# lrjconan/LanczosNetwork

Hardware: NVIDIA B200
Metric: QM8 molecules/sec (forward) (higher is better)
Workload: dtype f32

## Files before the change

include/lanczosnet_b200.h:

```cpp
#ifndef LANCZOSNET_B200_H_
#define LANCZOSNET_B200_H_

#include <stdint.h>

#ifdef __cplusplus
extern "C" {
#endif

typedef void* lnb_stream_t;

#define LNB_OK 0
#define LNB_ERR_ARG (-1)
#define LNB_ERR_UNSUPPORTED (-2)

int lnb_abi_version(void);
const char* lnb_last_error(void);
int64_t lnb_launch_count(void);

int lnb_unsorted_segment_sum_forward(lnb_stream_t stream, const float* data,
                                     const int64_t* segment_ids, const int* data_shape,
                                     int num_segments, float* output);
int lnb_unsorted_segment_sum_backward(lnb_stream_t stream, const float* grad_output,
                                      const int64_t* segment_ids, const int* data_shape,
                                      int num_segments, float* grad_data);

typedef struct lnb_gemm_desc {
  const float* A; int64_t a_sb, a_sz, a_sm, a_sk;
  const float* B; int64_t b_sb, b_sz, b_sk, b_sn;
  float* C;       int64_t c_sb, c_sz, c_sm, c_sn;
  const float* kscale; int64_t s_sb, s_sz, s_sk;
  const float* bias; int64_t bias_sz;
  int32_t batch, nz, M, N, K, relu;
  float alpha, beta;
  const float* addend; int64_t d_sb, d_sz, d_sm, d_sn;
} lnb_gemm_desc;
int lnb_batched_gemm(lnb_stream_t stream, const lnb_gemm_desc* desc );

int lnb_split_tf32(lnb_stream_t stream, const float* x, int64_t n, float* hi, float* lo);
int lnb_linear_tf32x3(lnb_stream_t stream, const float* A, const float* W_hi, const float* W_lo,
                      const float* bias, int M, int N, int K, int relu, float* C);
int lnb_linear_tf32x3_splitk(lnb_stream_t stream, const float* A, const float* W_hi, const float* W_lo,
                             const float* bias, int M, int N, int K, int relu, float* C, int splits,
                             float* workspace, int* counters);

int lnb_linear_tf32x3_grouped(lnb_stream_t stream, const float* A, const float* W_hi,
                              const float* W_lo, const float* bias, int M, int groups, int N, int K,
                              int relu, float* C);

int lnb_graph_prepare(lnb_stream_t stream, const float* L, const float* Q, int B, int N, int E1,
                      int K, float* ell_val, uint8_t* ell_idx, int32_t* ell_max, int32_t* gext,
                      int32_t* tiles, int32_t* rowmap, int32_t* nrows, int flags);
int lnb_spectral_conv_fused(lnb_stream_t stream, const float* X, const float* Q, const float* coeff,
                            const float* ell_val, const uint8_t* ell_idx, const int32_t* ell_max,
                            const int32_t* gext, const int32_t* tiles, const float* W_hi,
                            const float* W_lo, const float* bias, int B, int N, int Din, int E1,
                            int K, int S, int H, int relu, int write_pad, float* out);

int lnb_graph_prepare_sparse(lnb_stream_t stream, const int32_t* sizes, const int32_t* node_ptr,
                             const int32_t* node_feat, const int32_t* edge_ptr, const uint8_t* edges,
                             const float* V_rows, const double* inv_sqrt_deg, int B, int N, int E1,
                             int K, int flags, float* ell_val, uint8_t* ell_idx, int32_t* ell_max,
                             int32_t* gext, int32_t* tiles, int32_t* rowmap, int32_t* nrows,
                             int64_t* node_ids, uint8_t* mask, float* V, float* L_dense);

#define LNB_PACKED_HOST_TILES 2
int lnb_graph_prepare_sparse_packed(lnb_stream_t stream, const uint8_t* blob, const double* inv_sqrt_deg,
                                    int B, int N, int E1, int K, int flags, float* ell_val,
                                    uint8_t* ell_idx, int32_t* ell_max, int32_t* gext, int32_t* tiles,
                                    int32_t* rowmap, int32_t* nrows, int64_t* node_ids, uint8_t* mask,
                                    float* V, float* L_dense);

typedef struct lnb_spectral_stack {
  const float* X; const int64_t* node_ids; const float* emb_table;
  const float* Q; const float* coeff; int64_t coeff_layer_stride;
  const float* ell_val; const uint8_t* ell_idx; const int32_t* ell_max; const int32_t* gext;
  const int32_t* tiles;
  const float* W_hi; const float* W_lo; const float* bias;
  float* out_state;
  const float* W_out; const float* b_out; const float* w_att; const float* b_att;
  const uint8_t* mask; float* score;
  int32_t Din[8];
  int32_t num_layers, Kw, emb_rows, P, write_pad;
  int32_t B, N, E1, K, S, H, relu;
} lnb_spectral_stack;
int lnb_spectral_stack_forward(lnb_stream_t stream, const lnb_spectral_stack* desc );

int lnb_embedding_rows(lnb_stream_t stream, const int64_t* idx, const float* table,
                       int64_t rows, int num_embeddings, int dim, float* out);

int lnb_ritz_power_table(lnb_stream_t stream, const float* D, int64_t rows, const int* powers,
                         int S, float* table );

int lnb_ritz_rowmap(lnb_stream_t stream, const int32_t* gext, int B, int K, int32_t* rowmap,
                    int32_t* nrows);
int lnb_ritz_filter_mlp(lnb_stream_t stream, const float* table, const int32_t* rowmap,
                        const int32_t* nrows, const float* W_hi, const float* W_lo,
                        const float* bias_all, int Rall, int L, int S, int Hd, float* coeff);

int lnb_readout(lnb_stream_t stream, const float* state, const float* W_out, const float* b_out,
                const float* w_att, const float* b_att, const uint8_t* mask, int B, int N, int H,
                int P, float* score );

int lnb_operator_chain(lnb_stream_t stream, const float* L, const float* X, int B, int N, int E1,
                       int D, int steps, int chebyshev, const int* block_of_step ,
                       float* out, int64_t out_batch_stride, int64_t out_row_stride, int out_col0);

int lnb_graph_messages(lnb_stream_t stream, const float* L, const float* X, const float* Q,
                       const float* filt, int B, int N, int E1, int D, int K, int S, int dense_filter,
                       int short_steps, const int* block_of_step , int n_short, float* out,
                       int64_t out_batch_stride, int64_t out_row_stride);

int lnb_gaussian_laplacian(lnb_stream_t stream, const float* x, const float* L, int B, int N,
                           int Dx, int E1, float* out );

int lnb_lanczos_tridiag(lnb_stream_t stream, const float* A, const uint8_t* mask, const float* q1,
                        int B, int N, int K, float* T, float* Q, float* alpha, float* beta,
                        int32_t* idx);

int lnb_tridiag_ritz(lnb_stream_t stream, const float* alpha, const float* beta, const float* Q,
                     int B, int N, int K, float* theta , float* ritz_vec ,
                     int32_t* status );

#define LNB_LANCZOS_PROPER 1
int lnb_lanczos_ritz(lnb_stream_t stream, const float* A, const uint8_t* mask, const float* q1,
                     int B, int N, int K, int flags, float* T, float* Q, float* alpha, float* beta,
                     int32_t* idx, float* theta , float* ritz_vec ,
                     int32_t* status );

int lnb_tridiag_powers(lnb_stream_t stream, const float* T, int B, int K, const int* powers, int S,
                       float* out );

int lnb_symmetrize_filters(lnb_stream_t stream, const float* Y, int B, int K, int S,
                           float* G );

int lnb_debug_set_prof(unsigned long long* buf);

#ifdef __cplusplus
}
#endif
#endif
```

lanczosnetwork_b200/_lib.py:

```python
import ctypes
import os
import threading

HERE = os.path.dirname(os.path.abspath(__file__))
LIB_PATH = os.path.join(HERE, 'liblanczosnet_b200.so')

c_f32p = ctypes.c_void_p
c_stream = ctypes.c_void_p
c_int = ctypes.c_int
c_i64 = ctypes.c_int64


class GemmDesc(ctypes.Structure):
  _fields_ = [
      ('A', ctypes.c_void_p), ('a_sb', c_i64), ('a_sz', c_i64), ('a_sm', c_i64), ('a_sk', c_i64),
      ('B', ctypes.c_void_p), ('b_sb', c_i64), ('b_sz', c_i64), ('b_sk', c_i64), ('b_sn', c_i64),
      ('C', ctypes.c_void_p), ('c_sb', c_i64), ('c_sz', c_i64), ('c_sm', c_i64), ('c_sn', c_i64),
      ('kscale', ctypes.c_void_p), ('s_sb', c_i64), ('s_sz', c_i64), ('s_sk', c_i64),
      ('bias', ctypes.c_void_p), ('bias_sz', c_i64),
      ('batch', ctypes.c_int32), ('nz', ctypes.c_int32), ('M', ctypes.c_int32),
      ('N', ctypes.c_int32), ('K', ctypes.c_int32), ('relu', ctypes.c_int32),
      ('alpha', ctypes.c_float), ('beta', ctypes.c_float),
      ('addend', ctypes.c_void_p), ('d_sb', c_i64), ('d_sz', c_i64), ('d_sm', c_i64), ('d_sn', c_i64),
  ]


class SpectralStack(ctypes.Structure):
  _fields_ = [
      ('X', ctypes.c_void_p), ('node_ids', ctypes.c_void_p), ('emb_table', ctypes.c_void_p),
      ('Q', ctypes.c_void_p), ('coeff', ctypes.c_void_p), ('coeff_layer_stride', c_i64),
      ('ell_val', ctypes.c_void_p), ('ell_idx', ctypes.c_void_p), ('ell_max', ctypes.c_void_p),
      ('gext', ctypes.c_void_p), ('tiles', ctypes.c_void_p),
      ('W_hi', ctypes.c_void_p), ('W_lo', ctypes.c_void_p), ('bias', ctypes.c_void_p),
      ('out_state', ctypes.c_void_p),
      ('W_out', ctypes.c_void_p), ('b_out', ctypes.c_void_p), ('w_att', ctypes.c_void_p),
      ('b_att', ctypes.c_void_p), ('mask', ctypes.c_void_p), ('score', ctypes.c_void_p),
      ('Din', ctypes.c_int32 * 8),
      ('num_layers', ctypes.c_int32), ('Kw', ctypes.c_int32), ('emb_rows', ctypes.c_int32),
      ('P', ctypes.c_int32), ('write_pad', ctypes.c_int32),
      ('B', ctypes.c_int32), ('N', ctypes.c_int32), ('E1', ctypes.c_int32), ('K', ctypes.c_int32),
      ('S', ctypes.c_int32), ('H', ctypes.c_int32), ('relu', ctypes.c_int32),
  ]


SIGNATURES = {
    'lnb_abi_version': (c_int, []),
    'lnb_last_error': (ctypes.c_char_p, []),
    'lnb_launch_count': (c_i64, []),
    'lnb_unsorted_segment_sum_forward':
        (c_int, [c_stream, c_f32p, ctypes.c_void_p, ctypes.POINTER(c_int), c_int, c_f32p]),
    'lnb_unsorted_segment_sum_backward':
        (c_int, [c_stream, c_f32p, ctypes.c_void_p, ctypes.POINTER(c_int), c_int, c_f32p]),
    'lnb_batched_gemm': (c_int, [c_stream, ctypes.POINTER(GemmDesc)]),
    'lnb_split_tf32': (c_int, [c_stream, c_f32p, c_i64, c_f32p, c_f32p]),
    'lnb_linear_tf32x3':
        (c_int, [c_stream, c_f32p, c_f32p, c_f32p, c_f32p, c_int, c_int, c_int, c_int, c_f32p]),
    'lnb_linear_tf32x3_splitk':
        (c_int, [c_stream, c_f32p, c_f32p, c_f32p, c_f32p, c_int, c_int, c_int, c_int, c_f32p, c_int,
                 c_f32p, ctypes.c_void_p]),
    'lnb_linear_tf32x3_grouped':
        (c_int, [c_stream, c_f32p, c_f32p, c_f32p, c_f32p, c_int, c_int, c_int, c_int, c_int, c_f32p]),
    'lnb_graph_prepare': (c_int, [c_stream, c_f32p, c_f32p, c_int, c_int, c_int, c_int, c_f32p,
                                  ctypes.c_void_p, ctypes.c_void_p, ctypes.c_void_p, ctypes.c_void_p,
                                  ctypes.c_void_p, ctypes.c_void_p, c_int]),
    'lnb_graph_prepare_sparse': (c_int, [c_stream] + [ctypes.c_void_p] * 7 + [c_int] * 5 +
                                 [ctypes.c_void_p] * 11),
    'lnb_graph_prepare_sparse_packed': (c_int, [c_stream] + [ctypes.c_void_p] * 2 + [c_int] * 5 +
                                        [ctypes.c_void_p] * 11),
    'lnb_spectral_conv_fused':
        (c_int, [c_stream, c_f32p, c_f32p, c_f32p, c_f32p, ctypes.c_void_p, ctypes.c_void_p,
                 ctypes.c_void_p, ctypes.c_void_p, c_f32p, c_f32p, c_f32p, c_int, c_int, c_int,
                 c_int, c_int, c_int, c_int, c_int, c_int, c_f32p]),
    'lnb_spectral_stack_forward': (c_int, [c_stream, ctypes.POINTER(SpectralStack)]),
    'lnb_ritz_rowmap': (c_int, [c_stream, ctypes.c_void_p, c_int, c_int, ctypes.c_void_p, ctypes.c_void_p]),
    'lnb_ritz_filter_mlp': (c_int, [c_stream, c_f32p, ctypes.c_void_p, ctypes.c_void_p, c_f32p, c_f32p,
                                    c_f32p, c_int, c_int, c_int, c_int, c_f32p]),
    'lnb_debug_set_prof': (c_int, [ctypes.c_void_p]),
    'lnb_embedding_rows': (c_int, [c_stream, ctypes.c_void_p, c_f32p, c_i64, c_int, c_int, c_f32p]),
    'lnb_ritz_power_table': (c_int, [c_stream, c_f32p, c_i64, ctypes.POINTER(c_int), c_int, c_f32p]),
    'lnb_readout': (c_int, [c_stream, c_f32p, c_f32p, c_f32p, c_f32p, c_f32p, ctypes.c_void_p,
                            c_int, c_int, c_int, c_int, c_f32p]),
    'lnb_operator_chain': (c_int, [c_stream, c_f32p, c_f32p, c_int, c_int, c_int, c_int, c_int, c_int,
                                   ctypes.POINTER(c_int), c_f32p, c_i64, c_i64, c_int]),
    'lnb_graph_messages': (c_int, [c_stream, c_f32p, c_f32p, c_f32p, c_f32p, c_int, c_int, c_int, c_int, c_int,
                                   c_int, c_int, c_int, ctypes.POINTER(c_int), c_int, c_f32p, c_i64, c_i64]),
    'lnb_gaussian_laplacian': (c_int, [c_stream, c_f32p, c_f32p, c_int, c_int, c_int, c_int, c_f32p]),
    'lnb_lanczos_tridiag': (c_int, [c_stream, c_f32p, ctypes.c_void_p, c_f32p, c_int, c_int, c_int,
                                    c_f32p, c_f32p, c_f32p, c_f32p, ctypes.c_void_p]),
    'lnb_tridiag_ritz': (c_int, [c_stream, c_f32p, c_f32p, c_f32p, c_int, c_int, c_int, c_f32p,
                                 c_f32p, ctypes.c_void_p]),
    'lnb_lanczos_ritz': (c_int, [c_stream, c_f32p, ctypes.c_void_p, c_f32p, c_int, c_int, c_int, c_int,
                                 c_f32p, c_f32p, c_f32p, c_f32p, ctypes.c_void_p, c_f32p, c_f32p,
                                 ctypes.c_void_p]),
    'lnb_tridiag_powers': (c_int, [c_stream, c_f32p, c_int, c_int, ctypes.POINTER(c_int), c_int,
                                   c_f32p]),
    'lnb_symmetrize_filters': (c_int, [c_stream, c_f32p, c_int, c_int, c_int, c_f32p]),
}

_lock = threading.Lock()
_lib = None


def load():
  global _lib
  if _lib is not None:
    return _lib
  with _lock:
    if _lib is None:
      if not os.path.exists(LIB_PATH):
        raise RuntimeError(
            'liblanczosnet_b200.so is not built (%s). Build it with '
            '`python -m lanczosnetwork_b200.build` (nvcc, sm_100a). There is no CPU fallback.'
            % LIB_PATH)
      lib = ctypes.CDLL(LIB_PATH)
      for name, (res, args) in SIGNATURES.items():
        fn = getattr(lib, name)
        fn.restype = res
        fn.argtypes = args
      if lib.lnb_abi_version() != 1:
        raise RuntimeError('liblanczosnet_b200.so ABI mismatch; rebuild')
      _lib = lib
  return _lib


def check(status, what):
  if status != 0:
    msg = load().lnb_last_error()
    raise RuntimeError('%s failed (status %d): %s' % (what, status, (msg or b'').decode()))


_replayed = [0]


def note_graph_replay(num_kernels):
  _replayed[0] += int(num_kernels)


def launch_count():
  return int(load().lnb_launch_count()) + _replayed[0]
```

lanczosnetwork_b200/csrc/linear_tf32x3.cu:

```cuda
#include "tc_gemm.cuh"

namespace {

struct RowLoadPolicy {
  static constexpr int kStagesB = 6;
  struct Params {
    const float* A;
    const float* bias;
    float* C;
    int M, N, K, relu, groups;
    int dbg;
    int splits;
    float* ws;
    int* counters;
  };
  static __device__ __forceinline__ int tiles_per_group(const Params& p) { return (p.N + tcg::BN - 1) / tcg::BN; }
  static __device__ __forceinline__ int n_tiles(const Params& p) { return p.groups * tiles_per_group(p); }
  static __device__ __forceinline__ int num_tiles(const Params& p) {
    return ((p.M + tcg::BM - 1) / tcg::BM) * n_tiles(p);
  }
  static __device__ __forceinline__ int num_steps(const Params& p, int cta, int ncta) {
    const int t = num_tiles(p) * p.splits;
    return t > cta ? (t - cta + ncta - 1) / ncta : 0;
  }
  static __device__ __forceinline__ void decode(const Params& p, int cta, int ncta, int it,
                                                int& m_tile, int& sub) {
    const int item = cta + it * ncta, nt = n_tiles(p);
    const int tile = item / p.splits, split = item - tile * p.splits;
    m_tile = tile / nt;
    sub = tile % nt + nt * split;
  }
  static __device__ __forceinline__ int kb_total(const Params& p) { return (p.K + tcg::BK - 1) / tcg::BK; }
  static __device__ __forceinline__ int kb_per_split(const Params& p) { return (kb_total(p) + p.splits - 1) / p.splits; }
  static __device__ __forceinline__ int kb_begin(const Params& p, int sub) { return (sub / n_tiles(p)) * kb_per_split(p); }
  static __device__ __forceinline__ int num_kblocks(const Params& p, int sub) {
    const int left = kb_total(p) - kb_begin(p, sub), per = kb_per_split(p);
    return left < per ? left : per;
  }
  static __device__ __forceinline__ int w_row0(const Params& p, int sub) {
    const int tpg = tiles_per_group(p), ns = sub % n_tiles(p);
    return (ns / tpg) * p.N + (ns % tpg) * tcg::BN;
  }
  static __device__ __forceinline__ void w_coords(const Params& p, int sub, int kb, int& col0, int& row0) {
    col0 = (kb_begin(p, sub) + kb) * tcg::BK;
    row0 = w_row0(p, sub);
  }

  const Params& p;
  const int r, grp;
  const int lda, ldc;
  const float* arow;
  bool row_ok;
  int row, kb0, tile;
  float cur[32];
  int* flag;

  __device__ RowLoadPolicy(const Params& p_, uint8_t* smem, int tid)
      : p(p_), r(tid & 127), grp(tid >> 7), lda(p_.groups * p_.K), ldc(p_.groups * p_.N),
        arow(nullptr), row_ok(false), row(0), kb0(0), tile(0), flag(reinterpret_cast<int*>(smem)) {}

  __device__ __forceinline__ void load(int kb, float (&v)[32]) {
#pragma unroll
    for (int j = 0; j < 8; ++j) {
      const int k = (kb0 + kb) * tcg::BK + 4 * j;
      float4 t = make_float4(0.f, 0.f, 0.f, 0.f);
      if (row_ok && k < p.K) t = __ldg(reinterpret_cast<const float4*>(arow + k));
      v[4 * j + 0] = t.x; v[4 * j + 1] = t.y; v[4 * j + 2] = t.z; v[4 * j + 3] = t.w;
    }
  }
  __device__ __forceinline__ void step_begin(int m_tile, int sub, int kb_first, tcg::PhaseTimer&) {
    row = m_tile * tcg::BM + r;
    row_ok = row < p.M;
    const int ns = sub % n_tiles(p);
    kb0 = kb_begin(p, sub);
    tile = m_tile * n_tiles(p) + ns;
    arow = p.A + (int64_t)(row_ok ? row : 0) * lda + (ns / tiles_per_group(p)) * p.K;
    load(kb_first, cur);
  }
  __device__ __forceinline__ void produce(int, int kb, float (&v)[32]) {
#pragma unroll
    for (int j = 0; j < 32; ++j) v[j] = cur[j];
    load(kb + tcg::NGROUPS, cur);
  }
  __device__ __forceinline__ void pre_epilogue(int) {}
  __device__ __forceinline__ void store(int sub, int col, const float (&x)[tcg::EW]) {
    if (p.splits > 1) {
      float4* dst = reinterpret_cast<float4*>(
          p.ws + (((int64_t)tile * p.splits + sub / n_tiles(p)) * tcg::BM + r) * tcg::BN + col);
#pragma unroll
      for (int q = 0; q < tcg::EW / 4; ++q)
        __stcg(dst + q, make_float4(x[4 * q], x[4 * q + 1], x[4 * q + 2], x[4 * q + 3]));
      return;
    }
    const int left = p.N - ((sub % n_tiles(p)) % tiles_per_group(p)) * tcg::BN;
    const int w0 = w_row0(p, sub);
    tcg::store_row_chunk(row_ok ? p.C + (int64_t)row * ldc + w0 : nullptr,
                         left < tcg::BN ? left : tcg::BN, p.bias ? p.bias + w0 : nullptr,
                         p.relu != 0, col, x);
  }
  __device__ __forceinline__ void post_epilogue(int sub) {
    if (p.splits == 1) return;
    const int tid = grp * 128 + r;
    __threadfence();
    tcg::producers_sync();
    if (tid == 0) {
      const int old = atomicAdd(p.counters + tile, 1);
      *flag = (old == p.splits - 1);
      if (old == p.splits - 1) p.counters[tile] = 0;
    }
    tcg::producers_sync();
    if (*flag) {
      __threadfence();
      const int ns = sub % n_tiles(p);
      const int m0 = (tile / n_tiles(p)) * tcg::BM;
      const int left = p.N - (ns % tiles_per_group(p)) * tcg::BN;
      const int ncols = left < tcg::BN ? left : tcg::BN;
      const int w0 = w_row0(p, sub);
      const float* base = p.ws + (int64_t)tile * p.splits * tcg::BM * tcg::BN;
      for (int e = tid; e < tcg::BM * tcg::BN / 4; e += tcg::PRODUCER_THREADS) {
        const int rr = e / (tcg::BN / 4), c4 = (e - rr * (tcg::BN / 4)) * 4;
        if (m0 + rr >= p.M || c4 >= ncols) continue;
        float4 acc = __ldcg(reinterpret_cast<const float4*>(base + rr * tcg::BN + c4));
        for (int sp = 1; sp < p.splits; ++sp) {
          const float4 t = __ldcg(reinterpret_cast<const float4*>(base + ((int64_t)sp * tcg::BM + rr) * tcg::BN + c4));
          acc.x += t.x; acc.y += t.y; acc.z += t.z; acc.w += t.w;
        }
        float y[4] = {acc.x, acc.y, acc.z, acc.w};
        float* out = p.C + (int64_t)(m0 + rr) * ldc + w0 + c4;
#pragma unroll
        for (int u = 0; u < 4; ++u) {
          if (c4 + u < ncols) {
            if (p.bias) y[u] += __ldg(p.bias + w0 + c4 + u);
            if (p.relu) y[u] = fmaxf(y[u], 0.f);
            out[u] = y[u];
          }
        }
      }
    }
    tcg::producers_sync();
  }
};

constexpr size_t SMEM_BYTES = tcg::core_smem(RowLoadPolicy::kStagesB) + 1024 + 16;

}

static int launch_linear(lnb_stream_t stream, const float* A, const float* W_hi, const float* W_lo,
                         const float* bias, int M, int N, int K, int groups, int relu, float* C,
                         const char* who, int splits = 1, float* ws = nullptr, int* counters = nullptr) {
  LNB_REQUIRE(A && W_hi && W_lo && C, "%s: null pointer", who);
  LNB_REQUIRE(M >= 0 && N >= 1 && K >= 1 && groups >= 1, "%s: bad dims M=%d N=%d K=%d groups=%d",
              who, M, N, K, groups);
  LNB_REQUIRE(K % 4 == 0, "%s: K=%d must be a multiple of 4 (16-byte rows)", who, K);
  LNB_REQUIRE(((uintptr_t)A & 15) == 0 && ((uintptr_t)W_hi & 15) == 0 && ((uintptr_t)W_lo & 15) == 0,
              "%s: A / W must be 16-byte aligned", who);
  if (M == 0) return LNB_OK;
  CUtensorMap map_hi, map_lo;
  int rc = tcg::make_weight_map(&map_hi, W_hi, groups * N, K, who);
  if (rc != LNB_OK) return rc;
  rc = tcg::make_weight_map(&map_lo, W_lo, groups * N, K, who);
  if (rc != LNB_OK) return rc;
  auto kern = tcg::tc_gemm_kernel<RowLoadPolicy>;
  cudaFuncSetAttribute(kern, cudaFuncAttributeMaxDynamicSharedMemorySize, (int)SMEM_BYTES);
  const int nkb = lnb::ceil_div(K, tcg::BK);
  LNB_REQUIRE(splits >= 1 && splits <= 16 && (splits == 1 || (ws && counters)),
              "%s: split-K needs 1 <= splits <= 16, a workspace and counters", who);
  LNB_REQUIRE(splits == 1 || lnb::ceil_div(nkb, splits) * (splits - 1) < nkb,
              "%s: %d splits leave an empty k range for K=%d", who, splits, K);
  RowLoadPolicy::Params p{A, bias, C, M, N, K, relu, groups, tcg::debug_flags(), splits, ws, counters};
  const int tiles = lnb::ceil_div(M, tcg::BM) * lnb::ceil_div(N, tcg::BN) * groups * splits;
  const int grid = tiles < tcg::sm_count() ? tiles : tcg::sm_count();
  kern<<<grid, tcg::THREADS, SMEM_BYTES, (cudaStream_t)stream>>>(map_hi, map_lo, p);
  lnb::count_launch();
  return lnb::finish_launch(who);
}

extern "C" {

int lnb_linear_tf32x3(lnb_stream_t stream, const float* A, const float* W_hi, const float* W_lo,
                      const float* bias, int M, int N, int K, int relu, float* C) {
  return launch_linear(stream, A, W_hi, W_lo, bias, M, N, K, 1, relu, C, "linear_tf32x3");
}

int lnb_linear_tf32x3_splitk(lnb_stream_t stream, const float* A, const float* W_hi, const float* W_lo,
                             const float* bias, int M, int N, int K, int relu, float* C, int splits,
                             float* workspace, int* counters) {
  return launch_linear(stream, A, W_hi, W_lo, bias, M, N, K, 1, relu, C, "linear_tf32x3_splitk", splits,
                       workspace, counters);
}

int lnb_linear_tf32x3_grouped(lnb_stream_t stream, const float* A, const float* W_hi,
                              const float* W_lo, const float* bias, int M, int groups, int N, int K,
                              int relu, float* C) {
  return launch_linear(stream, A, W_hi, W_lo, bias, M, N, K, groups, relu, C,
                       "linear_tf32x3_grouped");
}

}
```

lanczosnetwork_b200/csrc/spectral_conv_fused.cu:

```cuda
#include "tc_gemm.cuh"

namespace {

constexpr int KMAX = 32;
constexpr int GMAX = 32;
constexpr int RMAX = 128;
constexpr int EMAX = 16;
constexpr int FR = 8;

template <bool STAGE>
__global__ void __launch_bounds__(256)
graph_prepare_kernel(const float* __restrict__ L, const float* __restrict__ Q, int N, int E1, int K,
                     float* __restrict__ ell_val, uint8_t* __restrict__ ell_idx,
                     int32_t* __restrict__ ell_max, int32_t* __restrict__ gext, int binarize) {
  extern __shared__ __align__(16) float gp_smem[];
  __shared__ int s_max[EMAX];
  __shared__ int s_ext[2];
  __shared__ uint8_t cnt_s[256 * EMAX];
  const int b = blockIdx.x, tid = threadIdx.x;
  if (tid < EMAX) s_max[tid] = 0;
  if (tid < 2) s_ext[tid] = 0;
  const int64_t per = (int64_t)N * N * E1;
  const float* Lg = L + b * per;
  if (STAGE) {
    if ((per & 3) == 0) {
      for (int i = tid; i < (int)(per >> 2); i += 256) tc05::cp_async_16(gp_smem + 4 * i, Lg + 4 * i);
    } else {
      for (int i = tid; i < (int)per; i += 256) tc05::cp_async_4(gp_smem + i, Lg + i);
    }
  }
  const float* Lb = STAGE ? gp_smem : Lg;
  const float* Qb = Q + (int64_t)b * N * K;
  int ne = 0, ke = 0;
  for (int i = tid; i < N * K; i += 256) {
    if (__ldg(Qb + i) != 0.f) {
      ne = max(ne, i / K + 1);
      ke = max(ke, i % K + 1);
    }
  }
  if (STAGE) tc05::cp_async_wait_all();
  __syncthreads();
  const int pairs = N * E1;
  for (int p = tid; p < pairs; p += 256) {
    const int n = p / E1, e = p - n * E1;
    const float* row = Lb + (n * N) * E1 + e;
    float* val = ell_val + ((int64_t)(b * E1 + e) * N) * N + n;
    uint8_t* idx = ell_idx + ((int64_t)(b * E1 + e) * N) * N + n;
    int cnt = 0, far = 0;
    const float dg = row[n * E1];
    if (dg != 0.f) {
      val[0] = binarize ? 1.f : dg;
      idx[0] = (uint8_t)n;
      cnt = 1;
      far = n + 1;
    }
#pragma unroll 2
    for (int i = 0; i < N; ++i) {
      const float v = row[i * E1];
      if (v != 0.f && i != n) {
        val[cnt * N] = binarize ? 1.f : v;
        idx[cnt * N] = (uint8_t)i;
        ++cnt;
        far = max(far, i + 1);
      }
    }
    cnt_s[p] = (uint8_t)cnt;
    if (cnt) {
      atomicMax(&s_max[e], cnt);
      ne = max(ne, max(n + 1, far));
    }
  }
  if (ne) atomicMax(&s_ext[0], ne);
  if (ke) atomicMax(&s_ext[1], ke);
  __syncthreads();
  for (int pr = tid; pr < pairs; pr += 256) {
    const int n = pr / E1, e = pr - n * E1;
    float* val = ell_val + ((int64_t)(b * E1 + e) * N) * N + n;
    uint8_t* idx = ell_idx + ((int64_t)(b * E1 + e) * N) * N + n;
    for (int t = cnt_s[pr]; t < s_max[e]; ++t) {
      val[(int64_t)t * N] = 0.f;
      idx[(int64_t)t * N] = 0;
    }
  }
  if (tid < E1) ell_max[b * E1 + tid] = s_max[tid];
  if (tid < 2) gext[b * 2 + tid] = s_ext[tid];
}

template <bool in_smem>
__global__ void __launch_bounds__(1024)
tile_assign_kernel(const int32_t* __restrict__ gext, int B, int K, int32_t* __restrict__ tiles,
                   int32_t* __restrict__ scratch , int32_t* __restrict__ rowmap,
                   int32_t* __restrict__ nrows) {
  extern __shared__ int32_t ta_smem[];
  __shared__ int warp_n[32], warp_k[32], warp_r[32];
  __shared__ int run_n, run_k, run_r;
  const int tid = threadIdx.x, lane = tid & 31, warp = tid >> 5;
  int32_t* PN = in_smem ? ta_smem : scratch;
  int32_t* PK = PN + B;
  int32_t* NX = PK + B;
  int32_t* PR = NX + 3 * (B + 1);
  if (tid == 0) { run_n = 0; run_k = 0; run_r = 0; }
  __syncthreads();
  for (int b0 = 0; b0 < B; b0 += 1024) {
    const int b = b0 + tid;
    const int n = (b < B) ? gext[b * 2] : 0;
    const int kr = (b < B) ? min(gext[b * 2 + 1], K) : 0;
    const int k = (b < B) ? ((gext[b * 2 + 1] + 3) & ~3) : 0;
    int in = n, ik = k, ir = kr;
#pragma unroll
    for (int o = 1; o < 32; o <<= 1) {
      const int tn = __shfl_up_sync(0xffffffffu, in, o), tk = __shfl_up_sync(0xffffffffu, ik, o);
      const int tr = __shfl_up_sync(0xffffffffu, ir, o);
      if (lane >= o) { in += tn; ik += tk; ir += tr; }
    }
    if (lane == 31) { warp_n[warp] = in; warp_k[warp] = ik; warp_r[warp] = ir; }
    __syncthreads();
    if (warp == 0) {
      int wn = warp_n[lane], wk = warp_k[lane], wr = warp_r[lane], sn = wn, sk = wk, sr = wr;
#pragma unroll
      for (int o = 1; o < 32; o <<= 1) {
        const int tn = __shfl_up_sync(0xffffffffu, sn, o), tk = __shfl_up_sync(0xffffffffu, sk, o);
        const int tr = __shfl_up_sync(0xffffffffu, sr, o);
        if (lane >= o) { sn += tn; sk += tk; sr += tr; }
      }
      warp_n[lane] = sn - wn;
      warp_k[lane] = sk - wk;
      warp_r[lane] = sr - wr;
    }
    __syncthreads();
    if (b < B) {
      PN[b] = run_n + warp_n[warp] + in;
      PK[b] = run_k + warp_k[warp] + ik;
      if (in_smem) {
        PR[b] = run_r + warp_r[warp] + ir;
      } else if (rowmap) {
        const int base = run_r + warp_r[warp] + ir - kr;
        for (int i = 0; i < kr; ++i) rowmap[base + i] = b * K + i;
      }
    }
    __syncthreads();
    if (tid == 1023) { run_n += warp_n[31] + in; run_k += warp_k[31] + ik; run_r += warp_r[31] + ir; }
    __syncthreads();
  }
  if (tid == 0 && nrows) nrows[0] = run_r;
  __threadfence_block();
  if (in_smem && rowmap) {
    for (int b = warp; b < B; b += 32) {
      const int base = b ? PR[b - 1] : 0, kr = PR[b] - base;
      for (int i = lane; i < kr; i += 32) rowmap[base + i] = b * K + i;
    }
  }
  for (int i = tid; i < B; i += 1024) {
    const int pn0 = i ? PN[i - 1] : 0, pk0 = i ? PK[i - 1] : 0;
    int j = i + 1;
    const int jmax = min(B, i + GMAX);
    while (j < jmax && PN[j] - pn0 <= RMAX && PK[j] - pk0 <= RMAX) ++j;
    NX[i] = j;
  }
  __syncthreads();
  if (!in_smem) {
    if (tid == 0) {
      int T = 0, i = 0;
      while (i < B) { tiles[1 + T] = i; ++T; i = NX[i]; }
      tiles[0] = T;
      tiles[1 + T] = B;
    }
    return;
  }
  int32_t* Ja = NX;
  int32_t* Jb = NX + (B + 1);
  int32_t* MK = Jb + (B + 1);
  for (int i = tid; i <= B; i += 1024) MK[i] = (i == 0) ? 1 : 0;
  if (tid == 0) { Ja[B] = B; Jb[B] = B; }
  __syncthreads();
  for (int span = 1; span < B; span <<= 1) {
    for (int i = tid; i < B; i += 1024)
      if (MK[i]) MK[Ja[i]] = 1;
    for (int i = tid; i < B; i += 1024) Jb[i] = Ja[Ja[i]];
    __syncthreads();
    int32_t* t = Ja; Ja = Jb; Jb = t;
  }
  if (tid == 0) run_n = 0;
  __syncthreads();
  for (int b0 = 0; b0 < B; b0 += 1024) {
    const int b = b0 + tid;
    const int m = (b < B) ? MK[b] : 0;
    int in = m;
#pragma unroll
    for (int o = 1; o < 32; o <<= 1) {
      const int tn = __shfl_up_sync(0xffffffffu, in, o);
      if (lane >= o) in += tn;
    }
    if (lane == 31) warp_n[warp] = in;
    __syncthreads();
    if (warp == 0) {
      int wn = warp_n[lane], sn = wn;
#pragma unroll
      for (int o = 1; o < 32; o <<= 1) {
        const int tn = __shfl_up_sync(0xffffffffu, sn, o);
        if (lane >= o) sn += tn;
      }
      warp_n[lane] = sn - wn;
    }
    __syncthreads();
    if (m) tiles[1 + run_n + warp_n[warp] + in - 1] = b;
    __syncthreads();
    if (tid == 1023) run_n += warp_n[31] + in;
    __syncthreads();
  }
  if (tid == 0) {
    tiles[0] = run_n;
    tiles[1 + run_n] = B;
  }
}

struct SpectralPolicy {
  static constexpr int kStagesB = 2;
  static constexpr int LMAX = 8;
  struct Params {
    const float* X;
    const int64_t* node_ids;
    const float* emb;
    const float* Q;
    const float* coeff;
    int64_t coeff_stride;
    const float* ell_val;
    const uint8_t* ell_idx;
    const int32_t* ell_max;
    const int32_t* gext;
    const int32_t* tiles;
    const float* bias;
    float* out;
    const float* W_out;
    const float* b_out;
    const float* w_att;
    const float* b_att;
    const uint8_t* mask;
    float* score;
    int P, emb_rows;
    int L;
    int Din[LMAX];
    int B, N, E1, K, S, H, relu;
    int LB;
    int write_pad;
    int dbg;
  };
  static __device__ __forceinline__ int num_steps(const Params& p, int cta, int ncta) {
    const int T = __ldg(p.tiles);
    const int mine = T > cta ? (T - cta + ncta - 1) / ncta : 0;
    return (p.S > 0 ? 2 : 1) * p.L * mine;
  }
  static __device__ __forceinline__ void decode(const Params& p, int cta, int ncta, int it,
                                                int& m_tile, int& sub) {
    const int per = (p.S > 0 ? 2 : 1) * p.L;
    const int rem = it % per;
    m_tile = cta + (it / per) * ncta;
    sub = p.S > 0 ? rem : rem * 2 + 1;
  }
  static __device__ __forceinline__ int num_kblocks(const Params& p, int sub) {
    return ((sub & 1) == 0 ? p.S : p.E1) * p.Din[sub >> 1] / tcg::BK;
  }
  static __device__ __forceinline__ void w_coords(const Params& p, int sub, int kb, int& col0, int& row0) {
    col0 = ((sub & 1) == 0 ? 0 : p.S * p.Din[sub >> 1]) + kb * tcg::BK;
    row0 = (sub >> 1) * p.H;
  }

  struct Tables {
    int gs, ng, Rtot, Ztot, nquads, nlines;
    int nbase[GMAX + 1], kbase[GMAX + 1], gn[GMAX], gk[GMAX];
    int cnt_e[EMAX], base_e[EMAX], tmax_e[EMAX];
    uint8_t emax[GMAX][EMAX];
    uint8_t row_g[RMAX], row_n[RMAX], z_g[RMAX], z_k[RMAX];
    uint8_t q_g[RMAX / 4 + GMAX], q_n0[RMAX / 4 + GMAX];
    uint8_t line_e[256], line_t[256];
  };

  const Params& p;
  const int tid, r;
  const int N, K, S, E1, H, XP;
  int Din;
  float* Xs;
  float* UZ;
  float* Qs;
  Tables* tb;
  float* Ev;
  uint8_t* Ei;
  float fr[FR];
  tcg::PhaseTimer* ptm = nullptr;

  static __host__ __device__ constexpr size_t tables_bytes() { return (sizeof(Tables) + 15) & ~size_t(15); }

  __device__ SpectralPolicy(const Params& p_, uint8_t* smem, int tid_)
      : p(p_), tid(tid_), r(tid_ & 127), N(p_.N), K(p_.K), S(p_.S), E1(p_.E1),
        H(p_.H), XP((p_.Din[0] > p_.H ? p_.Din[0] : p_.H) + 4), Din(p_.Din[0]) {
    Xs = reinterpret_cast<float*>(smem);
    UZ = Xs + (size_t)RMAX * XP;
    Qs = UZ + (size_t)RMAX * XP;
    uint8_t* t8 = reinterpret_cast<uint8_t*>(Qs + (size_t)RMAX * K);
    tb = reinterpret_cast<Tables*>(t8);
    Ev = reinterpret_cast<float*>(t8 + tables_bytes());
    Ei = reinterpret_cast<uint8_t*>(Ev + (size_t)p.LB * RMAX);
  }
  static size_t smem_fixed(int Din, int K, int H) {
    const int W = (Din > H ? Din : H) + 4;
    return (size_t)2 * RMAX * W * 4 + (size_t)RMAX * K * 4 + tables_bytes() + 16;
  }
  static size_t ell_line_bytes() { return (size_t)RMAX * 5; }

  __device__ void build_tables(int m_tile) {
    const int lane = tid & 31;
    const int gs = __ldg(p.tiles + 1 + m_tile), ge = __ldg(p.tiles + 2 + m_tile);
    const int ng = ge - gs;
    int n = 0, k = 0;
    if (lane < ng) {
      n = __ldg(p.gext + (gs + lane) * 2);
      k = __ldg(p.gext + (gs + lane) * 2 + 1);
    }
    const int kp = (k + 3) & ~3, nq = (n + 3) >> 2;
    int pn = n, pk = kp, pq = nq;
#pragma unroll
    for (int o = 1; o < 32; o <<= 1) {
      const int a = __shfl_up_sync(0xffffffffu, pn, o), bq = __shfl_up_sync(0xffffffffu, pk, o);
      const int c = __shfl_up_sync(0xffffffffu, pq, o);
      if (lane >= o) { pn += a; pk += bq; pq += c; }
    }
    const int nb = pn - n, kb = pk - kp, qb = pq - nq;
    if (lane < ng) {
      tb->nbase[lane] = nb; tb->kbase[lane] = kb; tb->gn[lane] = n; tb->gk[lane] = k;
      for (int i = 0; i < n; ++i) { tb->row_g[nb + i] = (uint8_t)lane; tb->row_n[nb + i] = (uint8_t)i; }
      for (int i = 0; i < kp; ++i) { tb->z_g[kb + i] = (uint8_t)lane; tb->z_k[kb + i] = (uint8_t)i; }
      for (int i = 0; i < nq; ++i) { tb->q_g[qb + i] = (uint8_t)lane; tb->q_n0[qb + i] = (uint8_t)(4 * i); }
    }
    const int Rtot = __shfl_sync(0xffffffffu, pn, 31), Ztot = __shfl_sync(0xffffffffu, pk, 31);
    const int nquads = __shfl_sync(0xffffffffu, pq, 31);
    int em[EMAX];
#pragma unroll
    for (int e = 0; e < EMAX; ++e)
      em[e] = (e < E1 && lane < ng) ? __ldg(p.ell_max + (gs + lane) * E1 + e) : 0;
#pragma unroll
    for (int e = 0; e < EMAX; ++e) {
      if (e < E1) {
        int m = em[e];
        if (lane < ng) tb->emax[lane][e] = (uint8_t)m;
#pragma unroll
        for (int o = 16; o > 0; o >>= 1) m = max(m, __shfl_xor_sync(0xffffffffu, m, o));
        if (lane == 0) tb->tmax_e[e] = m;
      }
    }
    __syncwarp();
    if (lane == 0) {
      tb->gs = gs; tb->ng = ng; tb->Rtot = Rtot; tb->Ztot = Ztot; tb->nquads = nquads;
      tb->nbase[ng] = Rtot; tb->kbase[ng] = Ztot;
      int left = p.LB, base = 0;
      for (int e = 0; e < E1; ++e) {
        const int c = min(tb->tmax_e[e], left);
        tb->cnt_e[e] = c; tb->base_e[e] = base;
        for (int t = 0; t < c; ++t) { tb->line_e[base + t] = (uint8_t)e; tb->line_t[base + t] = (uint8_t)t; }
        base += c; left -= c;
      }
      tb->nlines = base;
    }
  }

  __device__ void step_begin(int m_tile, int sub, int , tcg::PhaseTimer& tm) {
    tcg::producers_sync();
    const int layer = sub >> 1, step = sub & 1;
    if (step == 1 && S > 0) return;
    Din = p.Din[layer];
    const int warp = tid >> 5, lane = tid & 31;
    constexpr int NW = tcg::PRODUCER_THREADS / 32;
    const int dv = Din / 4;
    ptm = &tm;
    if (layer == 0) {
    if (warp == 0) build_tables(m_tile);
    tcg::producers_sync();
    tm.lap(16);
    const int gs = tb->gs, Rtot = tb->Rtot;
    int64_t my_id = 0;
    if (!p.X && warp + lane * NW < Rtot) {
      const int row = warp + lane * NW;
      my_id = __ldg(p.node_ids + (int64_t)(gs + tb->row_g[row]) * N + tb->row_n[row]);
    }
    for (int row = warp, j = 0; row < Rtot; row += NW, ++j) {
      const int64_t src_row = (int64_t)(gs + tb->row_g[row]) * N + tb->row_n[row];
      const float* xsrc;
      if (p.X) {
        xsrc = p.X + src_row * Din;
      } else {
        int64_t id = __shfl_sync(0xffffffffu, my_id, j);
        id = id < 0 ? 0 : (id >= p.emb_rows ? p.emb_rows - 1 : id);
        xsrc = p.emb + id * Din;
      }
      float* xd = Xs + (size_t)row * XP;
      for (int q4 = lane; q4 < dv; q4 += 32) tc05::cp_async_16(xd + 4 * q4, xsrc + 4 * q4);
      const float* qsrc = p.Q + src_row * K;
      float* qd = Qs + (size_t)row * K;
      for (int k4 = lane; k4 < (K >> 2); k4 += 32) tc05::cp_async_16(qd + 4 * k4, qsrc + 4 * k4);
    }
    tm.lap(17);
    {
      constexpr int ELL_BATCH = 4;
      const int nlines = tb->nlines;
      for (int base = warp; base < nlines; base += NW * ELL_BATCH) {
        for (int r0 = 0; r0 < Rtot; r0 += 32) {
          const int rr = r0 + lane;
          float vv[ELL_BATCH];
          int ii[ELL_BATCH];
#pragma unroll
          for (int u = 0; u < ELL_BATCH; ++u) {
            const int line = base + u * NW;
            vv[u] = 0.f; ii[u] = 0;
            if (line < nlines && rr < Rtot) {
              const int e = tb->line_e[line], t = tb->line_t[line];
              const int g = tb->row_g[rr], n = tb->row_n[rr];
              if (t < tb->emax[g][e]) {
                const int64_t off = (((int64_t)(gs + g) * E1 + e) * N + t) * N + n;
                vv[u] = __ldg(p.ell_val + off);
                ii[u] = tb->nbase[g] + __ldg(p.ell_idx + off);
              }
            }
          }
#pragma unroll
          for (int u = 0; u < ELL_BATCH; ++u) {
            const int line = base + u * NW;
            if (line < nlines && rr < Rtot) {
              Ev[(size_t)line * RMAX + rr] = vv[u];
              Ei[(size_t)line * RMAX + rr] = (uint8_t)ii[u];
            }
          }
        }
      }
    }
    tm.lap(18);
    }
    const int gs = tb->gs, Ztot = tb->Ztot;
#pragma unroll
    for (int i = 0; i < FR; ++i) fr[i] = 0.f;
    if (S > 0 && r < Ztot) {
      const int g = tb->z_g[r], k = tb->z_k[r];
      if (k < tb->gk[g]) {
        const float* f = p.coeff + layer * p.coeff_stride + ((int64_t)(gs + g) * K + k) * S;
#pragma unroll
        for (int i = 0; i < FR; ++i)
          if (i < S) fr[i] = __ldg(f + i);
      }
    }
    tm.lap(0);
    tc05::cp_async_wait_all();
    tcg::producers_sync();
    tm.lap(1);
    if (S == 0) return;
    for (int task = tid; task < (Ztot >> 2) * dv; task += tcg::PRODUCER_THREADS) {
      const int dq = task % dv, zq = task / dv;
      const int g = tb->z_g[4 * zq], k0 = tb->z_k[4 * zq];
      const int n_g = tb->gn[g], nb = tb->nbase[g];
      float acc[4][4];
#pragma unroll
      for (int i = 0; i < 4; ++i)
#pragma unroll
        for (int j = 0; j < 4; ++j) acc[i][j] = 0.f;
      const float* xs = Xs + (size_t)nb * XP + 4 * dq;
      const float* qs = Qs + (size_t)nb * K + k0;
#pragma unroll 4
      for (int nn = 0; nn < n_g; ++nn) {
        const float4 x4 = *reinterpret_cast<const float4*>(xs + (size_t)nn * XP);
        const float4 q4 = *reinterpret_cast<const float4*>(qs + (size_t)nn * K);
        const float qv[4] = {q4.x, q4.y, q4.z, q4.w};
        const float xv[4] = {x4.x, x4.y, x4.z, x4.w};
#pragma unroll
        for (int i = 0; i < 4; ++i)
#pragma unroll
          for (int j = 0; j < 4; ++j) acc[i][j] = fmaf(qv[i], xv[j], acc[i][j]);
      }
#pragma unroll
      for (int i = 0; i < 4; ++i)
        *reinterpret_cast<float4*>(UZ + (size_t)(4 * zq + i) * XP + 4 * dq) =
            make_float4(acc[i][0], acc[i][1], acc[i][2], acc[i][3]);
    }
    tcg::producers_sync();
    tm.lap(2);
  }

  __device__ __forceinline__ void produce(int sub, int kb, float (&v)[32]) {
#pragma unroll
    for (int j = 0; j < 32; ++j) v[j] = 0.f;
    const int j0 = kb * tcg::BK;
    const int c = j0 / Din, d0 = j0 - c * Din;
    if ((sub & 1) == 0) {
      if (r >= tb->Ztot) return;
      float f = 0.f;
      if (S <= FR) {
#pragma unroll
        for (int i = 0; i < FR; ++i) f = (i == c) ? fr[i] : f;
      } else {
        const int g = tb->z_g[r], k = tb->z_k[r];
        f = (k < tb->gk[g]) ? __ldg(p.coeff + (sub >> 1) * p.coeff_stride + ((int64_t)(tb->gs + g) * K + k) * S + c) : 0.f;
      }
      const float4* u4 = reinterpret_cast<const float4*>(UZ + (size_t)r * XP + d0);
#pragma unroll
      for (int q = 0; q < 8; ++q) {
        const float4 t = u4[q];
        v[4 * q + 0] = f * t.x; v[4 * q + 1] = f * t.y; v[4 * q + 2] = f * t.z; v[4 * q + 3] = f * t.w;
      }
      return;
    }
    if (r >= tb->Rtot) return;
    const int e = c;
    const float* xs = Xs + d0;
    const int ts = tb->cnt_e[e], tmax = tb->tmax_e[e];
    const float* ev = Ev + (size_t)tb->base_e[e] * RMAX + r;
    const uint8_t* ei = Ei + (size_t)tb->base_e[e] * RMAX + r;
#pragma unroll 2
    for (int t = 0; t < ts; ++t) {
      const float a = ev[t * RMAX];
      if (a == 0.f) continue;
      const int i = ei[t * RMAX];
      const float4* x4 = reinterpret_cast<const float4*>(xs + (size_t)i * XP);
#pragma unroll
      for (int q = 0; q < 8; ++q) {
        const float4 tt = x4[q];
        v[4 * q + 0] = fmaf(a, tt.x, v[4 * q + 0]);
        v[4 * q + 1] = fmaf(a, tt.y, v[4 * q + 1]);
        v[4 * q + 2] = fmaf(a, tt.z, v[4 * q + 2]);
        v[4 * q + 3] = fmaf(a, tt.w, v[4 * q + 3]);
      }
    }
    if (ts < tmax) {
      const int g = tb->row_g[r], n = tb->row_n[r];
      const int my = tb->emax[g][e], nb = tb->nbase[g];
      const int64_t off0 = (((int64_t)(tb->gs + g) * E1 + e) * N) * N + n;
      for (int t = ts; t < tmax; ++t) {
        float a = 0.f;
        int i = 0;
        if (t < my) {
          a = __ldg(p.ell_val + off0 + (int64_t)t * N);
          i = nb + __ldg(p.ell_idx + off0 + (int64_t)t * N);
        }
        if (a == 0.f) continue;
        const float4* x4 = reinterpret_cast<const float4*>(xs + (size_t)i * XP);
#pragma unroll
        for (int q = 0; q < 8; ++q) {
          const float4 tt = x4[q];
          v[4 * q + 0] = fmaf(a, tt.x, v[4 * q + 0]);
          v[4 * q + 1] = fmaf(a, tt.y, v[4 * q + 1]);
          v[4 * q + 2] = fmaf(a, tt.z, v[4 * q + 2]);
          v[4 * q + 3] = fmaf(a, tt.w, v[4 * q + 3]);
        }
      }
    }
  }

  __device__ void pre_epilogue(int sub) {
    if ((sub & 1) == 0) return;
    tcg::producers_sync();
    if (ptm) ptm->lap(22);
    if (S == 0) return;
    const int hv = H / 4;
    for (int task = tid; task < tb->nquads * hv; task += tcg::PRODUCER_THREADS) {
      const int hq = task % hv, q = task / hv;
      const int g = tb->q_g[q], n0 = tb->q_n0[q];
      const int n_g = tb->gn[g], k_g = tb->gk[g];
      const int r0 = tb->nbase[g] + n0;
      float acc[4][4];
#pragma unroll
      for (int i = 0; i < 4; ++i)
#pragma unroll
        for (int j = 0; j < 4; ++j) acc[i][j] = 0.f;
      const float* z = UZ + (size_t)tb->kbase[g] * XP + 4 * hq;
      const float* q0 = Qs + (size_t)r0 * K;
      const int r1 = (n0 + 1 < n_g) ? 1 : 0, r2 = (n0 + 2 < n_g) ? 2 : 0, r3 = (n0 + 3 < n_g) ? 3 : 0;
      for (int k = 0; k < k_g; k += 4) {
        const float4 a0 = *reinterpret_cast<const float4*>(q0 + k);
        const float4 a1 = *reinterpret_cast<const float4*>(q0 + r1 * K + k);
        const float4 a2 = *reinterpret_cast<const float4*>(q0 + r2 * K + k);
        const float4 a3 = *reinterpret_cast<const float4*>(q0 + r3 * K + k);
        const float av[4][4] = {{a0.x, a0.y, a0.z, a0.w}, {a1.x, a1.y, a1.z, a1.w},
                                {a2.x, a2.y, a2.z, a2.w}, {a3.x, a3.y, a3.z, a3.w}};
#pragma unroll
        for (int kk = 0; kk < 4; ++kk) {
          const float4 z4 = *reinterpret_cast<const float4*>(z + (size_t)(k + kk) * XP);
          const float zv[4] = {z4.x, z4.y, z4.z, z4.w};
#pragma unroll
          for (int i = 0; i < 4; ++i)
#pragma unroll
            for (int j = 0; j < 4; ++j) acc[i][j] = fmaf(av[i][kk], zv[j], acc[i][j]);
        }
      }
#pragma unroll
      for (int i = 0; i < 4; ++i)
        if (n0 + i < n_g)
          *reinterpret_cast<float4*>(Xs + (size_t)(r0 + i) * XP + 4 * hq) =
              make_float4(acc[i][0], acc[i][1], acc[i][2], acc[i][3]);
    }
    tcg::producers_sync();
  }

  __device__ __forceinline__ void store(int sub, int col, float (&x)[tcg::EW]) {
    if (col >= H) return;
    if ((sub & 1) == 0) {
      if (r < tb->Ztot) {
        float4* z4 = reinterpret_cast<float4*>(UZ + (size_t)r * XP + col);
#pragma unroll
        for (int q = 0; q < tcg::EW / 4; ++q)
          z4[q] = make_float4(x[4 * q + 0], x[4 * q + 1], x[4 * q + 2], x[4 * q + 3]);
      }
      return;
    }
    if (r >= tb->Rtot) return;
    float4* o4 = reinterpret_cast<float4*>(Xs + (size_t)r * XP + col);
    const bool relu = p.relu != 0;
    const float* bias = p.bias ? p.bias + (sub >> 1) * H : nullptr;
#pragma unroll
    for (int q = 0; q < tcg::EW / 4; ++q) {
      float y[4] = {x[4 * q + 0], x[4 * q + 1], x[4 * q + 2], x[4 * q + 3]};
      if (S > 0) {
        const float4 t = o4[q];
        y[0] += t.x; y[1] += t.y; y[2] += t.z; y[3] += t.w;
      }
      if (col + 4 * q + 3 < H) {
        if (bias) {
          const float4 b4 = __ldg(reinterpret_cast<const float4*>(bias + col) + q);
          y[0] += b4.x; y[1] += b4.y; y[2] += b4.z; y[3] += b4.w;
        }
        if (relu) { y[0] = fmaxf(y[0], 0.f); y[1] = fmaxf(y[1], 0.f); y[2] = fmaxf(y[2], 0.f); y[3] = fmaxf(y[3], 0.f); }
      } else {
#pragma unroll
        for (int u = 0; u < 4; ++u) {
          const int c = col + 4 * q + u;
          if (c < H) {
            if (bias) y[u] += __ldg(bias + c);
            if (relu) y[u] = fmaxf(y[u], 0.f);
          }
        }
      }
      o4[q] = make_float4(y[0], y[1], y[2], y[3]);
    }
  }

  __device__ void post_epilogue(int sub) {
    if ((sub & 1) == 0 || (sub >> 1) != p.L - 1) return;
    tcg::producers_sync();
    if (ptm) ptm->lap(19);
    const int warp = tid >> 5, lane = tid & 31;
    constexpr int NW = tcg::PRODUCER_THREADS / 32;
    const int hv = H / 4, gs = tb->gs, Rtot = tb->Rtot;
    const float* bias = p.bias ? p.bias + (p.L - 1) * H : nullptr;
    if (p.out) {
      for (int row = warp; row < Rtot; row += NW) {
        const float4* src = reinterpret_cast<const float4*>(Xs + (size_t)row * XP);
        float4* dst = reinterpret_cast<float4*>(
            p.out + ((int64_t)(gs + tb->row_g[row]) * N + tb->row_n[row]) * H);
        for (int q4 = lane; q4 < hv; q4 += 32) dst[q4] = src[q4];
      }
      if (p.write_pad) {
        const int npad = tb->ng * N - Rtot;
        for (int i = warp; i < npad; i += NW) {
          int g = 0, rem = i;
          while (rem >= N - tb->gn[g]) { rem -= N - tb->gn[g]; ++g; }
          float4* dst = reinterpret_cast<float4*>(p.out + ((int64_t)(gs + g) * N + tb->gn[g] + rem) * H);
          for (int q4 = lane; q4 < hv; q4 += 32) {
            float y[4];
#pragma unroll
            for (int u = 0; u < 4; ++u) {
              float t = bias ? __ldg(bias + 4 * q4 + u) : 0.f;
              y[u] = (p.relu != 0) ? fmaxf(t, 0.f) : t;
            }
            dst[q4] = make_float4(y[0], y[1], y[2], y[3]);
          }
        }
      }
    }
    if (p.score) readout(bias);
  }

  __device__ void readout(const float* bias_last) {
    const int P = p.P, P1 = p.P + 1, PQ = (P1 + 3) >> 2, HP = H + 4;
    float* Wr = UZ;
    float* Yr = Wr + (size_t)4 * PQ * HP;
    float* cx = Yr + (size_t)(RMAX + 1) * P1 + ((4 - ((RMAX + 1) * P1 & 3)) & 3);
    for (int e = tid; e < 4 * PQ * H; e += tcg::PRODUCER_THREADS) {
      const int o = e / H, h = e - o * H;
      Wr[o * HP + h] = (o < P) ? __ldg(p.W_out + o * H + h) : (o == P ? __ldg(p.w_att + h) : 0.f);
    }
    for (int h = tid; h < H; h += tcg::PRODUCER_THREADS) {
      float t = bias_last ? __ldg(bias_last + h) : 0.f;
      cx[h] = (p.relu != 0) ? fmaxf(t, 0.f) : t;
    }
    uint8_t* mk = reinterpret_cast<uint8_t*>(cx + H);
    for (int e = tid; e < tb->ng * N; e += tcg::PRODUCER_THREADS)
      mk[e] = p.mask ? __ldg(p.mask + (int64_t)tb->gs * N + e) : (uint8_t)1;
    tcg::producers_sync();
    if (ptm) ptm->lap(20);
    const int Rtot = tb->Rtot;
    {
      const int warp = tid >> 5, lane = tid & 31;
      const int rb = warp & 3, og = warp >> 2;
      const int per = (P1 + tcg::NGROUPS - 1) / tcg::NGROUPS;
      const int o_end = min(P1, (og + 1) * per);
      const int row = rb * 32 + lane;
      const float4* x4 = reinterpret_cast<const float4*>(Xs + (size_t)(row < Rtot ? row : 0) * XP);
      for (int o0 = og * per; o0 < o_end; o0 += 6) {
        const int cnt = min(6, o_end - o0);
        const float4* w4 = reinterpret_cast<const float4*>(Wr + (size_t)o0 * HP);
        float acc[6] = {0.f, 0.f, 0.f, 0.f, 0.f, 0.f};
#pragma unroll 4
        for (int h4 = 0; h4 < H / 4; ++h4) {
          const float4 x = x4[h4];
#pragma unroll
          for (int j = 0; j < 6; ++j) {
            if (j < cnt) {
              const float4 wv = w4[j * (HP / 4) + h4];
              acc[j] = fmaf(x.x, wv.x, acc[j]); acc[j] = fmaf(x.y, wv.y, acc[j]);
              acc[j] = fmaf(x.z, wv.z, acc[j]); acc[j] = fmaf(x.w, wv.w, acc[j]);
            }
          }
        }
        if (row < Rtot) {
#pragma unroll
          for (int j = 0; j < 6; ++j)
            if (j < cnt) {
              const int o = o0 + j;
              const float v = acc[j] + ((o < P) ? __ldg(p.b_out + o) : __ldg(p.b_att));
              Yr[row * P1 + o] = (o < P) ? v : 1.f / (1.f + expf(-v));
            }
        }
      }
      for (int o = warp; o < P1; o += tcg::PRODUCER_THREADS / 32) {
        float acc = 0.f;
        for (int h = lane; h < H; h += 32) acc = fmaf(cx[h], Wr[o * HP + h], acc);
#pragma unroll
        for (int sh = 16; sh > 0; sh >>= 1) acc += __shfl_xor_sync(0xffffffffu, acc, sh);
        if (lane == 0) {
          const float v = acc + ((o < P) ? __ldg(p.b_out + o) : __ldg(p.b_att));
          Yr[RMAX * P1 + o] = (o < P) ? v : 1.f / (1.f + expf(-v));
        }
      }
    }
    tcg::producers_sync();
    if (ptm) ptm->lap(21);
    for (int e = tid; e < tb->ng * P; e += tcg::PRODUCER_THREADS) {
      const int g = e / P, o = e - g * P;
      const int nb = tb->nbase[g], n_g = tb->gn[g];
      const uint8_t* m = mk + g * N;
      float acc = 0.f;
      int cnt = 0;
      for (int n = 0; n < N; ++n) {
        if (m[n] == 0) continue;
        const float* y = Yr + (n < n_g ? nb + n : RMAX) * P1;
        acc += y[P] * y[o];
        ++cnt;
      }
      p.score[(int64_t)(tb->gs + g) * P + o] = acc / (float)cnt;
    }
  }
};

}

namespace lnb {
void launch_tile_assign(cudaStream_t s, const int32_t* gext, int B, int K, int32_t* tiles,
                        int32_t* rowmap, int32_t* nrows) {
  const size_t tbytes = (size_t)6 * (B + 1) * sizeof(int32_t);
  const int tsm = tbytes <= 200 * 1024;
  if (tsm && tbytes > 40 * 1024)
    cudaFuncSetAttribute(tile_assign_kernel<true>, cudaFuncAttributeMaxDynamicSharedMemorySize, (int)tbytes);
  if (tsm)
    tile_assign_kernel<true><<<1, 1024, tbytes, s>>>(gext, B, K, tiles, tiles + B + 2, rowmap, nrows);
  else
    tile_assign_kernel<false><<<1, 1024, 0, s>>>(gext, B, K, tiles, tiles + B + 2, rowmap, nrows);
}
}

extern "C" {

int lnb_debug_set_prof(unsigned long long* buf) {
  cudaError_t e = cudaMemcpyToSymbol(tcg::g_prof, &buf, sizeof(buf));
  if (e != cudaSuccess) { lnb::set_err("debug_set_prof: %s", cudaGetErrorString(e)); return (int)e; }
  lnb::set_prof_buffer(buf);
  return LNB_OK;
}

int lnb_graph_prepare(lnb_stream_t stream, const float* L, const float* Q, int B, int N, int E1,
                      int K, float* ell_val, uint8_t* ell_idx, int32_t* ell_max, int32_t* gext,
                      int32_t* tiles ,
                      int32_t* rowmap, int32_t* nrows, int flags) {
  LNB_REQUIRE(L && Q && ell_val && ell_idx && ell_max && gext && tiles, "graph_prepare: null pointer");
  LNB_REQUIRE((rowmap == nullptr) == (nrows == nullptr), "graph_prepare: rowmap and nrows go together");
  LNB_REQUIRE(B >= 0 && N >= 1 && N <= 255 && E1 >= 1 && E1 <= EMAX && K >= 1,
              "graph_prepare: bad dims B=%d N=%d E1=%d K=%d", B, N, E1, K);
  if (B == 0) return LNB_OK;
  cudaStream_t s = (cudaStream_t)stream;
  const size_t lbytes = (size_t)N * N * E1 * sizeof(float);
  const int stage = lbytes <= 64 * 1024;
  if (stage) {
    if (lbytes > 40 * 1024)
      cudaFuncSetAttribute(graph_prepare_kernel<true>, cudaFuncAttributeMaxDynamicSharedMemorySize, (int)lbytes);
    graph_prepare_kernel<true><<<B, 256, lbytes, s>>>(L, Q, N, E1, K, ell_val, ell_idx, ell_max, gext,
                                                      flags & 1);
  } else {
    graph_prepare_kernel<false><<<B, 256, 0, s>>>(L, Q, N, E1, K, ell_val, ell_idx, ell_max, gext,
                                                  flags & 1);
  }
  lnb::launch_tile_assign(s, gext, B, K, tiles, rowmap, nrows);
  lnb::count_launch(2);
  return lnb::finish_launch("graph_prepare");
}

static int launch_stack(lnb_stream_t stream, const lnb_spectral_stack& d, const char* who) {
  LNB_REQUIRE((d.X || (d.node_ids && d.emb_table)) && d.Q && d.ell_val && d.ell_idx && d.ell_max &&
                  d.gext && d.tiles && d.W_hi && d.W_lo && (d.out_state || d.score) &&
                  (d.coeff || d.S == 0),
              "%s: null pointer", who);
  LNB_REQUIRE(d.B >= 0 && d.N >= 1 && d.E1 >= 1 && d.K >= 1 && d.S >= 0 && d.H >= 1 &&
                  d.num_layers >= 1 && d.num_layers <= SpectralPolicy::LMAX,
              "%s: bad dims", who);
  LNB_REQUIRE(!d.score || (d.W_out && d.b_out && d.w_att && d.b_att && d.P >= 1 && d.P <= 48),
              "%s: readout needs W_out, b_out, w_att, b_att and 1 <= P <= 48", who);
  int dmax = 0;
  bool ok = d.N <= RMAX && d.K <= KMAX && d.K % 4 == 0 && d.H % 4 == 0 && d.H <= tcg::BN && d.E1 <= EMAX;
  for (int l = 0; l < d.num_layers; ++l) {
    ok = ok && d.Din[l] % 32 == 0 && d.Din[l] >= 32 && (l == 0 || d.Din[l] == d.H);
    dmax = d.Din[l] > dmax ? d.Din[l] : dmax;
  }
  ok = ok && (d.S + d.E1) * dmax <= d.Kw;
  if (!ok) {
    lnb::set_err("%s: unsupported shape N=%d K=%d H=%d E1=%d (needs N<=128, Din%%32==0, inner "
                 "layers Din==H, K%%4==0, K<=%d, H%%4==0, H<=128, E1<=%d)", who, d.N, d.K, d.H, d.E1,
                 KMAX, EMAX);
    return LNB_ERR_UNSUPPORTED;
  }
  if ((d.bias && (reinterpret_cast<uintptr_t>(d.bias) & 15)) || (reinterpret_cast<uintptr_t>(d.Q) & 15) ||
      (d.X && (reinterpret_cast<uintptr_t>(d.X) & 15)) || (d.emb_table && (reinterpret_cast<uintptr_t>(d.emb_table) & 15))) {
    lnb::set_err("%s: X / emb_table / Q / bias must be 16-byte aligned", who);
    return LNB_ERR_ARG;
  }
  if (d.B == 0) return LNB_OK;
  size_t smem = tcg::core_smem(SpectralPolicy::kStagesB) + 1024 + SpectralPolicy::smem_fixed(dmax, d.K, d.H);
  if (smem > 227 * 1024) {
    lnb::set_err("%s: tile state (Din=%d, K=%d, H=%d) needs %zu B of shared memory", who, dmax, d.K,
                 d.H, smem);
    return LNB_ERR_UNSUPPORTED;
  }
  int lb = (int)((227 * 1024 - smem) / SpectralPolicy::ell_line_bytes());
  if (lb > 255) lb = 255;
  smem += (size_t)lb * SpectralPolicy::ell_line_bytes();
  CUtensorMap map_hi, map_lo;
  int rc = tcg::make_weight_map(&map_hi, d.W_hi, d.num_layers * d.H, d.Kw, who);
  if (rc != LNB_OK) return rc;
  rc = tcg::make_weight_map(&map_lo, d.W_lo, d.num_layers * d.H, d.Kw, who);
  if (rc != LNB_OK) return rc;
  auto kern = tcg::tc_gemm_kernel<SpectralPolicy>;
  cudaFuncSetAttribute(kern, cudaFuncAttributeMaxDynamicSharedMemorySize, (int)smem);
  SpectralPolicy::Params p{};
  p.X = d.X; p.node_ids = d.node_ids; p.emb = d.emb_table; p.Q = d.Q;
  p.coeff = d.coeff; p.coeff_stride = d.coeff_layer_stride;
  p.ell_val = d.ell_val; p.ell_idx = d.ell_idx; p.ell_max = d.ell_max; p.gext = d.gext; p.tiles = d.tiles;
  p.bias = d.bias; p.out = d.out_state;
  p.W_out = d.W_out; p.b_out = d.b_out; p.w_att = d.w_att; p.b_att = d.b_att; p.mask = d.mask;
  p.score = d.score; p.P = d.P; p.emb_rows = d.emb_rows; p.L = d.num_layers;
  for (int l = 0; l < d.num_layers; ++l) p.Din[l] = d.Din[l];
  p.B = d.B; p.N = d.N; p.E1 = d.E1; p.K = d.K; p.S = d.S; p.H = d.H; p.relu = d.relu;
  p.LB = lb; p.write_pad = d.write_pad; p.dbg = tcg::debug_flags();
  const int grid = d.B < tcg::sm_count() ? d.B : tcg::sm_count();
  kern<<<grid, tcg::THREADS, smem, (cudaStream_t)stream>>>(map_hi, map_lo, p);
  lnb::count_launch();
  return lnb::finish_launch(who);
}

int lnb_spectral_stack_forward(lnb_stream_t stream, const lnb_spectral_stack* desc) {
  LNB_REQUIRE(desc, "spectral_stack_forward: null descriptor");
  return launch_stack(stream, *desc, "spectral_stack_forward");
}

int lnb_spectral_conv_fused(lnb_stream_t stream, const float* X, const float* Q, const float* coeff,
                            const float* ell_val, const uint8_t* ell_idx, const int32_t* ell_max,
                            const int32_t* gext, const int32_t* tiles, const float* W_hi,
                            const float* W_lo, const float* bias, int B, int N, int Din, int E1,
                            int K, int S, int H, int relu, int write_pad, float* out) {
  lnb_spectral_stack d{};
  d.X = X; d.Q = Q; d.coeff = coeff; d.coeff_layer_stride = 0;
  d.ell_val = ell_val; d.ell_idx = ell_idx; d.ell_max = ell_max; d.gext = gext; d.tiles = tiles;
  d.W_hi = W_hi; d.W_lo = W_lo; d.Kw = (S + E1) * Din; d.bias = bias;
  d.Din[0] = Din; d.num_layers = 1; d.out_state = out; d.write_pad = write_pad;
  d.B = B; d.N = N; d.E1 = E1; d.K = K; d.S = S; d.H = H; d.relu = relu;
  return launch_stack(stream, d, "spectral_conv_fused");
}

}
```

lanczosnetwork_b200/csrc/tc05.cuh:

```cuda
#pragma once
#include <cuda.h>
#include <cuda_runtime.h>
#include <stdint.h>

namespace tc05 {

__device__ __forceinline__ uint32_t smem_u32(const void* p) {
  return static_cast<uint32_t>(__cvta_generic_to_shared(p));
}

__device__ __forceinline__ void mbar_init(uint64_t* bar, uint32_t count) {
  asm volatile("mbarrier.init.shared::cta.b64 [%0], %1;" ::"r"(smem_u32(bar)), "r"(count));
}
__device__ __forceinline__ void fence_barrier_init() {
  asm volatile("fence.mbarrier_init.release.cluster;" ::: "memory");
}
__device__ __forceinline__ void mbar_arrive(uint64_t* bar) {
  asm volatile("mbarrier.arrive.shared::cta.b64 _, [%0];" ::"r"(smem_u32(bar)) : "memory");
}
__device__ __forceinline__ void mbar_arrive_expect_tx(uint64_t* bar, uint32_t bytes) {
  asm volatile("mbarrier.arrive.expect_tx.shared::cta.b64 _, [%0], %1;" ::"r"(smem_u32(bar)),
               "r"(bytes)
               : "memory");
}
__device__ __forceinline__ bool mbar_try_wait(uint64_t* bar, uint32_t parity) {
  uint32_t ok;
  asm volatile(
      "{\n\t.reg .pred p;\n\t"
      "mbarrier.try_wait.parity.shared::cta.b64 p, [%1], %2;\n\t"
      "selp.b32 %0, 1, 0, p;\n\t}"
      : "=r"(ok)
      : "r"(smem_u32(bar)), "r"(parity)
      : "memory");
  return ok != 0;
}
__device__ __forceinline__ void mbar_wait(uint64_t* bar, uint32_t parity) {
  while (!mbar_try_wait(bar, parity)) {
  }
}
__device__ __forceinline__ void mbar_wait2(uint64_t* bar_a, uint32_t parity_a, uint64_t* bar_b,
                                           uint32_t parity_b) {
  bool oka = mbar_try_wait(bar_a, parity_a), okb = mbar_try_wait(bar_b, parity_b);
  while (!(oka && okb)) {
    if (!oka) oka = mbar_try_wait(bar_a, parity_a);
    if (!okb) okb = mbar_try_wait(bar_b, parity_b);
  }
}

__device__ __forceinline__ void tma_prefetch_desc(const CUtensorMap* m) {
  asm volatile("prefetch.tensormap [%0];" ::"l"(reinterpret_cast<uint64_t>(m)) : "memory");
}
__device__ __forceinline__ void tma_load_2d(void* smem_dst, const CUtensorMap* m, uint64_t* bar,
                                            int32_t c0, int32_t c1) {
  asm volatile(
      "cp.async.bulk.tensor.2d.shared::cluster.global.mbarrier::complete_tx::bytes"
      " [%0], [%1, {%3, %4}], [%2];"
      ::"r"(smem_u32(smem_dst)), "l"(reinterpret_cast<uint64_t>(m)), "r"(smem_u32(bar)), "r"(c0),
      "r"(c1)
      : "memory");
}

__device__ __forceinline__ void cp_async_16(void* smem_dst, const void* gmem_src) {
  asm volatile("cp.async.cg.shared.global [%0], [%1], 16;" ::"r"(smem_u32(smem_dst)), "l"(gmem_src)
               : "memory");
}
__device__ __forceinline__ void cp_async_4(void* smem_dst, const void* gmem_src) {
  asm volatile("cp.async.ca.shared.global [%0], [%1], 4;" ::"r"(smem_u32(smem_dst)), "l"(gmem_src)
               : "memory");
}
__device__ __forceinline__ void cp_async_wait_all() {
  asm volatile("cp.async.commit_group;\n\tcp.async.wait_group 0;" ::: "memory");
}

__device__ __forceinline__ void tmem_alloc(uint32_t* smem_holder, uint32_t ncols) {
  asm volatile("tcgen05.alloc.cta_group::1.sync.aligned.shared::cta.b32 [%0], %1;" ::"r"(
                   smem_u32(smem_holder)),
               "r"(ncols)
               : "memory");
  asm volatile("tcgen05.relinquish_alloc_permit.cta_group::1.sync.aligned;" ::: "memory");
}
__device__ __forceinline__ void tmem_dealloc(uint32_t taddr, uint32_t ncols) {
  asm volatile("tcgen05.dealloc.cta_group::1.sync.aligned.b32 %0, %1;" ::"r"(taddr), "r"(ncols)
               : "memory");
}
__device__ __forceinline__ void fence_before_thread_sync() {
  asm volatile("tcgen05.fence::before_thread_sync;" ::: "memory");
}
__device__ __forceinline__ void fence_after_thread_sync() {
  asm volatile("tcgen05.fence::after_thread_sync;" ::: "memory");
}
__device__ __forceinline__ void tmem_wait_ld() {
  asm volatile("tcgen05.wait::ld.sync.aligned;" ::: "memory");
}
__device__ __forceinline__ void tmem_wait_st() {
  asm volatile("tcgen05.wait::st.sync.aligned;" ::: "memory");
}

__device__ __forceinline__ void tmem_ld_32x32(uint32_t taddr, uint32_t (&v)[32]) {
  asm volatile(
      "tcgen05.ld.sync.aligned.32x32b.x32.b32 "
      "{%0, %1, %2, %3, %4, %5, %6, %7, %8, %9, %10, %11, %12, %13, %14, %15, "
      "%16, %17, %18, %19, %20, %21, %22, %23, %24, %25, %26, %27, %28, %29, %30, %31}, [%32];"
      : "=r"(v[0]), "=r"(v[1]), "=r"(v[2]), "=r"(v[3]), "=r"(v[4]), "=r"(v[5]), "=r"(v[6]),
        "=r"(v[7]), "=r"(v[8]), "=r"(v[9]), "=r"(v[10]), "=r"(v[11]), "=r"(v[12]), "=r"(v[13]),
        "=r"(v[14]), "=r"(v[15]), "=r"(v[16]), "=r"(v[17]), "=r"(v[18]), "=r"(v[19]),
        "=r"(v[20]), "=r"(v[21]), "=r"(v[22]), "=r"(v[23]), "=r"(v[24]), "=r"(v[25]),
        "=r"(v[26]), "=r"(v[27]), "=r"(v[28]), "=r"(v[29]), "=r"(v[30]), "=r"(v[31])
      : "r"(taddr)
      : "memory");
}
__device__ __forceinline__ void tmem_ld_32x16(uint32_t taddr, uint32_t (&v)[16]) {
  asm volatile(
      "tcgen05.ld.sync.aligned.32x32b.x16.b32 "
      "{%0, %1, %2, %3, %4, %5, %6, %7, %8, %9, %10, %11, %12, %13, %14, %15}, [%16];"
      : "=r"(v[0]), "=r"(v[1]), "=r"(v[2]), "=r"(v[3]), "=r"(v[4]), "=r"(v[5]), "=r"(v[6]),
        "=r"(v[7]), "=r"(v[8]), "=r"(v[9]), "=r"(v[10]), "=r"(v[11]), "=r"(v[12]), "=r"(v[13]),
        "=r"(v[14]), "=r"(v[15])
      : "r"(taddr)
      : "memory");
}
__device__ __forceinline__ void tmem_st_32x32(uint32_t taddr, const uint32_t (&v)[32]) {
  asm volatile(
      "tcgen05.st.sync.aligned.32x32b.x32.b32 [%0], "
      "{%1, %2, %3, %4, %5, %6, %7, %8, %9, %10, %11, %12, %13, %14, %15, %16, "
      "%17, %18, %19, %20, %21, %22, %23, %24, %25, %26, %27, %28, %29, %30, %31, %32};"
      ::"r"(taddr), "r"(v[0]), "r"(v[1]), "r"(v[2]), "r"(v[3]), "r"(v[4]), "r"(v[5]), "r"(v[6]),
      "r"(v[7]), "r"(v[8]), "r"(v[9]), "r"(v[10]), "r"(v[11]), "r"(v[12]), "r"(v[13]),
      "r"(v[14]), "r"(v[15]), "r"(v[16]), "r"(v[17]), "r"(v[18]), "r"(v[19]), "r"(v[20]),
      "r"(v[21]), "r"(v[22]), "r"(v[23]), "r"(v[24]), "r"(v[25]), "r"(v[26]), "r"(v[27]),
      "r"(v[28]), "r"(v[29]), "r"(v[30]), "r"(v[31])
      : "memory");
}

__device__ __forceinline__ uint64_t umma_desc_kmajor_sw128(uint32_t smem_addr) {
  uint64_t d = 0;
  d |= (uint64_t)((smem_addr >> 4) & 0x3FFFu);
  d |= (uint64_t)1 << 16;
  d |= (uint64_t)64 << 32;
  d |= (uint64_t)1 << 46;
  d |= (uint64_t)2 << 61;
  return d;
}

__host__ __device__ constexpr uint32_t umma_idesc_tf32(int M, int N) {
  return (1u << 4)
         | (2u << 7)
         | (2u << 10)
         | ((uint32_t)(N >> 3) << 17) | ((uint32_t)(M >> 4) << 24);
}

__device__ __forceinline__ void umma_tf32_ts(uint32_t d_tmem, uint32_t a_tmem, uint64_t b_desc,
                                             uint32_t idesc, uint32_t accumulate) {
  asm volatile(
      "{\n\t.reg .pred p;\n\t"
      "setp.ne.b32 p, %4, 0;\n\t"
      "tcgen05.mma.cta_group::1.kind::tf32 [%0], [%1], %2, %3, p;\n\t}"
      ::"r"(d_tmem), "r"(a_tmem), "l"(b_desc), "r"(idesc), "r"(accumulate)
      : "memory");
}
__device__ __forceinline__ void umma_tf32_ss(uint32_t d_tmem, uint64_t a_desc, uint64_t b_desc,
                                             uint32_t idesc, uint32_t accumulate) {
  asm volatile(
      "{\n\t.reg .pred p;\n\t"
      "setp.ne.b32 p, %4, 0;\n\t"
      "tcgen05.mma.cta_group::1.kind::tf32 [%0], %1, %2, %3, p;\n\t}"
      ::"r"(d_tmem), "l"(a_desc), "l"(b_desc), "r"(idesc), "r"(accumulate)
      : "memory");
}
__device__ __forceinline__ void umma_commit(uint64_t* bar) {
  asm volatile("tcgen05.commit.cta_group::1.mbarrier::arrive::one.shared::cluster.b64 [%0];" ::"r"(
                   smem_u32(bar))
               : "memory");
}

__device__ __forceinline__ bool elect_one() {
  uint32_t pred;
  asm volatile(
      "{\n\t.reg .pred p;\n\t"
      "elect.sync _|p, 0xffffffff;\n\t"
      "selp.b32 %0, 1, 0, p;\n\t}"
      : "=r"(pred));
  return pred != 0;
}

__device__ __forceinline__ uint32_t tf32_rna_bits(float v) {
  uint32_t r;
  asm("cvt.rna.tf32.f32 %0, %1;" : "=r"(r) : "f"(v));
  return r;
}

}
```

lanczosnetwork_b200/csrc/tc_gemm.cuh:

```cuda
#pragma once
#include "common.cuh"
#include "tc05.cuh"
#include <stdlib.h>

namespace tcg {

constexpr int BM = 128, BN = 128, BK = 32;
constexpr int NGROUPS = 3;
constexpr int TILE_B_BYTES = BN * BK * 4;
constexpr int STAGE_B_BYTES = 2 * TILE_B_BYTES;
constexpr int EW = 16;
constexpr int TMEM_COLS = 512;
constexpr int COL_MAIN = 0, COL_CORR = 128, COL_A = 256;
constexpr int PRODUCER_THREADS = 128 * NGROUPS;
constexpr int TMA_WARP = 4 * NGROUPS, MMA_WARP = 4 * NGROUPS + 1;
constexpr int THREADS = PRODUCER_THREADS + 64;
constexpr int MAX_B_STAGES = 6;
__host__ __device__ constexpr int core_smem(int stages_b) { return stages_b * STAGE_B_BYTES + 256; }

struct Core {
  uint8_t* Bst;
  uint64_t* b_full;
  uint64_t* b_empty;
  uint64_t* a_full;
  uint64_t* a_empty;
  uint64_t* acc_full;
  uint64_t* acc_empty;
  uint32_t* tmem_holder;
};

__device__ __forceinline__ Core carve(uint8_t* base, int stages_b) {
  Core c;
  c.Bst = base;
  uint64_t* bars = reinterpret_cast<uint64_t*>(base + stages_b * STAGE_B_BYTES);
  c.b_full = bars;
  c.b_empty = c.b_full + MAX_B_STAGES;
  c.a_full = c.b_empty + MAX_B_STAGES;
  c.a_empty = c.a_full + NGROUPS;
  c.acc_full = c.a_empty + NGROUPS;
  c.acc_empty = c.acc_full + 1;
  c.tmem_holder = reinterpret_cast<uint32_t*>(c.acc_empty + 1);
  return c;
}

__device__ unsigned long long* g_prof = nullptr;

struct PhaseTimer {
  unsigned long long* buf;
  long long t0;
  __device__ __forceinline__ void start(int cta, int tid) {
    buf = (tid == 0 && g_prof) ? g_prof + cta * 32 : nullptr;
    if (buf) t0 = clock64();
  }
  __device__ __forceinline__ void lap(int slot) {
    if (buf) { long long t = clock64(); atomicAdd(&buf[slot], (unsigned long long)(t - t0)); t0 = t; }
  }
};

__device__ __forceinline__ void producers_sync() {
  asm volatile("bar.sync 1, %0;" ::"n"(PRODUCER_THREADS) : "memory");
}

template <class Policy>
__global__ void __launch_bounds__(THREADS, 1)
tc_gemm_kernel(const __grid_constant__ CUtensorMap map_hi,
               const __grid_constant__ CUtensorMap map_lo, const typename Policy::Params p) {
  extern __shared__ __align__(16) uint8_t smem_raw[];
  const uint32_t pad = (1024u - (tc05::smem_u32(smem_raw) & 1023u)) & 1023u;
  uint8_t* base = smem_raw + pad;
  constexpr int SB = Policy::kStagesB;
  Core c = carve(base, SB);
  uint8_t* policy_smem = base + core_smem(SB);

  const int tid = threadIdx.x, warp = tid >> 5, lane = tid & 31;
  const int cta = blockIdx.x, ncta = gridDim.x;
  const int nsteps = Policy::num_steps(p, cta, ncta);
  unsigned long long prof_ns0 = 0;
  long long prof_c0 = 0;
  if (tid == 0 && g_prof) {
    asm volatile("mov.u64 %0, %globaltimer;" : "=l"(prof_ns0));
    prof_c0 = clock64();
  }

  if (warp == TMA_WARP && lane == 0) {
    tc05::tma_prefetch_desc(&map_hi);
    tc05::tma_prefetch_desc(&map_lo);
  }
  if (warp == MMA_WARP) {
    if (lane == 0) {
      for (int s = 0; s < SB; ++s) { tc05::mbar_init(&c.b_full[s], 1); tc05::mbar_init(&c.b_empty[s], 1); }
      for (int s = 0; s < NGROUPS; ++s) { tc05::mbar_init(&c.a_full[s], 4); tc05::mbar_init(&c.a_empty[s], 1); }
      tc05::mbar_init(c.acc_full, 1);
      tc05::mbar_init(c.acc_empty, 4 * NGROUPS);
      tc05::fence_barrier_init();
    }
    __syncwarp();
    tc05::tmem_alloc(c.tmem_holder, TMEM_COLS);
  }
  tc05::fence_before_thread_sync();
  __syncthreads();
  tc05::fence_after_thread_sync();
  const uint32_t tmem_base = *c.tmem_holder;

  if (warp < TMA_WARP) {
    const int grp = warp >> 2;
    const int wq = warp & 3;
    const uint32_t lane_addr = tmem_base + ((uint32_t)(wq * 32) << 16);
    const uint32_t a_hi = lane_addr + COL_A + grp * 64;
    Policy pol(p, policy_smem, tid);
    uint32_t use = 0;
    uint32_t gk0 = 0;
    for (int it = 0; it < nsteps; ++it) {
      int m_tile, sub;
      Policy::decode(p, cta, ncta, it, m_tile, sub);
      const int nkb = Policy::num_kblocks(p, sub);
      const int kb_first = (grp + NGROUPS - (int)(gk0 % NGROUPS)) % NGROUPS;
      gk0 += nkb;
      PhaseTimer tm;
      tm.start(cta, tid);
      pol.step_begin(m_tile, sub, kb_first, tm);
      for (int kb = kb_first; kb < nkb; kb += NGROUPS, ++use) {
        float v[32];
        if (!(p.dbg & 8)) pol.produce(sub, kb, v);
        tc05::mbar_wait(&c.a_empty[grp], (use & 1u) ^ 1u);
        tc05::fence_after_thread_sync();
        if (!(p.dbg & 1)) {
          uint32_t part[32];
#pragma unroll
          for (int j = 0; j < 32; ++j) part[j] = tc05::tf32_rna_bits(v[j]);
          tc05::tmem_st_32x32(a_hi, part);
#pragma unroll
          for (int j = 0; j < 32; ++j) part[j] = tc05::tf32_rna_bits(v[j] - __uint_as_float(part[j]));
          tc05::tmem_st_32x32(a_hi + 32, part);
          tc05::tmem_wait_st();
        }
        tc05::fence_before_thread_sync();
        __syncwarp();
        if (lane == 0) tc05::mbar_arrive(&c.a_full[grp]);
      }
      tm.lap((sub & 1) ? 8 : 3);
      pol.pre_epilogue(sub);
      tm.lap(4);
      tc05::mbar_wait(c.acc_full, (uint32_t)it & 1u);
      tc05::fence_after_thread_sync();
      tm.lap((sub & 1) ? 9 : 5);
      {
        uint32_t vm[EW], vc[EW];
        tc05::tmem_ld_32x16(lane_addr + COL_MAIN + grp * EW, vm);
        tc05::tmem_ld_32x16(lane_addr + COL_CORR + grp * EW, vc);
        tc05::tmem_wait_ld();
#pragma unroll 1
        for (int cc = grp; cc < BN / EW; cc += NGROUPS) {
          const int col = cc * EW;
          float x[EW];
#pragma unroll
          for (int j = 0; j < EW; ++j) x[j] = __uint_as_float(vm[j]) + __uint_as_float(vc[j]);
          if (cc + NGROUPS < BN / EW) {
            tc05::tmem_ld_32x16(lane_addr + COL_MAIN + col + NGROUPS * EW, vm);
            tc05::tmem_ld_32x16(lane_addr + COL_CORR + col + NGROUPS * EW, vc);
          }
          tm.lap(6);
          pol.store(sub, col, x);
          tc05::tmem_wait_ld();
          tm.lap(7);
        }
      }
      tc05::fence_before_thread_sync();
      __syncwarp();
      if (lane == 0) tc05::mbar_arrive(c.acc_empty);
      pol.post_epilogue(sub);
      tm.lap(10);
    }
  } else if (warp == TMA_WARP) {
    uint32_t cnt = 0;
    for (int it = 0; it < nsteps; ++it) {
      int m_tile, sub;
      Policy::decode(p, cta, ncta, it, m_tile, sub);
      const int nkb = Policy::num_kblocks(p, sub);
      for (int kb = 0; kb < nkb; ++kb, ++cnt) {
        int col0, row0;
        Policy::w_coords(p, sub, kb, col0, row0);
        const uint32_t st = cnt % SB;
        tc05::mbar_wait(&c.b_empty[st], ((cnt / SB) & 1u) ^ 1u);
        if (tc05::elect_one()) {
          if (p.dbg & 4) {
            tc05::mbar_arrive(&c.b_full[st]);
          } else {
            uint8_t* dst = c.Bst + st * STAGE_B_BYTES;
            tc05::mbar_arrive_expect_tx(&c.b_full[st], STAGE_B_BYTES);
            tc05::tma_load_2d(dst, &map_hi, &c.b_full[st], col0, row0);
            tc05::tma_load_2d(dst + TILE_B_BYTES, &map_lo, &c.b_full[st], col0, row0);
          }
        }
        __syncwarp();
      }
    }
  } else {
    constexpr uint32_t idesc256 = tc05::umma_idesc_tf32(BM, 2 * BN);
    constexpr uint32_t idesc128 = tc05::umma_idesc_tf32(BM, BN);
    uint32_t cnt = 0;
    const uint32_t d_main = tmem_base + COL_MAIN, d_corr = tmem_base + COL_CORR;
    for (int it = 0; it < nsteps; ++it) {
      int m_tile, sub;
      Policy::decode(p, cta, ncta, it, m_tile, sub);
      const int nkb = Policy::num_kblocks(p, sub);
      tc05::mbar_wait(c.acc_empty, ((uint32_t)it & 1u) ^ 1u);
      tc05::fence_after_thread_sync();
      for (int kb = 0; kb < nkb; ++kb, ++cnt) {
        const uint32_t sb = cnt % SB, sa = cnt % NGROUPS;
        tc05::mbar_wait2(&c.b_full[sb], (cnt / SB) & 1u, &c.a_full[sa], (cnt / NGROUPS) & 1u);
        tc05::fence_after_thread_sync();
        if (tc05::elect_one()) {
          const uint32_t a_hi = tmem_base + COL_A + sa * 64, a_lo = a_hi + 32;
          const uint64_t dB = tc05::umma_desc_kmajor_sw128(tc05::smem_u32(c.Bst + sb * STAGE_B_BYTES));
          if (!(p.dbg & 2)) {
#pragma unroll
            for (int k = 0; k < BK / 8; ++k) {
              const uint32_t acc = (kb | k) != 0 ? 1u : 0u;
              tc05::umma_tf32_ts(d_main, a_hi + 8 * k, dB + 2 * k, idesc256, acc);
              tc05::umma_tf32_ts(d_corr, a_lo + 8 * k, dB + 2 * k, idesc128, 1u);
            }
          }
          tc05::umma_commit(&c.a_empty[sa]);
          tc05::umma_commit(&c.b_empty[sb]);
          if (kb == nkb - 1) tc05::umma_commit(c.acc_full);
        }
        __syncwarp();
      }
    }
  }

  tc05::fence_before_thread_sync();
  __syncthreads();
  if (warp == MMA_WARP) {
    __syncwarp();
    tc05::tmem_dealloc(tmem_base, TMEM_COLS);
  }
  if (tid == 0 && g_prof) {
    unsigned long long ns1;
    asm volatile("mov.u64 %0, %globaltimer;" : "=l"(ns1));
    atomicAdd(&g_prof[cta * 32 + 11], ns1 - prof_ns0);
    atomicAdd(&g_prof[cta * 32 + 12], (unsigned long long)(clock64() - prof_c0));
    g_prof[cta * 32 + 13] = prof_ns0;
  }
}

__device__ __forceinline__ void store_row_chunk(float* orow, int ncols, const float* bias, bool relu,
                                                int col, const float (&x)[EW]) {
  if (orow == nullptr || col >= ncols) return;
  const bool vec_ok = (reinterpret_cast<uintptr_t>(orow + col) & 15) == 0;
#pragma unroll
  for (int j = 0; j < EW; j += 4) {
    float o[4];
#pragma unroll
    for (int u = 0; u < 4; ++u) {
      const int n = col + j + u;
      float y = x[j + u];
      if (n < ncols) {
        if (bias) y += __ldg(bias + n);
        if (relu) y = fmaxf(y, 0.f);
      }
      o[u] = y;
    }
    if (vec_ok && col + j + 3 < ncols) {
      *reinterpret_cast<float4*>(orow + col + j) = make_float4(o[0], o[1], o[2], o[3]);
    } else {
#pragma unroll
      for (int u = 0; u < 4; ++u)
        if (col + j + u < ncols) orow[col + j + u] = o[u];
    }
  }
}

typedef CUresult (*EncodeTiledFn)(CUtensorMap*, CUtensorMapDataType, cuuint32_t, void*,
                                  const cuuint64_t*, const cuuint64_t*, const cuuint32_t*,
                                  const cuuint32_t*, CUtensorMapInterleave, CUtensorMapSwizzle,
                                  CUtensorMapL2promotion, CUtensorMapFloatOOBfill);

inline EncodeTiledFn get_encode_fn() {
  static EncodeTiledFn fn = nullptr;
  if (!fn) {
    void* ptr = nullptr;
    cudaDriverEntryPointQueryResult q;
    if (cudaGetDriverEntryPoint("cuTensorMapEncodeTiled", &ptr, cudaEnableDefault, &q) == cudaSuccess &&
        q == cudaDriverEntryPointSuccess)
      fn = reinterpret_cast<EncodeTiledFn>(ptr);
  }
  return fn;
}

inline int make_weight_map(CUtensorMap* map, const float* W, int rows, int cols, const char* who,
                           int box_rows = BN) {
  EncodeTiledFn enc = get_encode_fn();
  if (!enc) { lnb::set_err("%s: cuTensorMapEncodeTiled unavailable", who); return LNB_ERR_UNSUPPORTED; }
  cuuint64_t gdim[2] = {(cuuint64_t)cols, (cuuint64_t)rows};
  cuuint64_t gstride[1] = {(cuuint64_t)cols * sizeof(float)};
  cuuint32_t box[2] = {(cuuint32_t)BK, (cuuint32_t)box_rows};
  cuuint32_t estr[2] = {1, 1};
  CUresult r = enc(map, CU_TENSOR_MAP_DATA_TYPE_FLOAT32, 2, const_cast<float*>(W), gdim, gstride,
                   box, estr, CU_TENSOR_MAP_INTERLEAVE_NONE, CU_TENSOR_MAP_SWIZZLE_128B,
                   CU_TENSOR_MAP_L2_PROMOTION_L2_256B, CU_TENSOR_MAP_FLOAT_OOB_FILL_NONE);
  if (r != CUDA_SUCCESS) {
    lnb::set_err("%s: cuTensorMapEncodeTiled failed (CUresult %d)", who, (int)r);
    return LNB_ERR_ARG;
  }
  return LNB_OK;
}

inline int debug_flags() {
  const char* e = getenv("LNB_DBG");
  return e ? atoi(e) : 0;
}

inline int sm_count() {
  int dev = 0, n = 148;
  if (cudaGetDevice(&dev) == cudaSuccess)
    cudaDeviceGetAttribute(&n, cudaDevAttrMultiProcessorCount, dev);
  return n > 0 ? n : 148;
}

}
```

lanczosnetwork_b200/model/_common.py:

```python
import os

import torch
import torch.nn as nn

from .. import _lib, ops
from ..data import check_dist
from ..spectral_conv import (GraphContext, WeightCache, graph_conv_layer,
                             ritz_filter_coefficients)


class Ragged(object):

  def __init__(self, tensor, capacity=None, bucket=4096):
    self.tensor = tensor
    rows = int(tensor.shape[0])
    self.capacity = int(capacity) if capacity is not None else max(bucket, -(-rows // bucket) * bucket)
    if rows > self.capacity:
      raise ValueError('Ragged: %d rows exceed the capacity %d' % (rows, self.capacity))

  @property
  def rows(self):
    return int(self.tensor.shape[0])

  def static_shape(self):
    return (self.capacity,) + tuple(self.tensor.shape[1:])


def _raw(t):
  return t.tensor if isinstance(t, Ragged) else t


def _opt(obj, name, default):
  return getattr(obj, name) if hasattr(obj, name) else default


class SpectralNetBase(nn.Module):

  def _setup_common(self, config, num_edgetype, filter_mlp_in, filter_mlp_hidden):
    m = config.model
    self.config = config
    self.input_dim = m.input_dim
    self.hidden_dim = m.hidden_dim
    self.output_dim = m.output_dim
    self.num_layer = m.num_layer
    self.num_edgetype = num_edgetype
    self.dropout = _opt(m, 'dropout', 0.0)
    self.short_diffusion_dist = check_dist(m.short_diffusion_dist)
    self.long_diffusion_dist = check_dist(m.long_diffusion_dist)
    self.max_short_diffusion_dist = max(self.short_diffusion_dist) if self.short_diffusion_dist else None
    self.max_long_diffusion_dist = max(self.long_diffusion_dist) if self.long_diffusion_dist else None
    self.num_scale_short = len(self.short_diffusion_dist)
    self.num_scale_long = len(self.long_diffusion_dist)
    self.num_eig_vec = m.num_eig_vec
    self.spectral_filter_kind = m.spectral_filter_kind
    self._filter_mlp_dims = (filter_mlp_in, filter_mlp_hidden)
    self._wcache = WeightCache()

  def _build_layers(self):
    C = self.num_scale_short + self.num_scale_long + self.num_edgetype + 1
    dims = [self.input_dim] + list(self.hidden_dim) + [self.output_dim]
    self.filter = nn.ModuleList(
        [nn.Linear(dims[t] * C, dims[t + 1]) for t in range(self.num_layer)] +
        [nn.Linear(dims[-2], dims[-1])])
    return dims

  def _build_spectral_filter(self):
    if self.spectral_filter_kind == 'MLP' and self.num_scale_long > 0:
      n_in, hid = self._filter_mlp_dims
      self.spectral_filter = nn.ModuleList([
          nn.Sequential(nn.Linear(n_in, hid), nn.ReLU(), nn.Linear(hid, hid), nn.ReLU(),
                        nn.Linear(hid, hid), nn.ReLU(), nn.Linear(hid, n_in))
          for _ in range(self.num_layer)
      ])

  def _build_head(self, dims):
    self.att_func = nn.Sequential(nn.Linear(dims[-2], 1), nn.Sigmoid())
    loss = self.config.model.loss
    if loss == 'CrossEntropy':
      self.loss_func = torch.nn.CrossEntropyLoss()
    elif loss == 'MSE':
      self.loss_func = torch.nn.MSELoss()
    elif loss == 'L1':
      self.loss_func = torch.nn.L1Loss()
    else:
      raise ValueError("Non-supported loss function!")

  def _init_param(self):
    groups = [self.filter, self.att_func]
    if hasattr(self, 'spectral_filter'):
      groups += list(self.spectral_filter)
    for grp in groups:
      for mod in grp:
        if isinstance(mod, nn.Linear):
          nn.init.xavier_uniform_(mod.weight.data)
          if mod.bias is not None:
            mod.bias.data.zero_()

  def _device(self):
    dev = self.filter[0].weight.device
    if dev.type != 'cuda':
      raise RuntimeError(
          '%s runs on CUDA (sm_100a) only -- move the module with .cuda(); there is no CPU '
          'fallback (the CPU reference is the oracle).' % type(self).__name__)
    if getattr(self, '_is_replica', False) and hasattr(self, '_wcache') and not self._wcache.bypass:
      self._wcache = type(self._wcache)()
      self._wcache.bypass = True
    return dev

  def invalidate_caches(self):
    if hasattr(self, '_wcache'):
      self._wcache.invalidate()
    for name in ('_graphs', '_graphs_resident', '_resident_seen'):
      self.__dict__.pop(name, None)

  def graph_stats(self):
    st = self.__dict__.setdefault('_graph_stats', {'captures': 0, 'replays': 0})
    return dict(st, live=len(self.__dict__.get('_graphs', {})),
                live_resident=len(self.__dict__.get('_graphs_resident', {})))

  def _has_trainable_parameters(self):
    for m in self.modules():
      for group in (m._parameters, getattr(m, '_former_parameters', None) or {}):
        for p in group.values():
          if p is not None and p.requires_grad:
            return True
    return False

  def _check_mode(self):
    if torch.is_grad_enabled() and self._has_trainable_parameters():
      if not hasattr(self, '_train_impl'):
        raise NotImplementedError(
            '%s has no training path in this build: call it under torch.no_grad() (as '
            'runner.test() / the validation loop do).' % type(self).__name__)
      return True
    if self.training and self.dropout > 0.0:
      raise NotImplementedError('dropout > 0 in training mode needs autograd enabled (the inference '
                                'kernels implement eval() semantics)')
    return False

  @staticmethod
  def _to(dev, t, dtype=None):
    if t is None:
      return None
    if t.device != dev:
      t = t.to(dev, non_blocking=True)
    if dtype is not None and t.dtype != dtype:
      t = t.to(dtype)
    return t

  use_cuda_graph = os.environ.get('LNB_NO_GRAPH', '0') != '1'

  def _param_signature(self):
    return tuple((p.data_ptr(), p._version) for p in self.parameters())

  def _graph_forward(self, impl, inputs, extra_key=()):
    dev = self._device()
    eligible = (self.use_cuda_graph and not self.training and not torch.is_grad_enabled() and
                not getattr(self, '_is_replica', False) and
                not torch.cuda.is_current_stream_capturing())
    if not eligible:
      return impl(*[self._to(dev, _raw(t)) for t in inputs])
    key = (dev.index,) + tuple(extra_key) + tuple(
        None if t is None else ((t.static_shape(), t.tensor.dtype, 'ragged') if isinstance(t, Ragged)
                                else (tuple(t.shape), t.dtype)) for t in inputs)
    cache = self.__dict__.setdefault('_graphs', {})
    stats = self.__dict__.setdefault('_graph_stats', {'captures': 0, 'replays': 0})
    entry = cache.get(key)
    if entry is not None:
      cache[key] = cache.pop(key)
    sig = self._param_signature()
    cur = torch.cuda.current_stream(dev)
    raw = [_raw(t) for t in inputs]
    if all(t is None or (t.is_cuda and t.device == dev and t.is_contiguous()) for t in raw):
      pkey = key + tuple(None if t is None else t.data_ptr() for t in raw)
      zc = self.__dict__.setdefault('_graphs_resident', {})
      hit = zc.get(pkey)
      if hit is not None and hit['sig'] == sig:
        zc[pkey] = zc.pop(pkey)
        stats['replays'] += 1
        hit['graph'].replay()
        _lib.note_graph_replay(hit['kernels'])
        return hit['out'].clone()
      seen = self.__dict__.setdefault('_resident_seen', {})
      if len(seen) > 256:
        seen.clear()
      seen[pkey] = seen.get(pkey, 0) + 1
      if seen[pkey] >= 2 and entry is not None and entry['sig'] == sig:
        if len(zc) >= 16:
          zc.pop(next(iter(zc)))
        if '_resident_pool' not in self.__dict__:
          self._resident_pool = torch.cuda.graph_pool_handle()
        torch.cuda.synchronize(dev)
        graph = torch.cuda.CUDAGraph()
        n0 = int(_lib.load().lnb_launch_count())
        with torch.cuda.graph(graph, pool=self._resident_pool):
          out = impl(*raw)
        hit = {'graph': graph, 'out': out, 'sig': sig,
               'kernels': int(_lib.load().lnb_launch_count()) - n0}
        zc[pkey] = hit
        stats['captures'] += 1
        graph.replay()
        _lib.note_graph_replay(hit['kernels'])
        return out.clone()
    if entry is None or entry['sig'] != sig:
      slots = []
      for _ in range(2):
        static_in = [None if t is None else
                     (torch.zeros(t.static_shape(), dtype=t.tensor.dtype, device=dev)
                      if isinstance(t, Ragged) else torch.empty(t.shape, dtype=t.dtype, device=dev))
                     for t in inputs]
        for s_, t in zip(static_in, inputs):
          if isinstance(t, Ragged):
            s_[:t.rows].copy_(t.tensor, non_blocking=True)
          elif s_ is not None:
            s_.copy_(t, non_blocking=True)
        if not slots:
          side = torch.cuda.Stream(device=dev)
          side.wait_stream(cur)
          with torch.cuda.stream(side):
            impl(*static_in)
          cur.wait_stream(side)
        torch.cuda.synchronize(dev)
        graph = torch.cuda.CUDAGraph()
        n0 = int(_lib.load().lnb_launch_count())
        with torch.cuda.graph(graph):
          static_out = impl(*static_in)
        slots.append({'graph': graph, 'in': static_in, 'out': static_out,
                      'kernels': int(_lib.load().lnb_launch_count()) - n0,
                      'free': torch.cuda.Event(), 'ready': torch.cuda.Event()})
        slots[-1]['free'].record(cur)
      entry = {'sig': sig, 'slots': slots, 'next': 0, 'copy': torch.cuda.Stream(device=dev)}
      stats['captures'] += 1
      cache.pop(key, None)
      if len(cache) >= 8:
        cache.pop(next(iter(cache)))
      cache[key] = entry
    slot = entry['slots'][entry['next']]
    entry['next'] ^= 1
    copy = entry['copy']
    copy.wait_event(slot['free'])
    if any(t is not None and t.is_cuda for t in raw):
      copy.wait_stream(cur)
    with torch.cuda.stream(copy):
      for s_, t in zip(slot['in'], inputs):
        if isinstance(t, Ragged):
          s_[:t.rows].copy_(t.tensor, non_blocking=True)
        elif s_ is not None:
          s_.copy_(t, non_blocking=True)
      slot['ready'].record(copy)
    cur.wait_event(slot['ready'])
    stats['replays'] += 1
    slot['graph'].replay()
    slot['free'].record(cur)
    _lib.note_graph_replay(slot['kernels'])
    return slot['out'].clone()

  def _filter_mlp_params(self):
    if not hasattr(self, 'spectral_filter'):
      return None
    out = []
    for l, seq in enumerate(self.spectral_filter):
      out.append([('spectral_filter.%d.%d' % (l, i), seq[i].weight, seq[i].bias)
                  for i in (0, 2, 4, 6)])
    return out

  def _ritz_conv_stack(self, state, node_ids, L, D, V, mask, prep=None, dims_hint=None):
    S, nl = self.num_scale_long, self.num_layer
    if L is not None:
      N, K, E1 = L.shape[1], V.shape[2], L.shape[3]
    else:
      (N, E1), K = dims_hint, V.shape[2]
    din0 = self.embedding.weight.shape[1] if node_ids is not None else state.shape[2]
    dims = [din0] + list(self.hidden_dim)
    ok = [ops.fused_conv_supported(N, dims[t], K, dims[t + 1], len(self.short_diffusion_dist),
                                   False, S, E1) for t in range(nl)]
    H = dims[1]
    uniform = all(d == H for d in dims[1:])
    first = 0
    while first < nl and not ok[first]:
      first += 1
    stack_ok = uniform and first < nl and all(ok[first:]) and nl - first <= 8
    binarize = getattr(self, '_binarize_operators', False)
    if binarize and not (stack_ok and first == 0):
      L = (L != 0).to(L.dtype)
      binarize = False
    if L is None and not (stack_ok and first == 0):
      raise RuntimeError('sparse batches without the dense operators need every layer on the fused '
                         'stack kernel; call ops.graph_prepare_sparse(..., want_dense=True)')
    ctx = GraphContext(L, V, binarize)
    if prep is not None:
      ctx._prep = prep
    coeffs = table = None
    if S > 0:
      mlp = self._filter_mlp_params() if self.spectral_filter_kind == 'MLP' else None
      cur = torch.cuda.current_stream(D.device)
      side = self.__dict__.setdefault('_side_streams', {}).get(D.device.index)
      if side is None:
        side = self._side_streams[D.device.index] = torch.cuda.Stream(device=D.device)
      side.wait_stream(cur)
      with torch.cuda.stream(side):
        table = ops.ritz_power_table(D, self.long_diffusion_dist)
      table.record_stream(cur)
      gext = ctx.prep() if (mlp is not None and stack_ok and first == 0) else None
      cur.wait_stream(side)
      coeffs, table = ritz_filter_coefficients(D, self.long_diffusion_dist, mlp, self._wcache, gext,
                                               table=table)

    def layer_coeff(t):
      if S == 0:
        return None
      return coeffs[t] if coeffs is not None else table

    if node_ids is not None and not (stack_ok and first == 0):
      state = ops.embedding_rows(node_ids, self.embedding.weight)
    for t in range(first if stack_ok else nl):
      state = graph_conv_layer(state, ctx, layer_coeff(t), False, self.short_diffusion_dist, S,
                               self.filter[t].weight, self.filter[t].bias, self._wcache,
                               'filter.%d' % t, last=(t == nl - 1),
                               next_fused=(t + 1 < nl and ok[t + 1]))
    if not stack_ok:
      return self._readout(state, mask)
    layers = list(range(first, nl))
    kw = (S + E1) * max(dims[t] for t in layers)
    w_hi, w_lo, bias = self._wcache.split_conv_stack(
        'filter.stack.%d' % first, [self.filter[t].weight for t in layers],
        [self.filter[t].bias for t in layers], kw)
    if S == 0:
      coeff, stride = None, 0
    elif coeffs is not None:
      coeff, stride = coeffs[first], coeffs.stride(0)
    else:
      coeff, stride = table, 0
    head, att = self.filter[nl], self.att_func[0]
    if head.weight.shape[0] > 48:
      state, _ = ops.spectral_stack_forward(
          ctx.prep(), V, w_hi, w_lo, bias, [dims[t] for t in layers], H, S, coeff=coeff,
          coeff_stride=stride, X=None if (node_ids is not None and first == 0) else state,
          node_ids=node_ids if first == 0 else None,
          emb=self.embedding.weight if (node_ids is not None and first == 0) else None,
          want_state=True)
      return self._readout(state, mask)
    _, score = ops.spectral_stack_forward(
        ctx.prep(), V, w_hi, w_lo, bias, [dims[t] for t in layers], H, S, coeff=coeff,
        coeff_stride=stride, X=None if (node_ids is not None and first == 0) else state,
        node_ids=node_ids if first == 0 else None,
        emb=self.embedding.weight if (node_ids is not None and first == 0) else None,
        readout=(head.weight, head.bias, att.weight.reshape(-1), att.bias), mask=mask)
    return score

  def _sparse_stack_ok(self, N, E1, K):
    S = self.num_scale_long
    din0 = self.embedding.weight.shape[1]
    dims = [din0] + list(self.hidden_dim)
    ok = all(ops.fused_conv_supported(N, dims[t], K, dims[t + 1], len(self.short_diffusion_dist), False, S, E1)
             for t in range(self.num_layer))
    return ok and all(d == dims[1] for d in dims[1:]) and self.num_layer <= 8

  def _readout(self, state, mask):
    head = self.filter[self.num_layer]
    att = self.att_func[0]
    return ops.readout(state, head.weight, head.bias, att.weight.reshape(-1), att.bias, mask)

  def _finish(self, score, label):
    if label is not None:
      return score, self.loss_func(score, label)
    return score
```

lanczosnetwork_b200/ops.py:

```python
import ctypes

import torch

from . import _lib
from ._lib import GemmDesc, SpectralStack

__all__ = [
    'bgemm', 'split_tf32', 'linear_tf32x3', 'linear_tf32x3_grouped', 'graph_prepare', 'spectral_conv_fused',
    'graph_prepare_sparse', 'graph_prepare_sparse_packed', 'fused_conv_supported', 'spectral_stack_forward', 'ritz_rowmap', 'ritz_filter_mlp', 'embedding_rows', 'ritz_power_table', 'readout',
    'operator_chain', 'operator_chain_supported', 'graph_messages', 'graph_messages_supported', 'gaussian_laplacian', 'lanczos_tridiag', 'lanczos_ritz', 'tridiag_ritz', 'tridiag_powers',
    'symmetrize_filters', 'segment_sum_forward', 'segment_sum_backward', 'launch_count',
]


def _need_cuda(*tensors):
  for t in tensors:
    if t is None:
      continue
    if not t.is_cuda:
      raise RuntimeError('lanczosnetwork_b200 ops run on CUDA (sm_100a) only; got a %s tensor. '
                         'There is no CPU fallback.' % t.device)


def _f32c(t):
  if t.dtype != torch.float32:
    t = t.float()
  return t.contiguous()


def _ptr(t):
  return ctypes.c_void_p(t.data_ptr()) if t is not None else ctypes.c_void_p(0)


def _stream(t):
  return ctypes.c_void_p(torch.cuda.current_stream(t.device).cuda_stream)


def _ints(vals):
  arr = (ctypes.c_int * len(vals))(*[int(v) for v in vals])
  return arr


def launch_count():
  return _lib.launch_count()


def bgemm(A, a_str, Bm, b_str, C, c_str, batch, nz, M, N, K, kscale=None, s_str=(0, 0, 0),
          bias=None, bias_sz=0, relu=False, a_off=0, b_off=0, c_off=0, alpha=1.0, addend=None,
          add_str=(0, 0, 0, 0), add_off=0, beta=0.0):
  _need_cuda(A, Bm, C, kscale, bias)
  lib = _lib.load()
  d = GemmDesc()
  d.A = A.data_ptr() + 4 * a_off
  d.a_sb, d.a_sz, d.a_sm, d.a_sk = [int(v) for v in a_str]
  d.B = Bm.data_ptr() + 4 * b_off
  d.b_sb, d.b_sz, d.b_sk, d.b_sn = [int(v) for v in b_str]
  d.C = C.data_ptr() + 4 * c_off
  d.c_sb, d.c_sz, d.c_sm, d.c_sn = [int(v) for v in c_str]
  d.kscale = kscale.data_ptr() if kscale is not None else None
  d.s_sb, d.s_sz, d.s_sk = [int(v) for v in s_str]
  d.bias = bias.data_ptr() if bias is not None else None
  d.bias_sz = int(bias_sz)
  d.batch, d.nz, d.M, d.N, d.K, d.relu = int(batch), int(nz), int(M), int(N), int(K), int(bool(relu))
  d.alpha, d.beta = float(alpha), float(beta)
  d.addend = addend.data_ptr() + 4 * add_off if addend is not None else None
  d.d_sb, d.d_sz, d.d_sm, d.d_sn = [int(v) for v in add_str]
  with torch.cuda.device(C.device):
    _lib.check(lib.lnb_batched_gemm(_stream(C), ctypes.byref(d)), 'lnb_batched_gemm')
  return C


def split_tf32(x):
  _need_cuda(x)
  x = _f32c(x)
  hi = torch.empty_like(x)
  lo = torch.empty_like(x)
  with torch.cuda.device(x.device):
    _lib.check(_lib.load().lnb_split_tf32(_stream(x), _ptr(x), x.numel(), _ptr(hi), _ptr(lo)),
               'lnb_split_tf32')
  return hi, lo


def linear_tf32x3(x, w_hi, w_lo, bias=None, relu=False, out=None):
  _need_cuda(x, w_hi, w_lo, bias)
  x = _f32c(x)
  M, K = x.shape
  N = w_hi.shape[0]
  if out is None:
    out = torch.empty((M, N), device=x.device, dtype=torch.float32)
  tiles = ((M + 127) // 128) * ((N + 127) // 128)
  nkb = (K + 31) // 32
  splits = 1
  if tiles * 2 <= _sm_count(x.device) and nkb >= 32:
    splits = min(_sm_count(x.device) // tiles, 8, nkb // 16)
    while splits > 1 and ((nkb + splits - 1) // splits) * (splits - 1) >= nkb:
      splits -= 1
  with torch.cuda.device(x.device):
    if splits > 1:
      ws, counters = _splitk_workspace(x.device, tiles * splits * 128 * 128, tiles)
      _lib.check(_lib.load().lnb_linear_tf32x3_splitk(
          _stream(x), _ptr(x), _ptr(w_hi), _ptr(w_lo), _ptr(bias), M, N, K, int(bool(relu)),
          _ptr(out), splits, _ptr(ws), _ptr(counters)), 'lnb_linear_tf32x3_splitk')
    else:
      _lib.check(_lib.load().lnb_linear_tf32x3(_stream(x), _ptr(x), _ptr(w_hi), _ptr(w_lo),
                                               _ptr(bias), M, N, K, int(bool(relu)), _ptr(out)),
                 'lnb_linear_tf32x3')
  return out


_SPLITK_WS = {}
_SM_COUNT = {}


def _sm_count(device):
  idx = device.index if device.index is not None else torch.cuda.current_device()
  if idx not in _SM_COUNT:
    _SM_COUNT[idx] = torch.cuda.get_device_properties(idx).multi_processor_count
  return _SM_COUNT[idx]


def _splitk_workspace(device, nfloats, ntiles):
  key = (device.index, torch.cuda.current_stream(device).cuda_stream)
  ws, counters = _SPLITK_WS.get(key, (None, None))
  if ws is None or ws.numel() < nfloats or counters.numel() < ntiles:
    ws = torch.empty((max(nfloats, ws.numel() if ws is not None else 0),), device=device,
                     dtype=torch.float32)
    counters = torch.zeros((max(ntiles, 256),), device=device, dtype=torch.int32)
    _SPLITK_WS[key] = (ws, counters)
  return ws, counters


def linear_tf32x3_grouped(x, w_hi, w_lo, bias, groups, relu=False):
  _need_cuda(x, w_hi, w_lo, bias)
  x = _f32c(x)
  M = x.shape[0]
  K = w_hi.shape[1]
  N = w_hi.shape[0] // groups
  assert x.shape[1] == groups * K and w_hi.shape[0] == groups * N
  out = torch.empty((M, groups * N), device=x.device, dtype=torch.float32)
  with torch.cuda.device(x.device):
    _lib.check(_lib.load().lnb_linear_tf32x3_grouped(_stream(x), _ptr(x), _ptr(w_hi), _ptr(w_lo),
                                                     _ptr(bias), M, groups, N, K,
                                                     int(bool(relu)), _ptr(out)),
               'lnb_linear_tf32x3_grouped')
  return out


class GraphPrep(tuple):
  rowmap = None
  nrows = None


def graph_prepare(L, Q, binarize=False):
  _need_cuda(L, Q)
  L, Q = _f32c(L), _f32c(Q)
  B, N, _, E1 = L.shape
  K = Q.shape[2]
  dev = L.device
  ell_val = torch.empty((B, E1, N, N), device=dev, dtype=torch.float32)
  ell_idx = torch.empty((B, E1, N, N), device=dev, dtype=torch.uint8)
  ell_max = torch.empty((B, E1), device=dev, dtype=torch.int32)
  gext = torch.empty((B, 2), device=dev, dtype=torch.int32)
  tiles = torch.empty((4 * B + 2,), device=dev, dtype=torch.int32)
  rowmap = torch.empty((B * K,), device=dev, dtype=torch.int32)
  nrows = torch.empty((1,), device=dev, dtype=torch.int32)
  with torch.cuda.device(dev):
    _lib.check(_lib.load().lnb_graph_prepare(_stream(L), _ptr(L), _ptr(Q), B, N, E1, K,
                                             _ptr(ell_val), _ptr(ell_idx), _ptr(ell_max),
                                             _ptr(gext), _ptr(tiles), _ptr(rowmap), _ptr(nrows),
                                             1 if binarize else 0),
               'lnb_graph_prepare')
  prep = GraphPrep((ell_val, ell_idx, ell_max, gext, tiles))
  prep.rowmap, prep.nrows = rowmap, nrows
  return prep


_INV_SQRT_DEG = {}


def _inv_sqrt_deg_table(device):
  key = device.index if device.index is not None else torch.cuda.current_device()
  if key not in _INV_SQRT_DEG:
    import numpy as np
    deg = np.arange(256, dtype=np.float64)
    with np.errstate(divide='ignore'):
      t = np.power(deg, -0.5)
    t[np.isinf(t)] = 0.0
    _INV_SQRT_DEG[key] = torch.from_numpy(t).to(device)
  return _INV_SQRT_DEG[key]


def graph_prepare_sparse(sizes, node_ptr, node_feat, edge_ptr, edges, V_rows, N, E1, binarize=False,
                         want_dense=False):
  _need_cuda(sizes, node_ptr, node_feat, edge_ptr, edges, V_rows)
  dev = sizes.device
  B = sizes.shape[0]
  K = V_rows.shape[1]
  assert sizes.dtype == torch.int32 and node_ptr.dtype == torch.int32 and node_feat.dtype == torch.int32
  assert edge_ptr.dtype == torch.int32 and edges.dtype == torch.uint8 and edges.shape[1] == 4
  assert V_rows.dtype == torch.float32 and V_rows.is_contiguous() and edges.is_contiguous()
  ell_val = torch.empty((B, E1, N, N), device=dev, dtype=torch.float32)
  ell_idx = torch.empty((B, E1, N, N), device=dev, dtype=torch.uint8)
  ell_max = torch.empty((B, E1), device=dev, dtype=torch.int32)
  gext = torch.empty((B, 2), device=dev, dtype=torch.int32)
  tiles = torch.empty((4 * B + 2,), device=dev, dtype=torch.int32)
  rowmap = torch.empty((B * K,), device=dev, dtype=torch.int32)
  nrows = torch.empty((1,), device=dev, dtype=torch.int32)
  node_ids = torch.empty((B, N), device=dev, dtype=torch.int64)
  mask = torch.empty((B, N), device=dev, dtype=torch.uint8)
  V = torch.empty((B, N, K), device=dev, dtype=torch.float32)
  L = torch.empty((B, N, N, E1), device=dev, dtype=torch.float32) if want_dense else None
  with torch.cuda.device(dev):
    _lib.check(_lib.load().lnb_graph_prepare_sparse(
        _stream(sizes), _ptr(sizes), _ptr(node_ptr), _ptr(node_feat), _ptr(edge_ptr), _ptr(edges),
        _ptr(V_rows), _ptr(_inv_sqrt_deg_table(dev)), B, int(N), int(E1), int(K),
        1 if binarize else 0, _ptr(ell_val), _ptr(ell_idx), _ptr(ell_max), _ptr(gext), _ptr(tiles),
        _ptr(rowmap), _ptr(nrows), _ptr(node_ids), _ptr(mask), _ptr(V), _ptr(L)),
               'lnb_graph_prepare_sparse')
  prep = GraphPrep((ell_val, ell_idx, ell_max, gext, tiles))
  prep.rowmap, prep.nrows = rowmap, nrows
  return prep, node_ids, mask, V, L


def graph_prepare_sparse_packed(blob, B, N, E1, K, binarize=False, want_dense=False, host_tiles=True):
  _need_cuda(blob)
  assert blob.dtype == torch.uint8 and blob.is_contiguous()
  dev = blob.device
  ell_val = torch.empty((B, E1, N, N), device=dev, dtype=torch.float32)
  ell_idx = torch.empty((B, E1, N, N), device=dev, dtype=torch.uint8)
  ell_max = torch.empty((B, E1), device=dev, dtype=torch.int32)
  gext = torch.empty((B, 2), device=dev, dtype=torch.int32)
  if host_tiles:
    from .data import packed_offsets
    off_tiles = packed_offsets(B, K)[5]
    tiles = blob[off_tiles:off_tiles + 4 * (B + 2)].view(torch.int32)
  else:
    tiles = torch.empty((4 * B + 2,), device=dev, dtype=torch.int32)
  rowmap = torch.empty((B * K,), device=dev, dtype=torch.int32)
  nrows = torch.empty((1,), device=dev, dtype=torch.int32)
  node_ids = torch.empty((B, N), device=dev, dtype=torch.int64)
  mask = torch.empty((B, N), device=dev, dtype=torch.uint8)
  V = torch.empty((B, N, K), device=dev, dtype=torch.float32)
  L = torch.empty((B, N, N, E1), device=dev, dtype=torch.float32) if want_dense else None
  with torch.cuda.device(dev):
    _lib.check(_lib.load().lnb_graph_prepare_sparse_packed(
        _stream(blob), _ptr(blob), _ptr(_inv_sqrt_deg_table(dev)), int(B), int(N), int(E1), int(K),
        (1 if binarize else 0) | (2 if host_tiles else 0), _ptr(ell_val), _ptr(ell_idx), _ptr(ell_max), _ptr(gext), _ptr(tiles),
        _ptr(rowmap), _ptr(nrows), _ptr(node_ids), _ptr(mask), _ptr(V), _ptr(L)),
               'lnb_graph_prepare_sparse_packed')
  prep = GraphPrep((ell_val, ell_idx, ell_max, gext, tiles))
  prep.rowmap, prep.nrows = rowmap, nrows
  return prep, node_ids, mask, V, L


def fused_conv_supported(N, Din, K, H, n_short, dense_filter, S=8, E1=7):
  if (n_short or dense_filter or N > 128 or Din % 32 or K > 32 or K % 4 or H % 4 or H > 128 or
      E1 > 16):
    return False
  smem = 2 * 32768 + 256 + 1024 + 2 * 128 * (max(Din, H) + 4) * 4 + 128 * K * 4 + 4096
  return smem <= 227 * 1024


def spectral_conv_fused(X, Q, coeff, prep, w_hi, w_lo, bias, relu=True, write_pad=True):
  _need_cuda(X, Q, coeff, w_hi, w_lo, bias)
  X, Q = _f32c(X), _f32c(Q)
  ell_val, ell_idx, ell_max, gext, tiles = prep
  B, N, Din = X.shape
  K = Q.shape[2]
  S = 0
  if coeff is not None:
    coeff = _f32c(coeff)
    S = coeff.shape[2]
  E1 = ell_val.shape[1]
  H = w_hi.shape[0]
  assert w_hi.shape[1] == (S + E1) * Din, (w_hi.shape, S, E1, Din)
  out = torch.empty((B, N, H), device=X.device, dtype=torch.float32)
  with torch.cuda.device(X.device):
    _lib.check(_lib.load().lnb_spectral_conv_fused(
        _stream(X), _ptr(X), _ptr(Q), _ptr(coeff), _ptr(ell_val), _ptr(ell_idx), _ptr(ell_max),
        _ptr(gext), _ptr(tiles), _ptr(w_hi), _ptr(w_lo), _ptr(bias), B, N, Din, E1, K, S, H,
        int(bool(relu)), int(bool(write_pad)), _ptr(out)), 'lnb_spectral_conv_fused')
  return out


def spectral_stack_forward(prep, Q, w_hi, w_lo, bias, dins, H, S, coeff=None, coeff_stride=0,
                           X=None, node_ids=None, emb=None, want_state=False, write_pad=True,
                           readout=None, mask=None, relu=True):
  ell_val, ell_idx, ell_max, gext, tiles = prep
  _need_cuda(Q, w_hi, w_lo, bias, coeff, X, node_ids, emb, mask)
  Q = _f32c(Q)
  B, N, K = Q.shape
  E1 = ell_val.shape[1]
  dev = Q.device
  d = SpectralStack()
  if X is not None:
    X = _f32c(X)
    d.X = X.data_ptr()
  else:
    node_ids = node_ids.contiguous().long()
    emb = _f32c(emb)
    d.node_ids, d.emb_table, d.emb_rows = node_ids.data_ptr(), emb.data_ptr(), emb.shape[0]
  d.Q = Q.data_ptr()
  if coeff is not None:
    d.coeff, d.coeff_layer_stride = coeff.data_ptr(), int(coeff_stride)
  d.ell_val, d.ell_idx, d.ell_max = ell_val.data_ptr(), ell_idx.data_ptr(), ell_max.data_ptr()
  d.gext, d.tiles = gext.data_ptr(), tiles.data_ptr()
  d.W_hi, d.W_lo = w_hi.data_ptr(), w_lo.data_ptr()
  d.bias = bias.data_ptr() if bias is not None else None
  state = score = None
  if want_state or readout is None:
    state = torch.empty((B, N, H), device=dev, dtype=torch.float32)
    d.out_state = state.data_ptr()
  keep = []
  if readout is not None:
    W_out, b_out, w_att, b_att = [_f32c(t) for t in readout]
    keep += [W_out, b_out, w_att, b_att]
    score = torch.empty((B, W_out.shape[0]), device=dev, dtype=torch.float32)
    d.W_out, d.b_out, d.w_att, d.b_att = (W_out.data_ptr(), b_out.data_ptr(), w_att.data_ptr(),
                                          b_att.data_ptr())
    d.score, d.P = score.data_ptr(), W_out.shape[0]
    if mask is not None:
      if mask.dtype != torch.uint8:
        mask = (mask != 0).to(torch.uint8)
      mask = mask.contiguous()
      d.mask = mask.data_ptr()
  for i, v in enumerate(dins):
    d.Din[i] = int(v)
  d.num_layers, d.Kw, d.write_pad = len(dins), int(w_hi.shape[1]), int(bool(write_pad))
  d.B, d.N, d.E1, d.K, d.S, d.H, d.relu = B, N, E1, K, int(S), int(H), int(bool(relu))
  with torch.cuda.device(dev):
    _lib.check(_lib.load().lnb_spectral_stack_forward(_stream(Q), ctypes.byref(d)),
               'lnb_spectral_stack_forward')
  return state, score


def ritz_rowmap(gext, K):
  _need_cuda(gext)
  B = gext.shape[0]
  rowmap = torch.empty((B * K,), device=gext.device, dtype=torch.int32)
  nrows = torch.empty((1,), device=gext.device, dtype=torch.int32)
  with torch.cuda.device(gext.device):
    _lib.check(_lib.load().lnb_ritz_rowmap(_stream(gext), _ptr(gext), B, int(K), _ptr(rowmap),
                                           _ptr(nrows)), 'lnb_ritz_rowmap')
  return rowmap, nrows


def ritz_filter_mlp(table, w_hi, w_lo, bias_all, num_layers, rowmap=None, nrows=None):
  _need_cuda(table, w_hi, w_lo, bias_all, rowmap, nrows)
  table = _f32c(table)
  R, S = table.shape
  Hd = w_hi.shape[1]
  coeff = torch.empty((num_layers, R, S), device=table.device, dtype=torch.float32)
  with torch.cuda.device(table.device):
    _lib.check(_lib.load().lnb_ritz_filter_mlp(_stream(table), _ptr(table), _ptr(rowmap),
                                               _ptr(nrows), _ptr(w_hi), _ptr(w_lo),
                                               _ptr(bias_all), R, int(num_layers), S, Hd,
                                               _ptr(coeff)), 'lnb_ritz_filter_mlp')
  return coeff


def embedding_rows(idx, table):
  _need_cuda(idx, table)
  idx = idx.contiguous().long()
  table = _f32c(table)
  rows = idx.numel()
  out = torch.empty(tuple(idx.shape) + (table.shape[1],), device=table.device, dtype=torch.float32)
  with torch.cuda.device(table.device):
    _lib.check(_lib.load().lnb_embedding_rows(_stream(table), _ptr(idx), _ptr(table), rows,
                                              table.shape[0], table.shape[1], _ptr(out)),
               'lnb_embedding_rows')
  return out


def ritz_power_table(D, powers):
  _need_cuda(D)
  D = _f32c(D)
  S = len(powers)
  out = torch.empty(tuple(D.shape) + (S,), device=D.device, dtype=torch.float32)
  with torch.cuda.device(D.device):
    _lib.check(_lib.load().lnb_ritz_power_table(_stream(D), _ptr(D), D.numel(), _ints(powers), S,
                                                _ptr(out)), 'lnb_ritz_power_table')
  return out


def readout(state, W_out, b_out, w_att, b_att, mask=None):
  _need_cuda(state, W_out, b_out, w_att, b_att, mask)
  state = _f32c(state)
  B, N, H = state.shape
  P = W_out.shape[0]
  if mask is not None:
    mask = (mask != 0).to(torch.uint8).contiguous()
  out = torch.empty((B, P), device=state.device, dtype=torch.float32)
  with torch.cuda.device(state.device):
    _lib.check(_lib.load().lnb_readout(_stream(state), _ptr(state), _ptr(_f32c(W_out)),
                                       _ptr(_f32c(b_out)), _ptr(_f32c(w_att)), _ptr(_f32c(b_att)),
                                       _ptr(mask), B, N, H, P, _ptr(out)), 'lnb_readout')
  return out


def operator_chain_supported(N, steps):
  return N <= 32 and steps <= 64


def operator_chain(L, X, steps, block_of_step, out, out_col0, chebyshev=False):
  _need_cuda(L, X, out)
  L, X = _f32c(L), _f32c(X)
  B, N, D = X.shape
  E1 = L.shape[3]
  assert out.dtype == torch.float32 and out.is_contiguous() and out.shape[:2] == (B, N)
  sel = (ctypes.c_int * steps)(*[int(v) for v in block_of_step])
  with torch.cuda.device(X.device):
    _lib.check(_lib.load().lnb_operator_chain(_stream(X), _ptr(L), _ptr(X), B, N, E1, D, int(steps),
                                              1 if chebyshev else 0, sel, _ptr(out),
                                              out.stride(0), out.stride(1), int(out_col0)),
               'lnb_operator_chain')
  return out


def graph_messages_supported(N, K, E1, S, max_short):
  return N <= 32 and (S == 0 or K <= 32) and E1 <= 16 and S <= 8 and max_short <= 64


def graph_messages(L, X, Q, filt, dense_filter, short_dist, out):
  _need_cuda(L, X, Q, filt, out)
  L, X = _f32c(L), _f32c(X)
  B, N, D = X.shape
  E1 = L.shape[3]
  S = K = 0
  if filt is not None:
    filt, Q = _f32c(filt), _f32c(Q)
    K = Q.shape[2]
    S = filt.shape[1] if dense_filter else filt.shape[2]
  steps = sorted(short_dist)
  max_short = max(steps) if steps else 0
  sel = [steps.index(s) if s in steps else -1 for s in range(1, max_short + 1)]
  arr = (ctypes.c_int * max(1, max_short))(*([int(v) for v in sel] or [0]))
  assert out.dtype == torch.float32 and out.is_contiguous()
  with torch.cuda.device(X.device):
    _lib.check(_lib.load().lnb_graph_messages(
        _stream(X), _ptr(L), _ptr(X), _ptr(Q), _ptr(filt), B, N, E1, D, K, S,
        1 if dense_filter else 0, max_short, arr, len(steps), _ptr(out), out.stride(0), out.stride(1)),
               'lnb_graph_messages')
  return out


def gaussian_laplacian(x, L):
  _need_cuda(x, L)
  x, L = _f32c(x), _f32c(L)
  B, N, Dx = x.shape
  E1 = L.shape[3]
  out = torch.empty((B, N, N), device=x.device, dtype=torch.float32)
  with torch.cuda.device(x.device):
    _lib.check(_lib.load().lnb_gaussian_laplacian(_stream(x), _ptr(x), _ptr(L), B, N, Dx, E1,
                                                  _ptr(out)), 'lnb_gaussian_laplacian')
  return out


def lanczos_tridiag(A, mask, q1, K):
  _need_cuda(A, mask, q1)
  A = _f32c(A)
  B, N = A.shape[0], A.shape[1]
  q1 = _f32c(q1).reshape(B, N)
  if mask is not None:
    mask = (mask != 0).to(torch.uint8).contiguous()
  dev = A.device
  T = torch.empty((B, K, K), device=dev, dtype=torch.float32)
  Q = torch.empty((B, N, K), device=dev, dtype=torch.float32)
  alpha = torch.empty((B, K), device=dev, dtype=torch.float32)
  beta = torch.empty((B, K), device=dev, dtype=torch.float32)
  idx = torch.empty((B,), device=dev, dtype=torch.int32)
  with torch.cuda.device(dev):
    _lib.check(_lib.load().lnb_lanczos_tridiag(_stream(A), _ptr(A), _ptr(mask), _ptr(q1), B, N, K,
                                               _ptr(T), _ptr(Q), _ptr(alpha), _ptr(beta),
                                               _ptr(idx)), 'lnb_lanczos_tridiag')
  return {'T': T, 'Q': Q, 'alpha': alpha, 'beta': beta, 'idx': idx}


def tridiag_ritz(alpha, beta, Q):
  _need_cuda(alpha, beta, Q)
  alpha, beta, Q = _f32c(alpha), _f32c(beta), _f32c(Q)
  B, N, K = Q.shape
  theta = torch.empty((B, K), device=Q.device, dtype=torch.float32)
  V = torch.empty((B, N, K), device=Q.device, dtype=torch.float32)
  status = torch.empty((B,), device=Q.device, dtype=torch.int32)
  with torch.cuda.device(Q.device):
    _lib.check(_lib.load().lnb_tridiag_ritz(_stream(Q), _ptr(alpha), _ptr(beta), _ptr(Q), B, N, K,
                                            _ptr(theta), _ptr(V), _ptr(status)), 'lnb_tridiag_ritz')
  return theta, V, status


def lanczos_ritz(A, mask, q1, K, want_ritz=True, want_T=True, want_Q=True, proper=False):
  _need_cuda(A, mask, q1)
  A = _f32c(A)
  B, N = A.shape[0], A.shape[1]
  q1 = _f32c(q1).reshape(B, N)
  if mask is not None:
    mask = (mask != 0).to(torch.uint8).contiguous()
  dev = A.device
  out = {'alpha': torch.empty((B, K), device=dev, dtype=torch.float32),
         'beta': torch.empty((B, K), device=dev, dtype=torch.float32),
         'idx': torch.empty((B,), device=dev, dtype=torch.int32)}
  if want_T:
    out['T'] = torch.empty((B, K, K), device=dev, dtype=torch.float32)
  if want_Q:
    out['Q'] = torch.empty((B, N, K), device=dev, dtype=torch.float32)
  if want_ritz:
    out['theta'] = torch.empty((B, K), device=dev, dtype=torch.float32)
    out['V'] = torch.empty((B, N, K), device=dev, dtype=torch.float32)
    out['status'] = torch.empty((B,), device=dev, dtype=torch.int32)
  with torch.cuda.device(dev):
    _lib.check(_lib.load().lnb_lanczos_ritz(
        _stream(A), _ptr(A), _ptr(mask), _ptr(q1), B, N, K, 1 if proper else 0,
        _ptr(out.get('T')), _ptr(out.get('Q')),
        _ptr(out['alpha']), _ptr(out['beta']), _ptr(out['idx']), _ptr(out.get('theta')),
        _ptr(out.get('V')), _ptr(out.get('status'))), 'lnb_lanczos_ritz')
  return out


def tridiag_powers(T, powers):
  _need_cuda(T)
  T = _f32c(T)
  B, K = T.shape[0], T.shape[1]
  S = len(powers)
  out = torch.empty((B, K, S, K), device=T.device, dtype=torch.float32)
  with torch.cuda.device(T.device):
    _lib.check(_lib.load().lnb_tridiag_powers(_stream(T), _ptr(T), B, K, _ints(powers), S,
                                              _ptr(out)), 'lnb_tridiag_powers')
  return out


def symmetrize_filters(Y, K, S):
  _need_cuda(Y)
  Y = _f32c(Y)
  B = Y.shape[0]
  G = torch.empty((B, S, K, K), device=Y.device, dtype=torch.float32)
  with torch.cuda.device(Y.device):
    _lib.check(_lib.load().lnb_symmetrize_filters(_stream(Y), _ptr(Y), B, K, S, _ptr(G)),
               'lnb_symmetrize_filters')
  return G


def segment_sum_forward(data, segment_index, num_segments, output=None):
  _need_cuda(data, segment_index, output)
  data = _f32c(data)
  seg = segment_index.contiguous().long()
  B, d1, d2 = data.shape
  if output is None:
    output = torch.zeros((B, num_segments, d2), device=data.device, dtype=torch.float32)
  with torch.cuda.device(data.device):
    _lib.check(_lib.load().lnb_unsorted_segment_sum_forward(
        _stream(data), _ptr(data), _ptr(seg), _ints([B, d1, d2]), int(num_segments), _ptr(output)),
               'lnb_unsorted_segment_sum_forward')
  return output


def segment_sum_backward(grad_output, segment_index, data_shape, grad_data=None):
  _need_cuda(grad_output, segment_index, grad_data)
  grad_output = _f32c(grad_output)
  seg = segment_index.contiguous().long()
  B, d1, d2 = [int(v) for v in data_shape]
  if grad_data is None:
    grad_data = torch.empty((B, d1, d2), device=grad_output.device, dtype=torch.float32)
  with torch.cuda.device(grad_output.device):
    _lib.check(_lib.load().lnb_unsorted_segment_sum_backward(
        _stream(grad_output), _ptr(grad_output), _ptr(seg), _ints([B, d1, d2]),
        int(grad_output.shape[1]), _ptr(grad_data)), 'lnb_unsorted_segment_sum_backward')
  return grad_data
```

lanczosnetwork_b200/spectral_conv.py:

```python
import torch

from . import ops

__all__ = ['WeightCache', 'GraphContext', 'dense', 'graph_conv_layer', 'graph_conv_layer_unfused',
           'ritz_filter_coefficients']


class WeightCache(object):

  def __init__(self):
    import threading
    self._store = {}
    self._lock = threading.Lock()
    self.bypass = False

  def _get(self, key, tag, build, sources):
    if self.bypass:
      return build()
    with self._lock:
      hit = self._store.get(key)
    if hit is None or hit[0] != tag:
      hit = (tag,) + tuple(build()) + (tuple(sources),)
      with self._lock:
        self._store[key] = hit
    return hit[1:-1]

  def invalidate(self):
    with self._lock:
      self._store.clear()

  def split(self, name, weight, pad_to=None):
    def build():
      w = weight.detach()
      if pad_to is not None and pad_to != w.shape[1]:
        w = torch.nn.functional.pad(w, (0, pad_to - w.shape[1]))
      return ops.split_tf32(w)
    return self._get((name, weight.device.index), (weight.data_ptr(), weight._version, pad_to), build,
                     [weight])

  def split_stacked(self, name, weights, biases):
    dev = weights[0].device
    tag = tuple((w.data_ptr(), w._version) for w in list(weights) + list(biases))

    def build():
      hi, lo = ops.split_tf32(torch.cat([w.detach() for w in weights], dim=0))
      return hi, lo, torch.cat([b.detach() for b in biases], dim=0).contiguous()
    return self._get((name, dev.index), tag, build, list(weights) + list(biases))

  def split_mlp_chain(self, name, mlp_layers):
    ws = [w for layer in mlp_layers for (_, w, _) in layer]
    bs = [b for layer in mlp_layers for (_, _, b) in layer]
    tag = tuple((t.data_ptr(), t._version) for t in ws + bs)

    def build():
      hd = ws[1].shape[0]
      rows = []
      for layer in mlp_layers:
        w0 = layer[0][1].detach()
        rows.append(torch.nn.functional.pad(w0, (0, hd - w0.shape[1])))
        rows += [layer[1][1].detach(), layer[2][1].detach(), layer[3][1].detach()]
      hi, lo = ops.split_tf32(torch.cat(rows, dim=0).contiguous())
      return hi, lo, torch.cat([b.detach() for b in bs], dim=0).contiguous()
    return self._get((name, ws[0].device.index), tag, build, ws + bs)

  def split_conv_stack(self, name, weights, biases, kw):
    tag = tuple((t.data_ptr(), t._version) for t in list(weights) + list(biases)) + (kw,)

    def build():
      rows = [torch.nn.functional.pad(w.detach(), (0, kw - w.shape[1])) for w in weights]
      hi, lo = ops.split_tf32(torch.cat(rows, dim=0).contiguous())
      return hi, lo, torch.cat([b.detach() for b in biases], dim=0).contiguous()
    return self._get((name, weights[0].device.index), tag, build, list(weights) + list(biases))

  def clear(self):
    self.invalidate()


def dense(x2d, weight, bias, relu, cache, name):
  M, K = x2d.shape
  N = weight.shape[0]
  if K % 4 == 0:
    w_hi, w_lo = cache.split(name, weight, K)
    return ops.linear_tf32x3(x2d, w_hi, w_lo, bias, relu)
  assert K == weight.shape[1]
  out = torch.empty((M, N), device=x2d.device, dtype=torch.float32)
  w = weight.detach().contiguous()
  ops.bgemm(x2d, (0, 0, K, 1), w, (0, 0, 1, K), out, (0, 0, N, 1), 1, 1, M, N, K,
            bias=bias, relu=relu)
  return out


def ritz_filter_coefficients(D, powers, mlp_layers, cache, gext=None, table=None):
  B, K = D.shape
  S = len(powers)
  if table is None:
    table = ops.ritz_power_table(D, powers)
  if mlp_layers is None:
    return None, table
  nl = len(mlp_layers)
  flat = table.reshape(B * K, S)
  hd = mlp_layers[0][0][1].shape[0]
  if S <= 32 and hd % 32 == 0 and hd <= 128:
    w_hi, w_lo, bias_all = cache.split_mlp_chain('spectral_filter.chain', mlp_layers)
    rowmap = nrows = None
    if isinstance(gext, ops.GraphPrep):
      rowmap, nrows = gext.rowmap, gext.nrows
    elif gext is not None:
      rowmap, nrows = ops.ritz_rowmap(gext, K)
    coeff = ops.ritz_filter_mlp(flat, w_hi, w_lo, bias_all, nl, rowmap, nrows).reshape(nl, B, K, S)
    return coeff, table
  if S % 4 == 0 and hd % 4 == 0:
    h = flat
    for stage in range(4):
      ws = [mlp_layers[l][stage][1] for l in range(nl)]
      bs = [mlp_layers[l][stage][2] for l in range(nl)]
      w_hi, w_lo, bias = cache.split_stacked('spectral_filter.*.%d' % (2 * stage), ws, bs)
      if stage == 0:
        h = ops.linear_tf32x3(h, w_hi, w_lo, bias, True)
      else:
        h = ops.linear_tf32x3_grouped(h, w_hi, w_lo, bias, nl, stage < 3)
    coeff = h.reshape(B, K, nl, S).permute(2, 0, 1, 3).contiguous()
    return coeff, table
  out = []
  for params in mlp_layers:
    h = flat
    for i, (name, w, b) in enumerate(params):
      h = dense(h, w, b, i < len(params) - 1, cache, name)
    out.append(h.reshape(B, K, S))
  return torch.stack(out, dim=0), table


class GraphContext(object):

  def __init__(self, L, Qv, binarize=False):
    self.L = L
    self.Qv = Qv
    self.binarize = binarize
    self._prep = None

  def prep(self):
    if self._prep is None:
      self._prep = ops.graph_prepare(self.L, self.Qv, self.binarize)
    return self._prep


def graph_conv_layer(state, ctx, coeff, dense_filter, short_dist, num_long, weight, bias, cache,
                     name, last=True, next_fused=False):
  L, Qv = ctx.L, ctx.Qv
  B, N, Din = state.shape
  if (num_long > 0 and Qv is not None and
      ops.fused_conv_supported(N, Din, Qv.shape[2], weight.shape[0], len(short_dist), dense_filter,
                               num_long, L.shape[3])):
    w_hi, w_lo = cache.split(name, weight)
    return ops.spectral_conv_fused(state, Qv, coeff, ctx.prep(), w_hi, w_lo, bias, True,
                                   write_pad=last or not next_fused)
  return graph_conv_layer_unfused(state, L, Qv, coeff, dense_filter, short_dist, num_long, weight,
                                  bias, cache, name)


def graph_conv_layer_unfused(state, L, Qv, coeff, dense_filter, short_dist, num_long, weight, bias,
                             cache, name):
  B, N, Din = state.shape
  E1 = L.shape[3]
  S = num_long
  n_short = len(short_dist)
  C = n_short + S + E1
  CD = (C * Din + 3) // 4 * 4
  dev = state.device
  if CD != C * Din:
    msg = torch.zeros((B, N, CD), device=dev, dtype=torch.float32)
  else:
    msg = torch.empty((B, N, CD), device=dev, dtype=torch.float32)
  if ops.graph_messages_supported(N, Qv.shape[2] if (S and Qv is not None) else 0, E1, S,
                                  max(short_dist) if n_short else 0):
    ops.graph_messages(L, state, Qv if S else None, coeff if S else None, dense_filter, short_dist, msg)
    out = dense(msg.reshape(B * N, CD), weight, bias, True, cache, name)
    return out.reshape(B, N, -1)
  x_str = (N * Din, 0, Din, 1)
  col = 0
  if n_short and ops.operator_chain_supported(N, max(short_dist)):
    steps = sorted(short_dist)
    sel = [steps.index(s) if s in steps else -1 for s in range(1, max(short_dist) + 1)]
    ops.operator_chain(L, state, max(short_dist), sel, msg, 0)
    col = n_short
  elif n_short:
    l0_str = (N * N * E1, 0, N * E1, E1)
    src, src_str, src_off = state, x_str, 0
    tmp = None
    for step in range(1, max(short_dist) + 1):
      if step in short_dist:
        dst, dst_str, dst_off = msg, (N * CD, 0, CD, 1), col * Din
        col += 1
      else:
        tmp = torch.empty((B, N, Din), device=dev, dtype=torch.float32)
        dst, dst_str, dst_off = tmp, x_str, 0
      ops.bgemm(L, l0_str, src, src_str, dst, dst_str, B, 1, N, Din, N, b_off=src_off,
                c_off=dst_off)
      src, src_off = dst, dst_off
      src_str = (dst_str[0], 0, dst_str[2], 1)
  if S:
    K = Qv.shape[2]
    U = torch.empty((B, K, Din), device=dev, dtype=torch.float32)
    ops.bgemm(Qv, (N * K, 0, 1, K), state, x_str, U, (K * Din, 0, Din, 1), B, 1, K, Din, N)
    if dense_filter:
      W = torch.empty((B, S, K, Din), device=dev, dtype=torch.float32)
      ops.bgemm(coeff, (S * K * K, K * K, K, 1), U, (K * Din, 0, Din, 1), W,
                (S * K * Din, K * Din, Din, 1), B, S, K, Din, K)
      ops.bgemm(Qv, (N * K, 0, K, 1), W, (S * K * Din, K * Din, Din, 1), msg,
                (N * CD, Din, CD, 1), B, S, N, Din, K, c_off=col * Din)
    else:
      ops.bgemm(Qv, (N * K, 0, K, 1), U, (K * Din, 0, Din, 1), msg, (N * CD, Din, CD, 1),
                B, S, N, Din, K, kscale=coeff, s_str=(K * S, 1, S), c_off=col * Din)
    col += S
  ops.bgemm(L, (N * N * E1, 1, N * E1, E1), state, x_str, msg, (N * CD, Din, CD, 1),
            B, E1, N, Din, N, c_off=col * Din)
  out = dense(msg.reshape(B * N, CD), weight, bias, True, cache, name)
  return out.reshape(B, N, -1)
```

Measured before the change: 2.069 million.

## Switch fused spectral conv GEMM to scaled split-FP16 operands with dynamic exponents

Weights are pre-split into scaled hi/lo FP16 halves with per-row, per-block power-of-two exponents, and cached. The fused kernel computes running magnitude bounds for the activation side (Ritz projections, edge operator row norms, layer outputs) so it can pick per-row scale exponents and feed FP16 tensor-core MMAs instead of TF32x3. Half-size operands let the pipeline deepen from 2 to 3 B stages in less shared memory. In exchange it adds extra reductions and atomics in the producer path, and accuracy depends on the scaling bounds keeping values inside FP16 range.

```diff
diff --git a/include/lanczosnet_b200.h b/include/lanczosnet_b200.h
--- a/include/lanczosnet_b200.h
+++ b/include/lanczosnet_b200.h
@@ -52,9 +52,14 @@
                       int32_t* tiles, int32_t* rowmap, int32_t* nrows, int flags);
 int lnb_spectral_conv_fused(lnb_stream_t stream, const float* X, const float* Q, const float* coeff,
                             const float* ell_val, const uint8_t* ell_idx, const int32_t* ell_max,
-                            const int32_t* gext, const int32_t* tiles, const float* W_hi,
-                            const float* W_lo, const float* bias, int B, int N, int Din, int E1,
-                            int K, int S, int H, int relu, int write_pad, float* out);
+                            const int32_t* gext, const int32_t* tiles, const uint16_t* W_hi16,
+                            const uint16_t* W_lo16, const int32_t* w_exp, const float* bias, int B,
+                            int N, int Din, int E1, int K, int S, int H, int relu, int write_pad,
+                            float* out);
+
+int lnb_split_f16_scaled(lnb_stream_t stream, const float* w_hi, const float* w_lo, int rows, int cols,
+                         int rows_per_block, const int32_t* step_cols , uint16_t* hi16,
+                         uint16_t* lo16, int32_t* w_exp);
 
 int lnb_graph_prepare_sparse(lnb_stream_t stream, const int32_t* sizes, const int32_t* node_ptr,
                              const int32_t* node_feat, const int32_t* edge_ptr, const uint8_t* edges,
@@ -75,7 +80,7 @@
   const float* Q; const float* coeff; int64_t coeff_layer_stride;
   const float* ell_val; const uint8_t* ell_idx; const int32_t* ell_max; const int32_t* gext;
   const int32_t* tiles;
-  const float* W_hi; const float* W_lo; const float* bias;
+  const uint16_t* W_hi16; const uint16_t* W_lo16; const int32_t* w_exp; const float* bias;
   float* out_state;
   const float* W_out; const float* b_out; const float* w_att; const float* b_att;
   const uint8_t* mask; float* score;
diff --git a/lanczosnetwork_b200/_lib.py b/lanczosnetwork_b200/_lib.py
--- a/lanczosnetwork_b200/_lib.py
+++ b/lanczosnetwork_b200/_lib.py
@@ -31,7 +31,8 @@
       ('Q', ctypes.c_void_p), ('coeff', ctypes.c_void_p), ('coeff_layer_stride', c_i64),
       ('ell_val', ctypes.c_void_p), ('ell_idx', ctypes.c_void_p), ('ell_max', ctypes.c_void_p),
       ('gext', ctypes.c_void_p), ('tiles', ctypes.c_void_p),
-      ('W_hi', ctypes.c_void_p), ('W_lo', ctypes.c_void_p), ('bias', ctypes.c_void_p),
+      ('W_hi16', ctypes.c_void_p), ('W_lo16', ctypes.c_void_p), ('w_exp', ctypes.c_void_p),
+      ('bias', ctypes.c_void_p),
       ('out_state', ctypes.c_void_p),
       ('W_out', ctypes.c_void_p), ('b_out', ctypes.c_void_p), ('w_att', ctypes.c_void_p),
       ('b_att', ctypes.c_void_p), ('mask', ctypes.c_void_p), ('score', ctypes.c_void_p),
@@ -69,8 +70,10 @@
                                         [ctypes.c_void_p] * 11),
     'lnb_spectral_conv_fused':
         (c_int, [c_stream, c_f32p, c_f32p, c_f32p, c_f32p, ctypes.c_void_p, ctypes.c_void_p,
-                 ctypes.c_void_p, ctypes.c_void_p, c_f32p, c_f32p, c_f32p, c_int, c_int, c_int,
-                 c_int, c_int, c_int, c_int, c_int, c_int, c_f32p]),
+                 ctypes.c_void_p, ctypes.c_void_p, ctypes.c_void_p, ctypes.c_void_p, ctypes.c_void_p,
+                 c_f32p, c_int, c_int, c_int, c_int, c_int, c_int, c_int, c_int, c_int, c_f32p]),
+    'lnb_split_f16_scaled': (c_int, [c_stream, c_f32p, c_f32p, c_int, c_int, c_int, ctypes.POINTER(c_int),
+                                     ctypes.c_void_p, ctypes.c_void_p, ctypes.c_void_p]),
     'lnb_spectral_stack_forward': (c_int, [c_stream, ctypes.POINTER(SpectralStack)]),
     'lnb_ritz_rowmap': (c_int, [c_stream, ctypes.c_void_p, c_int, c_int, ctypes.c_void_p, ctypes.c_void_p]),
     'lnb_ritz_filter_mlp': (c_int, [c_stream, c_f32p, ctypes.c_void_p, ctypes.c_void_p, c_f32p, c_f32p,
diff --git a/lanczosnetwork_b200/csrc/linear_tf32x3.cu b/lanczosnetwork_b200/csrc/linear_tf32x3.cu
--- a/lanczosnetwork_b200/csrc/linear_tf32x3.cu
+++ b/lanczosnetwork_b200/csrc/linear_tf32x3.cu
@@ -3,6 +3,7 @@
 namespace {
 
 struct RowLoadPolicy {
+  static constexpr bool kF16 = false;
   static constexpr int kStagesB = 6;
   struct Params {
     const float* A;
diff --git a/lanczosnetwork_b200/csrc/spectral_conv_fused.cu b/lanczosnetwork_b200/csrc/spectral_conv_fused.cu
--- a/lanczosnetwork_b200/csrc/spectral_conv_fused.cu
+++ b/lanczosnetwork_b200/csrc/spectral_conv_fused.cu
@@ -1,4 +1,5 @@
 #include "tc_gemm.cuh"
+#include <cuda_fp16.h>
 
 namespace {
 
@@ -215,7 +216,8 @@
 }
 
 struct SpectralPolicy {
-  static constexpr int kStagesB = 2;
+  static constexpr bool kF16 = true;
+  static constexpr int kStagesB = 3;
   static constexpr int LMAX = 8;
   struct Params {
     const float* X;
@@ -229,6 +231,7 @@
     const int32_t* ell_max;
     const int32_t* gext;
     const int32_t* tiles;
+    const int32_t* w_exp;
     const float* bias;
     float* out;
     const float* W_out;
@@ -273,6 +276,9 @@
     uint8_t row_g[RMAX], row_n[RMAX], z_g[RMAX], z_k[RMAX];
     uint8_t q_g[RMAX / 4 + GMAX], q_n0[RMAX / 4 + GMAX];
     uint8_t line_e[256], line_t[256];
+    float lnorm[RMAX];
+    uint32_t umax[RMAX];
+    uint32_t xmax[2][GMAX];
   };
 
   const Params& p;
@@ -286,6 +292,7 @@
   float* Ev;
   uint8_t* Ei;
   float fr[FR];
+  int sig = 0;
   tcg::PhaseTimer* ptm = nullptr;
 
   static __host__ __device__ constexpr size_t tables_bytes() { return (sizeof(Tables) + 15) & ~size_t(15); }
@@ -348,6 +355,8 @@
       }
     }
     __syncwarp();
+    tb->xmax[0][lane] = 0u;
+    tb->xmax[1][lane] = 0u;
     if (lane == 0) {
       tb->gs = gs; tb->ng = ng; tb->Rtot = Rtot; tb->Ztot = Ztot; tb->nquads = nquads;
       tb->nbase[ng] = Rtot; tb->kbase[ng] = Ztot;
@@ -365,7 +374,11 @@
   __device__ void step_begin(int m_tile, int sub, int , tcg::PhaseTimer& tm) {
     tcg::producers_sync();
     const int layer = sub >> 1, step = sub & 1;
-    if (step == 1 && S > 0) return;
+    if (step == 1 && S > 0) {
+      edge_step_scale(layer);
+      return;
+    }
+    if (r == tid) tb->umax[r] = 0u;
     Din = p.Din[layer];
     const int warp = tid >> 5, lane = tid & 31;
     constexpr int NW = tcg::PRODUCER_THREADS / 32;
@@ -449,7 +462,12 @@
     tc05::cp_async_wait_all();
     tcg::producers_sync();
     tm.lap(1);
-    if (S == 0) return;
+    if (layer == 0) stage_bounds();
+    if (S == 0) {
+      tcg::producers_sync();
+      edge_step_scale(layer);
+      return;
+    }
     for (int task = tid; task < (Ztot >> 2) * dv; task += tcg::PRODUCER_THREADS) {
       const int dq = task % dv, zq = task / dv;
       const int g = tb->z_g[4 * zq], k0 = tb->z_k[4 * zq];
@@ -472,14 +490,77 @@
 #pragma unroll
           for (int j = 0; j < 4; ++j) acc[i][j] = fmaf(qv[i], xv[j], acc[i][j]);
       }
-#pragma unroll
-      for (int i = 0; i < 4; ++i)
+      const unsigned peers = __match_any_sync(__activemask(), zq);
+      const bool leader = (tid & 31) == __ffs(peers) - 1;
+#pragma unroll
+      for (int i = 0; i < 4; ++i) {
         *reinterpret_cast<float4*>(UZ + (size_t)(4 * zq + i) * XP + 4 * dq) =
             make_float4(acc[i][0], acc[i][1], acc[i][2], acc[i][3]);
+        uint32_t m = max(max(__float_as_uint(fabsf(acc[i][0])), __float_as_uint(fabsf(acc[i][1]))),
+                         max(__float_as_uint(fabsf(acc[i][2])), __float_as_uint(fabsf(acc[i][3]))));
+        m = __reduce_max_sync(peers, m);
+        if (leader) atomicMax(&tb->umax[4 * zq + i], m);
+      }
     }
     tcg::producers_sync();
     tm.lap(2);
-  }
+    float fm = 0.f;
+    if (r < Ztot) {
+      if (S <= FR) {
+#pragma unroll
+        for (int i = 0; i < FR; ++i) fm = fmaxf(fm, fabsf(fr[i]));
+      } else {
+        const int g = tb->z_g[r], k = tb->z_k[r];
+        if (k < tb->gk[g]) {
+          const float* f = p.coeff + layer * p.coeff_stride + ((int64_t)(gs + g) * K + k) * S;
+          uint32_t b = 0u;
+          for (int i = 0; i < S; ++i) b = max(b, __float_as_uint(fabsf(__ldg(f + i))));
+          fm = __uint_as_float(b);
+        }
+      }
+    }
+    sig = tc05::f16_scale_exp(fm * __uint_as_float(tb->umax[r]));
+  }
+
+  __device__ void stage_bounds() {
+    const int warp = tid >> 5, lane = tid & 31;
+    constexpr int NW = tcg::PRODUCER_THREADS / 32;
+    const int Rtot = tb->Rtot;
+    if (r == tid) {
+      float best = 0.f;
+      if (r < Rtot) {
+        const int g = tb->row_g[r], n = tb->row_n[r];
+        for (int e = 0; e < E1; ++e) {
+          const float* ev = Ev + (size_t)tb->base_e[e] * RMAX + r;
+          float sum = 0.f;
+          for (int t = 0; t < tb->cnt_e[e]; ++t) sum += fabsf(ev[t * RMAX]);
+          const int64_t off0 = (((int64_t)(tb->gs + g) * E1 + e) * N) * N + n;
+          for (int t = tb->cnt_e[e]; t < tb->emax[g][e]; ++t) sum += fabsf(__ldg(p.ell_val + off0 + (int64_t)t * N));
+          best = fmaxf(best, sum);
+        }
+      }
+      tb->lnorm[r] = best;
+    }
+    for (int row = warp; row < Rtot; row += NW) {
+      const float* xr = Xs + (size_t)row * XP;
+      uint32_t m = 0u;
+      for (int d = lane; d < Din; d += 32) m = max(m, __float_as_uint(fabsf(xr[d])));
+#pragma unroll
+      for (int o = 16; o > 0; o >>= 1) m = max(m, __shfl_xor_sync(0xffffffffu, m, o));
+      if (lane == 0) atomicMax(&tb->xmax[0][tb->row_g[row]], m);
+    }
+  }
+
+  __device__ void edge_step_scale(int layer) {
+    if (tid < GMAX) tb->xmax[(layer + 1) & 1][tid] = 0u;
+    float bound = 0.f;
+    if (r < tb->Rtot) bound = tb->lnorm[r] * __uint_as_float(tb->xmax[layer & 1][tb->row_g[r]]);
+    sig = tc05::f16_scale_exp(bound);
+  }
+
+  __device__ __forceinline__ int row_exp(int ) const { return sig; }
+  __device__ __forceinline__ const int32_t* col_exp(int sub) const { return p.w_exp + (size_t)sub * H; }
+  __device__ __forceinline__ int out_cols() const { return H; }
 
   __device__ __forceinline__ void produce(int sub, int kb, float (&v)[32]) {
 #pragma unroll
@@ -610,6 +691,7 @@
     float4* o4 = reinterpret_cast<float4*>(Xs + (size_t)r * XP + col);
     const bool relu = p.relu != 0;
     const float* bias = p.bias ? p.bias + (sub >> 1) * H : nullptr;
+    uint32_t m = 0u;
 #pragma unroll
     for (int q = 0; q < tcg::EW / 4; ++q) {
       float y[4] = {x[4 * q + 0], x[4 * q + 1], x[4 * q + 2], x[4 * q + 3]};
@@ -634,6 +716,15 @@
         }
       }
       o4[q] = make_float4(y[0], y[1], y[2], y[3]);
+      if (col + 4 * q < H)
+        m = max(m, max(max(__float_as_uint(fabsf(y[0])), __float_as_uint(fabsf(y[1]))),
+                       max(__float_as_uint(fabsf(y[2])), __float_as_uint(fabsf(y[3])))));
+    }
+    if ((sub >> 1) + 1 < p.L) {
+      const int g = tb->row_g[r];
+      const unsigned peers = __match_any_sync(__activemask(), g);
+      m = __reduce_max_sync(peers, m);
+      if ((tid & 31) == __ffs(peers) - 1) atomicMax(&tb->xmax[((sub >> 1) + 1) & 1][g], m);
     }
   }
 
@@ -755,6 +846,46 @@
   }
 };
 
+struct SplitCols { int c[SpectralPolicy::LMAX]; };
+
+__global__ void __launch_bounds__(128)
+split_f16_scaled_kernel(const float* __restrict__ w_hi, const float* __restrict__ w_lo, int cols,
+                        int rows_per_block, SplitCols sc, __half* __restrict__ hi16,
+                        __half* __restrict__ lo16, int32_t* __restrict__ w_exp) {
+  __shared__ uint32_t red[2][4];
+  const int row = blockIdx.x, tid = threadIdx.x;
+  const int blk = row / rows_per_block, n = row - blk * rows_per_block;
+  const int c1 = sc.c[blk];
+  const float* a = w_hi + (int64_t)row * cols;
+  const float* b = w_lo + (int64_t)row * cols;
+  uint32_t m0 = 0u, m1 = 0u;
+  for (int c = tid; c < cols; c += 128) {
+    const uint32_t u = __float_as_uint(fabsf(__ldg(a + c) + __ldg(b + c)));
+    if (c < c1) m0 = max(m0, u); else m1 = max(m1, u);
+  }
+#pragma unroll
+  for (int o = 16; o > 0; o >>= 1) {
+    m0 = max(m0, __shfl_xor_sync(0xffffffffu, m0, o));
+    m1 = max(m1, __shfl_xor_sync(0xffffffffu, m1, o));
+  }
+  if ((tid & 31) == 0) { red[0][tid >> 5] = m0; red[1][tid >> 5] = m1; }
+  __syncthreads();
+  m0 = max(max(red[0][0], red[0][1]), max(red[0][2], red[0][3]));
+  m1 = max(max(red[1][0], red[1][1]), max(red[1][2], red[1][3]));
+  const int e0 = tc05::f16_scale_exp(__uint_as_float(m0)), e1 = tc05::f16_scale_exp(__uint_as_float(m1));
+  if (tid == 0) {
+    w_exp[(int64_t)(2 * blk) * rows_per_block + n] = e0;
+    w_exp[(int64_t)(2 * blk + 1) * rows_per_block + n] = e1;
+  }
+  const float s0 = tc05::exp2i(e0), s1 = tc05::exp2i(e1);
+  for (int c = tid; c < cols; c += 128) {
+    const float x = (__ldg(a + c) + __ldg(b + c)) * (c < c1 ? s0 : s1);
+    const __half h = __float2half_rn(x);
+    hi16[(int64_t)row * cols + c] = h;
+    lo16[(int64_t)row * cols + c] = __float2half_rn(x - __half2float(h));
+  }
+}
+
 }
 
 namespace lnb {
@@ -808,7 +939,7 @@
 
 static int launch_stack(lnb_stream_t stream, const lnb_spectral_stack& d, const char* who) {
   LNB_REQUIRE((d.X || (d.node_ids && d.emb_table)) && d.Q && d.ell_val && d.ell_idx && d.ell_max &&
-                  d.gext && d.tiles && d.W_hi && d.W_lo && (d.out_state || d.score) &&
+                  d.gext && d.tiles && d.W_hi16 && d.W_lo16 && d.w_exp && (d.out_state || d.score) &&
                   (d.coeff || d.S == 0),
               "%s: null pointer", who);
   LNB_REQUIRE(d.B >= 0 && d.N >= 1 && d.E1 >= 1 && d.K >= 1 && d.S >= 0 && d.H >= 1 &&
@@ -835,7 +966,8 @@
     return LNB_ERR_ARG;
   }
   if (d.B == 0) return LNB_OK;
-  size_t smem = tcg::core_smem(SpectralPolicy::kStagesB) + 1024 + SpectralPolicy::smem_fixed(dmax, d.K, d.H);
+  size_t smem = tcg::core_smem(SpectralPolicy::kStagesB, SpectralPolicy::kF16) + 1024 +
+                SpectralPolicy::smem_fixed(dmax, d.K, d.H);
   if (smem > 227 * 1024) {
     lnb::set_err("%s: tile state (Din=%d, K=%d, H=%d) needs %zu B of shared memory", who, dmax, d.K,
                  d.H, smem);
@@ -845,9 +977,9 @@
   if (lb > 255) lb = 255;
   smem += (size_t)lb * SpectralPolicy::ell_line_bytes();
   CUtensorMap map_hi, map_lo;
-  int rc = tcg::make_weight_map(&map_hi, d.W_hi, d.num_layers * d.H, d.Kw, who);
+  int rc = tcg::make_weight_map(&map_hi, d.W_hi16, d.num_layers * d.H, d.Kw, who, tcg::BN, true);
   if (rc != LNB_OK) return rc;
-  rc = tcg::make_weight_map(&map_lo, d.W_lo, d.num_layers * d.H, d.Kw, who);
+  rc = tcg::make_weight_map(&map_lo, d.W_lo16, d.num_layers * d.H, d.Kw, who, tcg::BN, true);
   if (rc != LNB_OK) return rc;
   auto kern = tcg::tc_gemm_kernel<SpectralPolicy>;
   cudaFuncSetAttribute(kern, cudaFuncAttributeMaxDynamicSharedMemorySize, (int)smem);
@@ -855,7 +987,7 @@
   p.X = d.X; p.node_ids = d.node_ids; p.emb = d.emb_table; p.Q = d.Q;
   p.coeff = d.coeff; p.coeff_stride = d.coeff_layer_stride;
   p.ell_val = d.ell_val; p.ell_idx = d.ell_idx; p.ell_max = d.ell_max; p.gext = d.gext; p.tiles = d.tiles;
-  p.bias = d.bias; p.out = d.out_state;
+  p.w_exp = d.w_exp; p.bias = d.bias; p.out = d.out_state;
   p.W_out = d.W_out; p.b_out = d.b_out; p.w_att = d.w_att; p.b_att = d.b_att; p.mask = d.mask;
   p.score = d.score; p.P = d.P; p.emb_rows = d.emb_rows; p.L = d.num_layers;
   for (int l = 0; l < d.num_layers; ++l) p.Din[l] = d.Din[l];
@@ -867,6 +999,23 @@
   return lnb::finish_launch(who);
 }
 
+int lnb_split_f16_scaled(lnb_stream_t stream, const float* w_hi, const float* w_lo, int rows, int cols,
+                         int rows_per_block, const int32_t* step_cols, uint16_t* hi16, uint16_t* lo16,
+                         int32_t* w_exp) {
+  LNB_REQUIRE(w_hi && w_lo && step_cols && hi16 && lo16 && w_exp, "split_f16_scaled: null pointer");
+  LNB_REQUIRE(rows >= 0 && cols >= 0 && rows_per_block >= 1 && rows % rows_per_block == 0 &&
+                  rows / rows_per_block <= SpectralPolicy::LMAX,
+              "split_f16_scaled: bad dims rows=%d cols=%d rows_per_block=%d", rows, cols, rows_per_block);
+  if (rows == 0) return LNB_OK;
+  SplitCols sc{};
+  for (int i = 0; i < rows / rows_per_block; ++i) sc.c[i] = step_cols[i];
+  split_f16_scaled_kernel<<<rows, 128, 0, (cudaStream_t)stream>>>(
+      w_hi, w_lo, cols, rows_per_block, sc, reinterpret_cast<__half*>(hi16),
+      reinterpret_cast<__half*>(lo16), w_exp);
+  lnb::count_launch();
+  return lnb::finish_launch("split_f16_scaled");
+}
+
 int lnb_spectral_stack_forward(lnb_stream_t stream, const lnb_spectral_stack* desc) {
   LNB_REQUIRE(desc, "spectral_stack_forward: null descriptor");
   return launch_stack(stream, *desc, "spectral_stack_forward");
@@ -874,13 +1023,14 @@
 
 int lnb_spectral_conv_fused(lnb_stream_t stream, const float* X, const float* Q, const float* coeff,
                             const float* ell_val, const uint8_t* ell_idx, const int32_t* ell_max,
-                            const int32_t* gext, const int32_t* tiles, const float* W_hi,
-                            const float* W_lo, const float* bias, int B, int N, int Din, int E1,
-                            int K, int S, int H, int relu, int write_pad, float* out) {
+                            const int32_t* gext, const int32_t* tiles, const uint16_t* W_hi16,
+                            const uint16_t* W_lo16, const int32_t* w_exp, const float* bias, int B,
+                            int N, int Din, int E1, int K, int S, int H, int relu, int write_pad,
+                            float* out) {
   lnb_spectral_stack d{};
   d.X = X; d.Q = Q; d.coeff = coeff; d.coeff_layer_stride = 0;
   d.ell_val = ell_val; d.ell_idx = ell_idx; d.ell_max = ell_max; d.gext = gext; d.tiles = tiles;
-  d.W_hi = W_hi; d.W_lo = W_lo; d.Kw = (S + E1) * Din; d.bias = bias;
+  d.W_hi16 = W_hi16; d.W_lo16 = W_lo16; d.w_exp = w_exp; d.Kw = (S + E1) * Din; d.bias = bias;
   d.Din[0] = Din; d.num_layers = 1; d.out_state = out; d.write_pad = write_pad;
   d.B = B; d.N = N; d.E1 = E1; d.K = K; d.S = S; d.H = H; d.relu = relu;
   return launch_stack(stream, d, "spectral_conv_fused");
diff --git a/lanczosnetwork_b200/csrc/tc05.cuh b/lanczosnetwork_b200/csrc/tc05.cuh
--- a/lanczosnetwork_b200/csrc/tc05.cuh
+++ b/lanczosnetwork_b200/csrc/tc05.cuh
@@ -119,6 +119,15 @@
       : "r"(taddr)
       : "memory");
 }
+__device__ __forceinline__ void tmem_st_32x16(uint32_t taddr, const uint32_t (&v)[16]) {
+  asm volatile(
+      "tcgen05.st.sync.aligned.32x32b.x16.b32 [%0], "
+      "{%1, %2, %3, %4, %5, %6, %7, %8, %9, %10, %11, %12, %13, %14, %15, %16};"
+      ::"r"(taddr), "r"(v[0]), "r"(v[1]), "r"(v[2]), "r"(v[3]), "r"(v[4]), "r"(v[5]), "r"(v[6]),
+      "r"(v[7]), "r"(v[8]), "r"(v[9]), "r"(v[10]), "r"(v[11]), "r"(v[12]), "r"(v[13]),
+      "r"(v[14]), "r"(v[15])
+      : "memory");
+}
 __device__ __forceinline__ void tmem_st_32x32(uint32_t taddr, const uint32_t (&v)[32]) {
   asm volatile(
       "tcgen05.st.sync.aligned.32x32b.x32.b32 [%0], "
@@ -142,6 +151,21 @@
   return d;
 }
 
+__device__ __forceinline__ uint64_t umma_desc_kmajor_sw64(uint32_t smem_addr) {
+  uint64_t d = 0;
+  d |= (uint64_t)((smem_addr >> 4) & 0x3FFFu);
+  d |= (uint64_t)1 << 16;
+  d |= (uint64_t)32 << 32;
+  d |= (uint64_t)1 << 46;
+  d |= (uint64_t)4 << 61;
+  return d;
+}
+
+__host__ __device__ constexpr uint32_t umma_idesc_f16(int M, int N) {
+  return (1u << 4)
+         | ((uint32_t)(N >> 3) << 17) | ((uint32_t)(M >> 4) << 24);
+}
+
 __host__ __device__ constexpr uint32_t umma_idesc_tf32(int M, int N) {
   return (1u << 4)
          | (2u << 7)
@@ -158,6 +182,15 @@
       ::"r"(d_tmem), "r"(a_tmem), "l"(b_desc), "r"(idesc), "r"(accumulate)
       : "memory");
 }
+__device__ __forceinline__ void umma_f16_ts(uint32_t d_tmem, uint32_t a_tmem, uint64_t b_desc,
+                                            uint32_t idesc, uint32_t accumulate) {
+  asm volatile(
+      "{\n\t.reg .pred p;\n\t"
+      "setp.ne.b32 p, %4, 0;\n\t"
+      "tcgen05.mma.cta_group::1.kind::f16 [%0], [%1], %2, %3, p;\n\t}"
+      ::"r"(d_tmem), "r"(a_tmem), "l"(b_desc), "r"(idesc), "r"(accumulate)
+      : "memory");
+}
 __device__ __forceinline__ void umma_tf32_ss(uint32_t d_tmem, uint64_t a_desc, uint64_t b_desc,
                                              uint32_t idesc, uint32_t accumulate) {
   asm volatile(
@@ -189,4 +222,27 @@
   return r;
 }
 
-}
+__device__ __forceinline__ uint32_t f16x2_rn_bits(float lo, float hi) {
+  uint32_t r;
+  asm("cvt.rn.f16x2.f32 %0, %1, %2;" : "=r"(r) : "f"(hi), "f"(lo));
+  return r;
+}
+__device__ __forceinline__ void f16x2_to_f32(uint32_t h2, float& lo, float& hi) {
+  asm("{\n\t.reg .b16 l, h;\n\t"
+      "mov.b32 {l, h}, %2;\n\t"
+      "cvt.f32.f16 %0, l;\n\t"
+      "cvt.f32.f16 %1, h;\n\t}"
+      : "=f"(lo), "=f"(hi)
+      : "r"(h2));
+}
+
+__device__ __forceinline__ float exp2i(int e) { return __int_as_float((e + 127) << 23); }
+__device__ __forceinline__ int f16_scale_exp(float bound) {
+  const uint32_t bits = __float_as_uint(bound);
+  const int E = (int)((bits >> 23) & 0xFFu);
+  if (E == 0xFF || (bits & 0x7FFFFFFFu) == 0) return 0;
+  const int s = 141 - E;
+  return s < -126 ? -126 : (s > 126 ? 126 : s);
+}
+
+}
diff --git a/lanczosnetwork_b200/csrc/tc_gemm.cuh b/lanczosnetwork_b200/csrc/tc_gemm.cuh
--- a/lanczosnetwork_b200/csrc/tc_gemm.cuh
+++ b/lanczosnetwork_b200/csrc/tc_gemm.cuh
@@ -7,8 +7,10 @@
 
 constexpr int BM = 128, BN = 128, BK = 32;
 constexpr int NGROUPS = 3;
-constexpr int TILE_B_BYTES = BN * BK * 4;
-constexpr int STAGE_B_BYTES = 2 * TILE_B_BYTES;
+__host__ __device__ constexpr int tile_b_bytes(bool f16) { return BN * BK * (f16 ? 2 : 4); }
+__host__ __device__ constexpr int stage_b_bytes(bool f16) { return 2 * tile_b_bytes(f16); }
+constexpr int TILE_B_BYTES = tile_b_bytes(false);
+constexpr int STAGE_B_BYTES = stage_b_bytes(false);
 constexpr int EW = 16;
 constexpr int TMEM_COLS = 512;
 constexpr int COL_MAIN = 0, COL_CORR = 128, COL_A = 256;
@@ -16,7 +18,9 @@
 constexpr int TMA_WARP = 4 * NGROUPS, MMA_WARP = 4 * NGROUPS + 1;
 constexpr int THREADS = PRODUCER_THREADS + 64;
 constexpr int MAX_B_STAGES = 6;
-__host__ __device__ constexpr int core_smem(int stages_b) { return stages_b * STAGE_B_BYTES + 256; }
+__host__ __device__ constexpr int core_smem(int stages_b, bool f16 = false) {
+  return stages_b * stage_b_bytes(f16) + 256;
+}
 
 struct Core {
   uint8_t* Bst;
@@ -29,10 +33,10 @@
   uint32_t* tmem_holder;
 };
 
-__device__ __forceinline__ Core carve(uint8_t* base, int stages_b) {
+__device__ __forceinline__ Core carve(uint8_t* base, int stages_b, bool f16) {
   Core c;
   c.Bst = base;
-  uint64_t* bars = reinterpret_cast<uint64_t*>(base + stages_b * STAGE_B_BYTES);
+  uint64_t* bars = reinterpret_cast<uint64_t*>(base + stages_b * stage_b_bytes(f16));
   c.b_full = bars;
   c.b_empty = c.b_full + MAX_B_STAGES;
   c.a_full = c.b_empty + MAX_B_STAGES;
@@ -69,8 +73,10 @@
   const uint32_t pad = (1024u - (tc05::smem_u32(smem_raw) & 1023u)) & 1023u;
   uint8_t* base = smem_raw + pad;
   constexpr int SB = Policy::kStagesB;
-  Core c = carve(base, SB);
-  uint8_t* policy_smem = base + core_smem(SB);
+  constexpr bool F16 = Policy::kF16;
+  constexpr int STAGE_B = stage_b_bytes(F16), TILE_B = tile_b_bytes(F16);
+  Core c = carve(base, SB, F16);
+  uint8_t* policy_smem = base + core_smem(SB, F16);
 
   const int tid = threadIdx.x, warp = tid >> 5, lane = tid & 31;
   const int cta = blockIdx.x, ncta = gridDim.x;
@@ -106,7 +112,7 @@
     const int grp = warp >> 2;
     const int wq = warp & 3;
     const uint32_t lane_addr = tmem_base + ((uint32_t)(wq * 32) << 16);
-    const uint32_t a_hi = lane_addr + COL_A + grp * 64;
+    const uint32_t a_hi = lane_addr + COL_A + grp * (F16 ? 32 : 64);
     Policy pol(p, policy_smem, tid);
     uint32_t use = 0;
     uint32_t gk0 = 0;
@@ -119,19 +125,36 @@
       PhaseTimer tm;
       tm.start(cta, tid);
       pol.step_begin(m_tile, sub, kb_first, tm);
+      int sig = 0;
+      if constexpr (F16) sig = pol.row_exp(sub);
       for (int kb = kb_first; kb < nkb; kb += NGROUPS, ++use) {
         float v[32];
         if (!(p.dbg & 8)) pol.produce(sub, kb, v);
         tc05::mbar_wait(&c.a_empty[grp], (use & 1u) ^ 1u);
         tc05::fence_after_thread_sync();
         if (!(p.dbg & 1)) {
-          uint32_t part[32];
-#pragma unroll
-          for (int j = 0; j < 32; ++j) part[j] = tc05::tf32_rna_bits(v[j]);
-          tc05::tmem_st_32x32(a_hi, part);
-#pragma unroll
-          for (int j = 0; j < 32; ++j) part[j] = tc05::tf32_rna_bits(v[j] - __uint_as_float(part[j]));
-          tc05::tmem_st_32x32(a_hi + 32, part);
+          if constexpr (F16) {
+            const float sc = tc05::exp2i(sig);
+            uint32_t hi[16], lo[16];
+#pragma unroll
+            for (int j = 0; j < 16; ++j) {
+              const float x0 = v[2 * j] * sc, x1 = v[2 * j + 1] * sc;
+              hi[j] = tc05::f16x2_rn_bits(x0, x1);
+              float h0, h1;
+              tc05::f16x2_to_f32(hi[j], h0, h1);
+              lo[j] = tc05::f16x2_rn_bits(x0 - h0, x1 - h1);
+            }
+            tc05::tmem_st_32x16(a_hi, hi);
+            tc05::tmem_st_32x16(a_hi + 16, lo);
+          } else {
+            uint32_t part[32];
+#pragma unroll
+            for (int j = 0; j < 32; ++j) part[j] = tc05::tf32_rna_bits(v[j]);
+            tc05::tmem_st_32x32(a_hi, part);
+#pragma unroll
+            for (int j = 0; j < 32; ++j) part[j] = tc05::tf32_rna_bits(v[j] - __uint_as_float(part[j]));
+            tc05::tmem_st_32x32(a_hi + 32, part);
+          }
           tc05::tmem_wait_st();
         }
         tc05::fence_before_thread_sync();
@@ -149,12 +172,28 @@
         tc05::tmem_ld_32x16(lane_addr + COL_MAIN + grp * EW, vm);
         tc05::tmem_ld_32x16(lane_addr + COL_CORR + grp * EW, vc);
         tc05::tmem_wait_ld();
+        int ncols = BN;
+        const int32_t* wexp = nullptr;
+        float rsig = 1.f;
+        if constexpr (F16) { ncols = pol.out_cols(); wexp = pol.col_exp(sub); rsig = tc05::exp2i(-sig); }
 #pragma unroll 1
         for (int cc = grp; cc < BN / EW; cc += NGROUPS) {
           const int col = cc * EW;
           float x[EW];
 #pragma unroll
           for (int j = 0; j < EW; ++j) x[j] = __uint_as_float(vm[j]) + __uint_as_float(vc[j]);
+          if constexpr (F16) {
+            if (col >= ncols) break;
+#pragma unroll
+            for (int j = 0; j < EW; j += 4) {
+              int4 w = make_int4(0, 0, 0, 0);
+              if (col + j < ncols) w = __ldg(reinterpret_cast<const int4*>(wexp + col + j));
+              x[j + 0] = x[j + 0] * tc05::exp2i(-w.x) * rsig;
+              x[j + 1] = x[j + 1] * tc05::exp2i(-w.y) * rsig;
+              x[j + 2] = x[j + 2] * tc05::exp2i(-w.z) * rsig;
+              x[j + 3] = x[j + 3] * tc05::exp2i(-w.w) * rsig;
+            }
+          }
           if (cc + NGROUPS < BN / EW) {
             tc05::tmem_ld_32x16(lane_addr + COL_MAIN + col + NGROUPS * EW, vm);
             tc05::tmem_ld_32x16(lane_addr + COL_CORR + col + NGROUPS * EW, vc);
@@ -186,18 +225,18 @@
           if (p.dbg & 4) {
             tc05::mbar_arrive(&c.b_full[st]);
           } else {
-            uint8_t* dst = c.Bst + st * STAGE_B_BYTES;
-            tc05::mbar_arrive_expect_tx(&c.b_full[st], STAGE_B_BYTES);
+            uint8_t* dst = c.Bst + st * STAGE_B;
+            tc05::mbar_arrive_expect_tx(&c.b_full[st], STAGE_B);
             tc05::tma_load_2d(dst, &map_hi, &c.b_full[st], col0, row0);
-            tc05::tma_load_2d(dst + TILE_B_BYTES, &map_lo, &c.b_full[st], col0, row0);
+            tc05::tma_load_2d(dst + TILE_B, &map_lo, &c.b_full[st], col0, row0);
           }
         }
         __syncwarp();
       }
     }
   } else {
-    constexpr uint32_t idesc256 = tc05::umma_idesc_tf32(BM, 2 * BN);
-    constexpr uint32_t idesc128 = tc05::umma_idesc_tf32(BM, BN);
+    constexpr uint32_t idesc256 = F16 ? tc05::umma_idesc_f16(BM, 2 * BN) : tc05::umma_idesc_tf32(BM, 2 * BN);
+    constexpr uint32_t idesc128 = F16 ? tc05::umma_idesc_f16(BM, BN) : tc05::umma_idesc_tf32(BM, BN);
     uint32_t cnt = 0;
     const uint32_t d_main = tmem_base + COL_MAIN, d_corr = tmem_base + COL_CORR;
     for (int it = 0; it < nsteps; ++it) {
@@ -211,14 +250,26 @@
         tc05::mbar_wait2(&c.b_full[sb], (cnt / SB) & 1u, &c.a_full[sa], (cnt / NGROUPS) & 1u);
         tc05::fence_after_thread_sync();
         if (tc05::elect_one()) {
-          const uint32_t a_hi = tmem_base + COL_A + sa * 64, a_lo = a_hi + 32;
-          const uint64_t dB = tc05::umma_desc_kmajor_sw128(tc05::smem_u32(c.Bst + sb * STAGE_B_BYTES));
+          const uint32_t b_addr = tc05::smem_u32(c.Bst + sb * STAGE_B);
           if (!(p.dbg & 2)) {
-#pragma unroll
-            for (int k = 0; k < BK / 8; ++k) {
-              const uint32_t acc = (kb | k) != 0 ? 1u : 0u;
-              tc05::umma_tf32_ts(d_main, a_hi + 8 * k, dB + 2 * k, idesc256, acc);
-              tc05::umma_tf32_ts(d_corr, a_lo + 8 * k, dB + 2 * k, idesc128, 1u);
+            if constexpr (F16) {
+              const uint32_t a_hi = tmem_base + COL_A + sa * 32, a_lo = a_hi + 16;
+              const uint64_t dB = tc05::umma_desc_kmajor_sw64(b_addr);
+#pragma unroll
+              for (int k = 0; k < BK / 16; ++k) {
+                const uint32_t acc = (kb | k) != 0 ? 1u : 0u;
+                tc05::umma_f16_ts(d_main, a_hi + 8 * k, dB + 2 * k, idesc256, acc);
+                tc05::umma_f16_ts(d_corr, a_lo + 8 * k, dB + 2 * k, idesc128, 1u);
+              }
+            } else {
+              const uint32_t a_hi = tmem_base + COL_A + sa * 64, a_lo = a_hi + 32;
+              const uint64_t dB = tc05::umma_desc_kmajor_sw128(b_addr);
+#pragma unroll
+              for (int k = 0; k < BK / 8; ++k) {
+                const uint32_t acc = (kb | k) != 0 ? 1u : 0u;
+                tc05::umma_tf32_ts(d_main, a_hi + 8 * k, dB + 2 * k, idesc256, acc);
+                tc05::umma_tf32_ts(d_corr, a_lo + 8 * k, dB + 2 * k, idesc128, 1u);
+              }
             }
           }
           tc05::umma_commit(&c.a_empty[sa]);
@@ -289,16 +340,18 @@
   return fn;
 }
 
-inline int make_weight_map(CUtensorMap* map, const float* W, int rows, int cols, const char* who,
-                           int box_rows = BN) {
+inline int make_weight_map(CUtensorMap* map, const void* W, int rows, int cols, const char* who,
+                           int box_rows = BN, bool f16 = false) {
   EncodeTiledFn enc = get_encode_fn();
   if (!enc) { lnb::set_err("%s: cuTensorMapEncodeTiled unavailable", who); return LNB_ERR_UNSUPPORTED; }
+  const size_t esize = f16 ? 2 : 4;
   cuuint64_t gdim[2] = {(cuuint64_t)cols, (cuuint64_t)rows};
-  cuuint64_t gstride[1] = {(cuuint64_t)cols * sizeof(float)};
+  cuuint64_t gstride[1] = {(cuuint64_t)cols * esize};
   cuuint32_t box[2] = {(cuuint32_t)BK, (cuuint32_t)box_rows};
   cuuint32_t estr[2] = {1, 1};
-  CUresult r = enc(map, CU_TENSOR_MAP_DATA_TYPE_FLOAT32, 2, const_cast<float*>(W), gdim, gstride,
-                   box, estr, CU_TENSOR_MAP_INTERLEAVE_NONE, CU_TENSOR_MAP_SWIZZLE_128B,
+  CUresult r = enc(map, f16 ? CU_TENSOR_MAP_DATA_TYPE_FLOAT16 : CU_TENSOR_MAP_DATA_TYPE_FLOAT32, 2,
+                   const_cast<void*>(W), gdim, gstride, box, estr, CU_TENSOR_MAP_INTERLEAVE_NONE,
+                   f16 ? CU_TENSOR_MAP_SWIZZLE_64B : CU_TENSOR_MAP_SWIZZLE_128B,
                    CU_TENSOR_MAP_L2_PROMOTION_L2_256B, CU_TENSOR_MAP_FLOAT_OOB_FILL_NONE);
   if (r != CUDA_SUCCESS) {
     lnb::set_err("%s: cuTensorMapEncodeTiled failed (CUresult %d)", who, (int)r);
diff --git a/lanczosnetwork_b200/model/_common.py b/lanczosnetwork_b200/model/_common.py
--- a/lanczosnetwork_b200/model/_common.py
+++ b/lanczosnetwork_b200/model/_common.py
@@ -325,6 +325,9 @@
     w_hi, w_lo, bias = self._wcache.split_conv_stack(
         'filter.stack.%d' % first, [self.filter[t].weight for t in layers],
         [self.filter[t].bias for t in layers], kw)
+    w16 = self._wcache.conv_stack_f16(
+        'filter.stack.%d' % first, [self.filter[t].weight for t in layers],
+        [self.filter[t].bias for t in layers], kw, [dims[t] for t in layers], S)
     if S == 0:
       coeff, stride = None, 0
     elif coeffs is not None:
@@ -338,14 +341,14 @@
           coeff_stride=stride, X=None if (node_ids is not None and first == 0) else state,
           node_ids=node_ids if first == 0 else None,
           emb=self.embedding.weight if (node_ids is not None and first == 0) else None,
-          want_state=True)
+          want_state=True, w16=w16)
       return self._readout(state, mask)
     _, score = ops.spectral_stack_forward(
         ctx.prep(), V, w_hi, w_lo, bias, [dims[t] for t in layers], H, S, coeff=coeff,
         coeff_stride=stride, X=None if (node_ids is not None and first == 0) else state,
         node_ids=node_ids if first == 0 else None,
         emb=self.embedding.weight if (node_ids is not None and first == 0) else None,
-        readout=(head.weight, head.bias, att.weight.reshape(-1), att.bias), mask=mask)
+        readout=(head.weight, head.bias, att.weight.reshape(-1), att.bias), mask=mask, w16=w16)
     return score
 
   def _sparse_stack_ok(self, N, E1, K):
diff --git a/lanczosnetwork_b200/ops.py b/lanczosnetwork_b200/ops.py
--- a/lanczosnetwork_b200/ops.py
+++ b/lanczosnetwork_b200/ops.py
@@ -6,7 +6,7 @@
 from ._lib import GemmDesc, SpectralStack
 
 __all__ = [
-    'bgemm', 'split_tf32', 'linear_tf32x3', 'linear_tf32x3_grouped', 'graph_prepare', 'spectral_conv_fused',
+    'bgemm', 'split_tf32', 'split_f16_scaled', 'linear_tf32x3', 'linear_tf32x3_grouped', 'graph_prepare', 'spectral_conv_fused',
     'graph_prepare_sparse', 'graph_prepare_sparse_packed', 'fused_conv_supported', 'spectral_stack_forward', 'ritz_rowmap', 'ritz_filter_mlp', 'embedding_rows', 'ritz_power_table', 'readout',
     'operator_chain', 'operator_chain_supported', 'graph_messages', 'graph_messages_supported', 'gaussian_laplacian', 'lanczos_tridiag', 'lanczos_ritz', 'tridiag_ritz', 'tridiag_powers',
     'symmetrize_filters', 'segment_sum_forward', 'segment_sum_backward', 'launch_count',
@@ -257,11 +257,28 @@
   if (n_short or dense_filter or N > 128 or Din % 32 or K > 32 or K % 4 or H % 4 or H > 128 or
       E1 > 16):
     return False
-  smem = 2 * 32768 + 256 + 1024 + 2 * 128 * (max(Din, H) + 4) * 4 + 128 * K * 4 + 4096
+  smem = 3 * 16384 + 256 + 1024 + 2 * 128 * (max(Din, H) + 4) * 4 + 128 * K * 4 + 4096
   return smem <= 227 * 1024
 
 
-def spectral_conv_fused(X, Q, coeff, prep, w_hi, w_lo, bias, relu=True, write_pad=True):
+def split_f16_scaled(w_hi, w_lo, step_cols, rows_per_block):
+  _need_cuda(w_hi, w_lo)
+  w_hi, w_lo = _f32c(w_hi), _f32c(w_lo)
+  rows, cols = w_hi.shape
+  nb = rows // rows_per_block
+  assert nb * rows_per_block == rows and len(step_cols) == nb, (rows, rows_per_block, step_cols)
+  hi16 = torch.empty((rows, cols), device=w_hi.device, dtype=torch.float16)
+  lo16 = torch.empty_like(hi16)
+  w_exp = torch.empty((nb, 2, rows_per_block), device=w_hi.device, dtype=torch.int32)
+  sc = (ctypes.c_int * max(nb, 1))(*[int(c) for c in step_cols])
+  with torch.cuda.device(w_hi.device):
+    _lib.check(_lib.load().lnb_split_f16_scaled(
+        _stream(w_hi), _ptr(w_hi), _ptr(w_lo), rows, cols, int(rows_per_block), sc, _ptr(hi16),
+        _ptr(lo16), _ptr(w_exp)), 'lnb_split_f16_scaled')
+  return hi16, lo16, w_exp
+
+
+def spectral_conv_fused(X, Q, coeff, prep, w_hi, w_lo, bias, relu=True, write_pad=True, w16=None):
   _need_cuda(X, Q, coeff, w_hi, w_lo, bias)
   X, Q = _f32c(X), _f32c(Q)
   ell_val, ell_idx, ell_max, gext, tiles = prep
@@ -274,18 +291,21 @@
   E1 = ell_val.shape[1]
   H = w_hi.shape[0]
   assert w_hi.shape[1] == (S + E1) * Din, (w_hi.shape, S, E1, Din)
+  if w16 is None:
+    w16 = split_f16_scaled(w_hi, w_lo, [S * Din], H)
+  hi16, lo16, w_exp = w16
   out = torch.empty((B, N, H), device=X.device, dtype=torch.float32)
   with torch.cuda.device(X.device):
     _lib.check(_lib.load().lnb_spectral_conv_fused(
         _stream(X), _ptr(X), _ptr(Q), _ptr(coeff), _ptr(ell_val), _ptr(ell_idx), _ptr(ell_max),
-        _ptr(gext), _ptr(tiles), _ptr(w_hi), _ptr(w_lo), _ptr(bias), B, N, Din, E1, K, S, H,
+        _ptr(gext), _ptr(tiles), _ptr(hi16), _ptr(lo16), _ptr(w_exp), _ptr(bias), B, N, Din, E1, K, S, H,
         int(bool(relu)), int(bool(write_pad)), _ptr(out)), 'lnb_spectral_conv_fused')
   return out
 
 
 def spectral_stack_forward(prep, Q, w_hi, w_lo, bias, dins, H, S, coeff=None, coeff_stride=0,
                            X=None, node_ids=None, emb=None, want_state=False, write_pad=True,
-                           readout=None, mask=None, relu=True):
+                           readout=None, mask=None, relu=True, w16=None):
   ell_val, ell_idx, ell_max, gext, tiles = prep
   _need_cuda(Q, w_hi, w_lo, bias, coeff, X, node_ids, emb, mask)
   Q = _f32c(Q)
@@ -305,7 +325,10 @@
     d.coeff, d.coeff_layer_stride = coeff.data_ptr(), int(coeff_stride)
   d.ell_val, d.ell_idx, d.ell_max = ell_val.data_ptr(), ell_idx.data_ptr(), ell_max.data_ptr()
   d.gext, d.tiles = gext.data_ptr(), tiles.data_ptr()
-  d.W_hi, d.W_lo = w_hi.data_ptr(), w_lo.data_ptr()
+  if w16 is None:
+    w16 = split_f16_scaled(w_hi, w_lo, [int(S) * int(v) for v in dins], int(H))
+  hi16, lo16, w_exp = w16
+  d.W_hi16, d.W_lo16, d.w_exp = hi16.data_ptr(), lo16.data_ptr(), w_exp.data_ptr()
   d.bias = bias.data_ptr() if bias is not None else None
   state = score = None
   if want_state or readout is None:
diff --git a/lanczosnetwork_b200/spectral_conv.py b/lanczosnetwork_b200/spectral_conv.py
--- a/lanczosnetwork_b200/spectral_conv.py
+++ b/lanczosnetwork_b200/spectral_conv.py
@@ -71,6 +71,21 @@
       hi, lo = ops.split_tf32(torch.cat(rows, dim=0).contiguous())
       return hi, lo, torch.cat([b.detach() for b in biases], dim=0).contiguous()
     return self._get((name, weights[0].device.index), tag, build, list(weights) + list(biases))
+
+  def conv_f16(self, name, weight, S, Din):
+    def build():
+      hi, lo = self.split(name, weight)
+      return ops.split_f16_scaled(hi, lo, [S * Din], weight.shape[0])
+    return self._get((name + '.f16', weight.device.index), (weight.data_ptr(), weight._version, S, Din),
+                     build, [weight])
+
+  def conv_stack_f16(self, name, weights, biases, kw, dins, S):
+    tag = tuple((t.data_ptr(), t._version) for t in list(weights) + list(biases)) + (kw, tuple(dins), S)
+
+    def build():
+      hi, lo, _ = self.split_conv_stack(name, weights, biases, kw)
+      return ops.split_f16_scaled(hi, lo, [S * d for d in dins], weights[0].shape[0])
+    return self._get((name + '.f16', weights[0].device.index), tag, build, list(weights) + list(biases))
 
   def clear(self):
     self.invalidate()
@@ -152,8 +167,9 @@
       ops.fused_conv_supported(N, Din, Qv.shape[2], weight.shape[0], len(short_dist), dense_filter,
                                num_long, L.shape[3])):
     w_hi, w_lo = cache.split(name, weight)
+    w16 = cache.conv_f16(name, weight, num_long, Din)
     return ops.spectral_conv_fused(state, Qv, coeff, ctx.prep(), w_hi, w_lo, bias, True,
-                                   write_pad=last or not next_fused)
+                                   write_pad=last or not next_fused, w16=w16)
   return graph_conv_layer_unfused(state, L, Qv, coeff, dense_filter, short_dist, num_long, weight,
                                   bias, cache, name)
 
```

After: 2.297 million (median of 6 runs). +11.0%, better.
